# DearCaat/RRT-MIL

Hardware: AMD Instinct MI355X
Metric: slides/sec RRTEncoder fwd, N=9000 D=512 region_num=8 (higher is better)
Workload: dtype f32

## Files before the change

### include/rrt_hip.h

```cpp
#ifndef RRT_HIP_H
#define RRT_HIP_H
#include <stddef.h>
#include <stdint.h>

#ifdef __cplusplus
extern "C" {
#endif

#define RRT_ABI_VERSION 29
#define RRT_MAX_RMSA_LAYERS 8
#define RRT_MAX_CRMSA_K 8

enum {
  RRT_OK = 0,
  RRT_E_INVALID = -1,
  RRT_E_UNSUPPORTED = -2,
  RRT_E_WORKSPACE = -3,
  RRT_E_HANDOVER = -4
};

enum { RRT_COMPUTE_F32 = 0, RRT_COMPUTE_BF16 = 1, RRT_COMPUTE_F16 = 2, RRT_COMPUTE_F32X3 = 3 };
enum { RRT_POS_NONE = 0, RRT_POS_PEG = 1, RRT_POS_PPEG = 2 };
enum { RRT_EPEG_ATTN = 0, RRT_EPEG_VALUE_BF = 1, RRT_EPEG_VALUE_AF = 2 };

enum { RRT_ACT_NONE = 0, RRT_ACT_RELU = 1, RRT_ACT_GELU = 2, RRT_ACT_TANH = 3, RRT_ACT_SIGMOID = 4 };

typedef struct rrt_grid {
  int64_t L;
  int32_t H;
  int32_t s;
  int32_t regions_side;
  int64_t add;
} rrt_grid;

typedef struct rrt_encoder_desc {
  int32_t dim;
  int32_t n_heads;
  int32_t n_rmsa_layers;
  int32_t region_num;
  int32_t region_size;
  int32_t min_region_num;
  float   min_region_ratio;
  int32_t epeg;
  int32_t epeg_k;
  int32_t cr_msa;
  int32_t crmsa_k;
  int32_t crmsa_heads;
  int32_t crmsa_mlp;
  int32_t all_shortcut;
  int32_t compute;
  int32_t ffn;
  int32_t ffn_act;
  int32_t ffn_hidden;
  int32_t pos;
  int32_t pos_pos;
  int32_t peg_k;
  int32_t peg_1d;
  int32_t epeg_2d;
  int32_t epeg_type;
  int32_t weights16_valid;
  int32_t solo;
} rrt_encoder_desc;

typedef struct rrt_attn_weights {
  const float *norm_w, *norm_b;
  const float *qkv_w, *qkv_b;
  const float *proj_w, *proj_b;
  const float *pe_w, *pe_b;
  const float *norm2_w, *norm2_b;
  const float *fc1_w, *fc1_b;
  const float *fc2_w, *fc2_b;
} rrt_attn_weights;

typedef struct rrt_encoder_weights {
  rrt_attn_weights rmsa[RRT_MAX_RMSA_LAYERS];
  rrt_attn_weights crmsa;
  const float *phi;
  const float *phi0_w, *phi2_w;
  const float *norm_w, *norm_b;
  const float *pos_w[3], *pos_b[3];
  uint64_t version;
} rrt_encoder_weights;

int         rrt_abi_version(void);
const char *rrt_strerror(int code);

int rrt_region_grid(int64_t L, int32_t region_num, int32_t region_size,
                    int32_t min_region_num, float min_region_ratio, rrt_grid *out);

int rrt_encoder_workspace_size(const rrt_encoder_desc *desc, int64_t n_tokens, size_t *bytes);

#define RRT_PLAN_FUSED      1
#define RRT_PLAN_FUSED_PROJ 2
#define RRT_PLAN_FUSED16    4
#define RRT_PLAN_FUSED_X3   8
#define RRT_PLAN_CRMSA_PARTS 16
#define RRT_PLAN_ATTN_HD    32
int rrt_encoder_plan(const rrt_encoder_desc *desc, int64_t n_tokens, int32_t *flags);

int rrt_encoder_forward_f32(const rrt_encoder_desc *desc, const rrt_encoder_weights *w,
                            const float *x, float *y, int64_t n_tokens,
                            void *workspace, size_t workspace_bytes, void *stream);

enum {
  RRT_EV_START = 0,
  RRT_EV_LN_PARTITION,
  RRT_EV_QKV,
  RRT_EV_ATTN,
  RRT_EV_PROJ,
  RRT_EV_CR_COMBINE,
  RRT_EV_CR_INNER,
  RRT_EV_END,
  RRT_EV_COUNT
};
int rrt_encoder_forward_events_f32(const rrt_encoder_desc *desc, const rrt_encoder_weights *w,
                                   const float *x, float *y, int64_t n_tokens,
                                   void *workspace, size_t workspace_bytes, void *stream,
                                   void **events);

typedef struct rrt_phase_gate rrt_phase_gate;
int rrt_phase_gate_create(rrt_phase_gate **out);
int rrt_phase_gate_destroy(rrt_phase_gate *gate);
int rrt_encoder_forward_gated_f32(const rrt_encoder_desc *desc, const rrt_encoder_weights *w,
                                  const float *x, float *y, int64_t n_tokens,
                                  void *workspace, size_t workspace_bytes, void *stream,
                                  rrt_phase_gate *gate, void **events);

int rrt_encoder_batch_workspace_size(const rrt_encoder_desc *desc, int32_t batch, int64_t n_tokens, size_t *bytes);
int rrt_encoder_forward_batch_f32(const rrt_encoder_desc *desc, const rrt_encoder_weights *w,
                                  const float *x, float *y, int32_t batch, int64_t n_tokens,
                                  void *workspace, size_t workspace_bytes, void *stream);


int rrt_ln_partition_f32(const float *x, const float *gamma, const float *beta, float *u,
                         int64_t L, int32_t dim, const rrt_grid *g, void *stream);

int rrt_linear_f32(const float *A, const float *B, const float *bias, float *C,
                   int64_t M, int32_t N, int32_t K, int32_t q_cols, float q_scale,
                   int32_t compute , void *stream);

int rrt_linear_unpartition_residual_f32(const float *A, const float *B, const float *bias,
                                        const float *resid, float *out, int32_t N, int32_t K,
                                        const rrt_grid *g, int32_t compute, void *stream);

int rrt_region_attention_f32(const float *qkv, const float *pe_w, float *o,
                             int32_t n_regions, int32_t P, int32_t dim, int32_t heads,
                             int32_t epeg_k, void *stream);

int rrt_region_attention_hd_supported(int32_t P, int32_t dim, int32_t heads, int32_t epeg_k);
int rrt_region_attention_hd_f32(const float *qkv, const float *pe_w, float *o,
                                int32_t n_regions, int32_t P, int32_t dim, int32_t heads,
                                int32_t epeg_k, void *stream);

int rrt_rmsa_fused_f32(const float *u, const float *qkv_w, const float *qkv_b, const float *pe_w,
                       float *o, int32_t n_regions, int32_t P, int32_t dim, int32_t heads,
                       int32_t epeg_k, int32_t compute, void *stream);

int rrt_rmsa_fused_proj_f32(const float *u, const float *qkv_w, const float *qkv_b, const float *pe_w,
                            const float *proj_w, const float *proj_b, const float *resid, float *out,
                            float *o_scratch, int32_t *counters, int32_t dim, int32_t heads, int32_t epeg_k,
                            const rrt_grid *g, void *stream);
int rrt_rmsa_fused_proj_stats_f32(const float *u, const float *qkv_w, const float *qkv_b, const float *pe_w,
                                  const float *proj_w, const float *proj_b, const float *resid, float *out,
                                  float *o_scratch, int32_t *counters, const float *ln2_gamma, const float *phi,
                                  int32_t crmsa_k, float *part, int32_t dim, int32_t heads, int32_t epeg_k,
                                  const rrt_grid *g, void *stream);
int rrt_crmsa_combine_parts_f32(const float *x1, const float *part, const float *gamma, const float *beta,
                                const float *phi, float *wdisp, float *rep, int64_t n_tokens, int32_t dim, int32_t k,
                                const rrt_grid *g8, void *stream);
int rrt_device_error(int32_t clear);
int rrt_debug_rmsa_fused_proj_f32(const float *u, const float *qkv_w, const float *qkv_b, const float *pe_w,
                                  const float *proj_w, const float *proj_b, const float *resid, float *out,
                                  float *o_scratch, int32_t *counters, int32_t dim, int32_t heads, int32_t epeg_k,
                                  const rrt_grid *g, int32_t lag, int32_t spin_limit, int32_t wait_extra, void *stream);

int rrt_cast16(const float *src, uint16_t *dst, int64_t n, int32_t compute, void *stream);
int rrt_ln_partition16(const float *x, const float *gamma, const float *beta, uint16_t *u, int64_t L,
                       int32_t dim, const rrt_grid *g, int32_t compute, void *stream);
int rrt_linear16_f32(const uint16_t *A, const uint16_t *B, const float *bias, const float *resid, float *C,
                     int64_t M, int32_t N, int32_t K, const rrt_grid *g, int32_t compute, void *stream);
int rrt_rmsa_fused16(const uint16_t *u, const uint16_t *qkv_w, const float *qkv_b, const float *pe_w,
                     uint16_t *o, int32_t n_regions, int32_t P, int32_t dim, int32_t heads, int32_t epeg_k,
                     int32_t compute, void *stream);
int rrt_rmsa_pair16_proj(const uint16_t *u, const uint16_t *qkv_w, const float *qkv_b, const float *pe_w,
                         const uint16_t *proj_w, const float *proj_b, const float *resid, float *out, uint16_t *o,
                         int32_t *cnt, int32_t dim, int32_t heads, int32_t epeg_k, const rrt_grid *g, int32_t compute,
                         void *stream);

int rrt_cast_split(const float *src, void *dst, int64_t n, void *stream);
int rrt_ln_partition_split(const float *x, const float *gamma, const float *beta, void *u, int64_t L,
                           int32_t dim, const rrt_grid *g, void *stream);
int rrt_linear_split_f32(const void *A, const void *B, const float *bias, const float *resid, float *C,
                         int64_t M, int32_t N, int32_t K, const rrt_grid *g, void *stream);
int rrt_rmsa_fused_x3(const void *u, const void *qkv_w, const float *qkv_b, const float *pe_w, void *o,
                      int32_t n_regions, int32_t P, int32_t dim, int32_t heads, int32_t epeg_k, void *stream);

int rrt_crmsa_logits_f32(const float *x1, const float *gamma, const float *beta, const float *phi,
                         float *mean_rstd, float *logits, int64_t L, int32_t dim, int32_t k,
                         const rrt_grid *g8, void *stream);
int rrt_crmsa_combine_f32(const float *x1, const float *gamma, const float *beta,
                          const float *mean_rstd, const float *logits, float *wdisp, float *rep,
                          int64_t L, int32_t dim, int32_t k, const rrt_grid *g8, void *stream);
int rrt_crmsa_region_f32(const float *x1, const float *gamma, const float *beta, const float *phi,
                         float *mean_rstd, float *logits, float *wdisp, float *rep,
                         int64_t L, int32_t dim, int32_t k, const rrt_grid *g8, void *stream);
int rrt_crmsa_region4_f32(const float *x1, const float *gamma, const float *beta, const float *phi,
                          float *mean_rstd, float *logits, float *wdisp, float *rep,
                          int64_t L, int32_t dim, int32_t k, const rrt_grid *g8,
                          void *scratch, size_t scratch_bytes, void *stream);
int rrt_crmsa_stream4_f32(const float *x1, const float *gamma, const float *beta, const float *phi,
                          float *mean_rstd, float *logits, float *wdisp, float *rep,
                          int64_t L, int32_t dim, int32_t k, const rrt_grid *g8,
                          void *scratch, size_t scratch_bytes, void *stream);
int rrt_crmsa_dispatch_ln_f32(const float *x1, const float *x0, const float *wdisp,
                              const float *rep2, const float *gamma,
                              const float *beta, float *y, int64_t L, int32_t dim, int32_t k,
                              const rrt_grid *g8, void *stream);
int rrt_crmsa_mlp_logits_f32(const float *hid, const float *w2, float *logits, int64_t rows,
                             int32_t hdim, int32_t k, void *stream);
int rrt_layernorm_f32(const float *x1, const float *x0, const float *gamma, const float *beta,
                      float *y, int64_t L, int32_t dim, void *stream);

typedef struct rrt_mil_desc {
  rrt_encoder_desc enc;
  int32_t input_dim;
  int32_t emb_act;
  int32_t n_classes;
  int32_t pool_hidden;
  int32_t pool_act;
  int32_t pool_gated;
  int32_t input16;
} rrt_mil_desc;

typedef struct rrt_mil_weights {
  rrt_encoder_weights enc;
  const float *emb_w, *emb_b;
  const float *pool_a_w, *pool_a_b;
  const float *pool_b_w, *pool_b_b;
  const float *pool_c_w, *pool_c_b;
  const float *pred_w, *pred_b;
} rrt_mil_weights;

int rrt_attn_pool_workspace_size(int64_t n_tokens, int32_t dim, int32_t hidden, size_t *bytes);
int rrt_attn_pool_f32(const float *y, const float *hid_a, const float *hid_b, const float *c_w, const float *c_b,
                      float *pooled, float *attn, float *a_raw, int64_t n_tokens, int32_t dim, int32_t hidden,
                      void *workspace, size_t workspace_bytes, void *stream);
int rrt_attn_pool_backward_f32(const float *y, const float *hid_a, const float *hid_b, const float *c_w,
                               const float *attn, const float *pooled, const float *d_pooled,
                               const float *d_attn, const float *d_raw, const float *c_ext, float *dy,
                               float *dhid_a, float *dhid_b, float *dwcb, int64_t n_tokens, int32_t dim,
                               int32_t hidden, void *workspace, size_t workspace_bytes, void *stream);

int rrt_mil_workspace_size(const rrt_mil_desc *desc, int64_t n_tokens, size_t *bytes);

int rrt_mil_forward_f32(const rrt_mil_desc *desc, const rrt_mil_weights *w, const float *x,
                        float *logits, float *attn, int32_t no_norm, float *feat, int64_t n_tokens,
                        void *workspace, size_t workspace_bytes, void *stream);

int rrt_pool_workspace_size(int64_t n_tokens, int32_t dim, int32_t hidden, int32_t gated, size_t *bytes);
int rrt_pool_predict_f32(const float *y, const float *a_w, const float *a_b, const float *b_w,
                         const float *b_b, const float *c_w, const float *c_b, const float *pred_w,
                         const float *pred_b, float *pooled, float *logits, float *attn, int32_t no_norm,
                         int64_t n_tokens, int32_t dim, int32_t hidden, int32_t act, int32_t n_classes,
                         int32_t compute, void *workspace, size_t workspace_bytes, void *stream);

int rrt_linear_act_f32(const float *A, const float *B, const float *bias, float *C, int64_t M, int32_t N,
                       int32_t K, int32_t act, int32_t compute, void *stream);

int rrt_branch_pool_workspace_size(int64_t n_tokens, int32_t dim, int32_t hidden, int32_t n_branches, size_t *bytes);
int rrt_branch_pool_f32(const float *y, const float *hid_a, const float *hid_b, const float *c_w, const float *c_b,
                        float *pooled, float *attn, float *a_raw, int64_t n_tokens, int32_t dim, int32_t hidden,
                        int32_t n_branches, void *workspace, size_t workspace_bytes, void *stream);
int rrt_branch_pool_backward_f32(const float *y, const float *hid_a, const float *hid_b, const float *c_w,
                                 const float *attn, const float *pooled, const float *d_pooled, const float *d_raw,
                                 float *dy, float *dhid_a, float *dhid_b, float *dwcb, int64_t n_tokens, int32_t dim,
                                 int32_t hidden, int32_t n_branches, void *workspace, size_t workspace_bytes,
                                 void *stream);

int rrt_topk_rows_f32(const float *x, int64_t *idx, int32_t n_rows, int64_t n, int32_t k, void *stream);

typedef struct rrt_clam_desc {
  rrt_encoder_desc enc;
  int32_t input_dim;
  int32_t emb_act;
  int32_t has_rrt;
  int32_t n_classes;
  int32_t per_branch;
  int32_t gated;
  int32_t hidden;
  int32_t k_sample;
} rrt_clam_desc;

typedef struct rrt_clam_weights {
  rrt_encoder_weights enc;
  const float *emb_w, *emb_b;
  const float *a_w, *a_b;
  const float *b_w, *b_b;
  const float *c_w, *c_b;
  const float *cls_w, *cls_b;
} rrt_clam_weights;

int rrt_clam_workspace_size(const rrt_clam_desc *desc, int64_t n_tokens, size_t *bytes);
int rrt_clam_forward_f32(const rrt_clam_desc *desc, const rrt_clam_weights *w, const float *x, float *logits,
                         float *a_raw, float *attn, float *features, int64_t *topk_idx, int64_t n_tokens,
                         void *workspace, size_t workspace_bytes, void *stream);

int rrt_instance_max_workspace_size(int64_t n_tokens, int32_t dim, int32_t n_classes, size_t *bytes);
int rrt_instance_max_f32(const float *y, const float *w, const float *b, float *classes, float *cmax, int64_t *argmax,
                         int64_t n_tokens, int32_t dim, int32_t n_classes, void *workspace, size_t workspace_bytes,
                         void *stream);

int rrt_dsmil_pool_workspace_size(int64_t n_tokens, int32_t dim, int32_t q_dim, int32_t n_classes, size_t *bytes);
int rrt_dsmil_pool_f32(const float *feats, const int64_t *argmax, const float *q_w, const float *q_b, const float *fcc_w,
                       const float *fcc_b, float *logits, float *A, float *B, float *a_raw, int64_t n_tokens, int32_t dim,
                       int32_t q_dim, int32_t n_classes, void *workspace, size_t workspace_bytes, void *stream);

typedef struct rrt_dsmil_desc {
  rrt_encoder_desc enc;
  int32_t input_dim;
  int32_t emb_act;
  int32_t has_rrt;
  int32_t n_classes;
  int32_t q_dim;
} rrt_dsmil_desc;

typedef struct rrt_dsmil_weights {
  rrt_encoder_weights enc;
  const float *emb_w, *emb_b;
  const float *icls_w, *icls_b;
  const float *q_w, *q_b;
  const float *fcc_w, *fcc_b;
} rrt_dsmil_weights;

int rrt_dsmil_workspace_size(const rrt_dsmil_desc *desc, int64_t n_tokens, size_t *bytes);
int rrt_dsmil_forward_f32(const rrt_dsmil_desc *desc, const rrt_dsmil_weights *w, const float *x, float *logits,
                          float *classes_max, float *A, float *B, int64_t *argmax, int64_t n_tokens, void *workspace,
                          size_t workspace_bytes, void *stream);

typedef struct rrt_executor rrt_executor;
typedef struct rrt_bag {
  const float *x;
  float *y;
  int64_t n_tokens;
} rrt_bag;
int rrt_executor_create(const rrt_encoder_desc *desc, int32_t n_streams, int64_t max_tokens,
                        rrt_executor **out);
int rrt_executor_create_on_streams(const rrt_encoder_desc *desc, int32_t n_streams, void *const *streams,
                                   int64_t max_tokens, rrt_executor **out);
int rrt_executor_forward(rrt_executor *ex, const rrt_encoder_weights *w, const rrt_bag *bags,
                         int32_t n_bags, void *stream);
int rrt_executor_destroy(rrt_executor *ex);

int rrt_region_attention_backward_workspace_size(int32_t n_regions, int32_t P, int32_t dim, int32_t heads,
                                                 int32_t epeg_k, size_t *bytes);
int rrt_region_attention_backward_f32(const float *qkv, const float *pe_w, const float *o, const float *d_o,
                                      float *d_qkv, float *d_pe_w, int32_t n_regions, int32_t P, int32_t dim,
                                      int32_t heads, int32_t epeg_k, void *workspace, size_t workspace_bytes,
                                      void *stream);
int rrt_peg_f32(const float *x, const float *const *w, const float *const *b, float *y, int64_t N, int32_t dim, int32_t k,
                int32_t conv_1d, int32_t ppeg, void *stream);
int rrt_peg_backward_workspace_size(int64_t N, int32_t dim, int32_t k, int32_t ppeg, size_t *bytes);
int rrt_peg_backward_f32(const float *x, const float *dy, const float *const *w, float *dx, float *const *dw, float *const *db,
                         int64_t N, int32_t dim, int32_t k, int32_t conv_1d, int32_t ppeg, void *workspace,
                         size_t workspace_bytes, void *stream);
int rrt_attn_scoremap_scratch_size(int32_t n_regions, int32_t P, int32_t heads, int32_t k, int32_t backward, size_t *bytes);
int rrt_attn_scoremap_f32(const float *qkv, const float *pe_w, float *o, int32_t n_regions, int32_t P, int32_t dim,
                          int32_t heads, int32_t k, void *scratch, size_t scratch_bytes, void *stream);
int rrt_attn_scoremap_backward_f32(const float *qkv, const float *pe_w, const float *d_o, float *d_qkv, float *d_pe_w,
                                   int32_t n_regions, int32_t P, int32_t dim, int32_t heads, int32_t k, void *scratch,
                                   size_t scratch_bytes, void *stream);
// ... 110 lines not shown
```

### rrt-mil_amd/_lib.py

```python
import ctypes as C
import os

HERE = os.path.dirname(os.path.abspath(__file__))
LIB_PATH = os.path.join(HERE, "librrt_hip.so")

RRT_MAX_RMSA_LAYERS = 8
RRT_MAX_CRMSA_K = 8
ABI_VERSION = 29

_f32p = C.POINTER(C.c_float)


class Grid(C.Structure):
    _fields_ = [("L", C.c_int64), ("H", C.c_int32), ("s", C.c_int32),
                ("regions_side", C.c_int32), ("add", C.c_int64)]


class EncoderDesc(C.Structure):
    _fields_ = [("dim", C.c_int32), ("n_heads", C.c_int32), ("n_rmsa_layers", C.c_int32),
                ("region_num", C.c_int32), ("region_size", C.c_int32), ("min_region_num", C.c_int32),
                ("min_region_ratio", C.c_float), ("epeg", C.c_int32), ("epeg_k", C.c_int32),
                ("cr_msa", C.c_int32), ("crmsa_k", C.c_int32), ("crmsa_heads", C.c_int32),
                ("crmsa_mlp", C.c_int32), ("all_shortcut", C.c_int32), ("compute", C.c_int32),
                ("ffn", C.c_int32), ("ffn_act", C.c_int32), ("ffn_hidden", C.c_int32),
                ("pos", C.c_int32), ("pos_pos", C.c_int32), ("peg_k", C.c_int32), ("peg_1d", C.c_int32),
                ("epeg_2d", C.c_int32), ("epeg_type", C.c_int32), ("weights16_valid", C.c_int32),
                ("solo", C.c_int32)]


class AttnWeights(C.Structure):
    _fields_ = [(n, C.c_void_p) for n in ("norm_w", "norm_b", "qkv_w", "qkv_b", "proj_w", "proj_b",
                                          "pe_w", "pe_b", "norm2_w", "norm2_b", "fc1_w", "fc1_b",
                                          "fc2_w", "fc2_b")]


class EncoderWeights(C.Structure):
    _fields_ = [("rmsa", AttnWeights * RRT_MAX_RMSA_LAYERS), ("crmsa", AttnWeights),
                ("phi", C.c_void_p), ("phi0_w", C.c_void_p), ("phi2_w", C.c_void_p),
                ("norm_w", C.c_void_p), ("norm_b", C.c_void_p),
                ("pos_w", C.c_void_p * 3), ("pos_b", C.c_void_p * 3), ("version", C.c_uint64)]


class AttnGrads(C.Structure):
    _fields_ = [(n, C.c_void_p) for n in ("norm", "qkv_w", "qkv_b", "proj_w", "proj_b", "pe_w", "pe_b", "norm2",
                                          "fc1_w", "fc1_b", "fc2_w", "fc2_b")]


class EncoderGrads(C.Structure):
    _fields_ = [("rmsa", AttnGrads * RRT_MAX_RMSA_LAYERS), ("crmsa", AttnGrads), ("phi", C.c_void_p),
                ("phi0_w", C.c_void_p), ("phi2_w", C.c_void_p), ("norm", C.c_void_p),
                ("pos_w", C.c_void_p * 3), ("pos_b", C.c_void_p * 3)]


class MilDesc(C.Structure):
    _fields_ = [("enc", EncoderDesc), ("input_dim", C.c_int32), ("emb_act", C.c_int32),
                ("n_classes", C.c_int32), ("pool_hidden", C.c_int32), ("pool_act", C.c_int32),
                ("pool_gated", C.c_int32), ("input16", C.c_int32)]


class MilWeights(C.Structure):
    _fields_ = [("enc", EncoderWeights)] + [(n, C.c_void_p) for n in (
        "emb_w", "emb_b", "pool_a_w", "pool_a_b", "pool_b_w", "pool_b_b", "pool_c_w", "pool_c_b",
        "pred_w", "pred_b")]


class ClamDesc(C.Structure):
    _fields_ = [("enc", EncoderDesc), ("input_dim", C.c_int32), ("emb_act", C.c_int32), ("has_rrt", C.c_int32),
                ("n_classes", C.c_int32), ("per_branch", C.c_int32), ("gated", C.c_int32), ("hidden", C.c_int32),
                ("k_sample", C.c_int32)]


class ClamWeights(C.Structure):
    _fields_ = [("enc", EncoderWeights)] + [(n, C.c_void_p) for n in (
        "emb_w", "emb_b", "a_w", "a_b", "b_w", "b_b", "c_w", "c_b", "cls_w", "cls_b")]


class DsmilDesc(C.Structure):
    _fields_ = [("enc", EncoderDesc), ("input_dim", C.c_int32), ("emb_act", C.c_int32), ("has_rrt", C.c_int32),
                ("n_classes", C.c_int32), ("q_dim", C.c_int32)]


class DsmilWeights(C.Structure):
    _fields_ = [("enc", EncoderWeights)] + [(n, C.c_void_p) for n in (
        "emb_w", "emb_b", "icls_w", "icls_b", "q_w", "q_b", "fcc_w", "fcc_b")]


class NystromDesc(C.Structure):
    _fields_ = [(n, C.c_int32) for n in ("dim", "heads", "dim_head", "num_landmarks", "pinv_iterations", "residual",
                                         "residual_conv_kernel")]


class NystromWeights(C.Structure):
    _fields_ = [(n, C.c_void_p) for n in ("qkv_w", "out_w", "out_b", "conv_w")]


class TransmilDesc(C.Structure):
    _fields_ = [("input_dim", C.c_int32), ("n_classes", C.c_int32), ("act", C.c_int32), ("attn", NystromDesc)]


class TransmilLayerWeights(C.Structure):
    _fields_ = [("norm_w", C.c_void_p), ("norm_b", C.c_void_p), ("attn", NystromWeights)]


class TransmilWeights(C.Structure):
    _fields_ = [("fc1_w", C.c_void_p), ("fc1_b", C.c_void_p), ("cls_token", C.c_void_p), ("layer", TransmilLayerWeights * 2),
                ("pos_w", C.c_void_p * 3), ("pos_b", C.c_void_p * 3), ("norm_w", C.c_void_p), ("norm_b", C.c_void_p),
                ("fc2_w", C.c_void_p), ("fc2_b", C.c_void_p)]


class Bag(C.Structure):
    _fields_ = [("x", C.c_void_p), ("y", C.c_void_p), ("n_tokens", C.c_int64)]


ACT_NONE, ACT_RELU, ACT_GELU, ACT_TANH, ACT_SIGMOID = 0, 1, 2, 3, 4
ACT_BY_NAME = {"relu": ACT_RELU, "gelu": ACT_GELU, "tanh": ACT_TANH}

SIGNATURES = {
    "rrt_abi_version": (C.c_int, []),
    "rrt_strerror": (C.c_char_p, [C.c_int]),
    "rrt_region_grid": (C.c_int, [C.c_int64, C.c_int32, C.c_int32, C.c_int32, C.c_float, C.POINTER(Grid)]),
    "rrt_encoder_workspace_size": (C.c_int, [C.POINTER(EncoderDesc), C.c_int64, C.POINTER(C.c_size_t)]),
    "rrt_encoder_plan": (C.c_int, [C.POINTER(EncoderDesc), C.c_int64, C.POINTER(C.c_int32)]),
    "rrt_encoder_forward_f32": (C.c_int, [C.POINTER(EncoderDesc), C.POINTER(EncoderWeights), C.c_void_p,
                                          C.c_void_p, C.c_int64, C.c_void_p, C.c_size_t, C.c_void_p]),
    "rrt_encoder_forward_events_f32": (C.c_int, [C.POINTER(EncoderDesc), C.POINTER(EncoderWeights), C.c_void_p,
                                                 C.c_void_p, C.c_int64, C.c_void_p, C.c_size_t, C.c_void_p,
                                                 C.POINTER(C.c_void_p)]),
    "rrt_encoder_batch_workspace_size": (C.c_int, [C.POINTER(EncoderDesc), C.c_int32, C.c_int64, C.POINTER(C.c_size_t)]),
    "rrt_encoder_forward_batch_f32": (C.c_int, [C.POINTER(EncoderDesc), C.POINTER(EncoderWeights), C.c_void_p, C.c_void_p,
                                                C.c_int32, C.c_int64, C.c_void_p, C.c_size_t, C.c_void_p]),
    "rrt_phase_gate_create": (C.c_int, [C.POINTER(C.c_void_p)]),
    "rrt_phase_gate_destroy": (C.c_int, [C.c_void_p]),
    "rrt_encoder_forward_gated_f32": (C.c_int, [C.POINTER(EncoderDesc), C.POINTER(EncoderWeights), C.c_void_p,
                                                C.c_void_p, C.c_int64, C.c_void_p, C.c_size_t, C.c_void_p,
                                                C.c_void_p, C.POINTER(C.c_void_p)]),
    "rrt_ln_partition_f32": (C.c_int, [C.c_void_p, C.c_void_p, C.c_void_p, C.c_void_p, C.c_int64,
                                       C.c_int32, C.POINTER(Grid), C.c_void_p]),
    "rrt_linear_f32": (C.c_int, [C.c_void_p, C.c_void_p, C.c_void_p, C.c_void_p, C.c_int64, C.c_int32,
                                 C.c_int32, C.c_int32, C.c_float, C.c_int32, C.c_void_p]),
    "rrt_linear_unpartition_residual_f32": (C.c_int, [C.c_void_p, C.c_void_p, C.c_void_p, C.c_void_p,
                                                      C.c_void_p, C.c_int32, C.c_int32, C.POINTER(Grid),
                                                      C.c_int32, C.c_void_p]),
    "rrt_region_attention_f32": (C.c_int, [C.c_void_p, C.c_void_p, C.c_void_p, C.c_int32, C.c_int32,
                                           C.c_int32, C.c_int32, C.c_int32, C.c_void_p]),
    "rrt_region_attention_hd_supported": (C.c_int, [C.c_int32] * 4),
    "rrt_region_attention_hd_f32": (C.c_int, [C.c_void_p, C.c_void_p, C.c_void_p, C.c_int32, C.c_int32,
                                              C.c_int32, C.c_int32, C.c_int32, C.c_void_p]),
    "rrt_rmsa_fused_f32": (C.c_int, [C.c_void_p] * 5 + [C.c_int32] * 6 + [C.c_void_p]),
    "rrt_rmsa_fused_proj_f32": (C.c_int, [C.c_void_p] * 10 + [C.c_int32] * 3 + [C.c_void_p] * 2),
    "rrt_device_error": (C.c_int, [C.c_int32]),
    "rrt_rmsa_fused_proj_stats_f32": (C.c_int, [C.c_void_p] * 12 + [C.c_int32, C.c_void_p] + [C.c_int32] * 3 + [C.c_void_p] * 2),
    "rrt_crmsa_combine_parts_f32": (C.c_int, [C.c_void_p] * 7 + [C.c_int64, C.c_int32, C.c_int32, C.POINTER(Grid), C.c_void_p]),
    "rrt_debug_rmsa_fused_proj_f32": (C.c_int, [C.c_void_p] * 10 + [C.c_int32] * 3 + [C.c_void_p] + [C.c_int32] * 3 + [C.c_void_p]),
    "rrt_cast16": (C.c_int, [C.c_void_p, C.c_void_p, C.c_int64, C.c_int32, C.c_void_p]),
    "rrt_ln_partition16": (C.c_int, [C.c_void_p, C.c_void_p, C.c_void_p, C.c_void_p, C.c_int64, C.c_int32,
                                     C.POINTER(Grid), C.c_int32, C.c_void_p]),
    "rrt_linear16_f32": (C.c_int, [C.c_void_p] * 5 + [C.c_int64, C.c_int32, C.c_int32, C.POINTER(Grid), C.c_int32,
                                                      C.c_void_p]),
    "rrt_rmsa_fused16": (C.c_int, [C.c_void_p] * 5 + [C.c_int32] * 6 + [C.c_void_p]),
    "rrt_rmsa_pair16_proj": (C.c_int, [C.c_void_p] * 10 + [C.c_int32] * 3 + [C.POINTER(Grid), C.c_int32, C.c_void_p]),
    "rrt_cast_split": (C.c_int, [C.c_void_p, C.c_void_p, C.c_int64, C.c_void_p]),
    "rrt_ln_partition_split": (C.c_int, [C.c_void_p, C.c_void_p, C.c_void_p, C.c_void_p, C.c_int64, C.c_int32,
                                         C.POINTER(Grid), C.c_void_p]),
    "rrt_linear_split_f32": (C.c_int, [C.c_void_p] * 5 + [C.c_int64, C.c_int32, C.c_int32, C.POINTER(Grid), C.c_void_p]),
    "rrt_rmsa_fused_x3": (C.c_int, [C.c_void_p] * 5 + [C.c_int32] * 5 + [C.c_void_p]),
    "rrt_crmsa_logits_f32": (C.c_int, [C.c_void_p] * 6 + [C.c_int64, C.c_int32, C.c_int32,
                                                         C.POINTER(Grid), C.c_void_p]),
    "rrt_crmsa_combine_f32": (C.c_int, [C.c_void_p] * 7 + [C.c_int64, C.c_int32, C.c_int32,
                                                          C.POINTER(Grid), C.c_void_p]),
    "rrt_crmsa_region_f32": (C.c_int, [C.c_void_p] * 8 + [C.c_int64, C.c_int32, C.c_int32, C.POINTER(Grid), C.c_void_p]),
    "rrt_crmsa_region4_f32": (C.c_int, [C.c_void_p] * 8 + [C.c_int64, C.c_int32, C.c_int32, C.POINTER(Grid), C.c_void_p,
                                                         C.c_size_t, C.c_void_p]),
    "rrt_crmsa_stream4_f32": (C.c_int, [C.c_void_p] * 8 + [C.c_int64, C.c_int32, C.c_int32, C.POINTER(Grid), C.c_void_p,
                                                         C.c_size_t, C.c_void_p]),
    "rrt_crmsa_dispatch_ln_f32": (C.c_int, [C.c_void_p] * 7 + [C.c_int64, C.c_int32, C.c_int32,
                                                              C.POINTER(Grid), C.c_void_p]),
    "rrt_crmsa_mlp_logits_f32": (C.c_int, [C.c_void_p] * 3 + [C.c_int64, C.c_int32, C.c_int32, C.c_void_p]),
    "rrt_layernorm_f32": (C.c_int, [C.c_void_p] * 5 + [C.c_int64, C.c_int32, C.c_void_p]),
    "rrt_peg_f32": (C.c_int, [C.c_void_p] * 4 + [C.c_int64] + [C.c_int32] * 4 + [C.c_void_p]),
    "rrt_peg_backward_workspace_size": (C.c_int, [C.c_int64] + [C.c_int32] * 3 + [C.POINTER(C.c_size_t)]),
    "rrt_peg_backward_f32": (C.c_int, [C.c_void_p] * 6 + [C.c_int64] + [C.c_int32] * 4 + [C.c_void_p, C.c_size_t, C.c_void_p]),
    "rrt_attn_scoremap_scratch_size": (C.c_int, [C.c_int32] * 5 + [C.POINTER(C.c_size_t)]),
    "rrt_attn_scoremap_f32": (C.c_int, [C.c_void_p] * 3 + [C.c_int32] * 5 + [C.c_void_p, C.c_size_t, C.c_void_p]),
    "rrt_attn_scoremap_backward_f32": (C.c_int, [C.c_void_p] * 5 + [C.c_int32] * 5 + [C.c_void_p, C.c_size_t, C.c_void_p]),
    "rrt_value_pe_f32": (C.c_int, [C.c_void_p] * 4 + [C.c_int32] * 7 + [C.c_void_p]),
    "rrt_value_pe_backward_f32": (C.c_int, [C.c_void_p] * 7 + [C.c_int32] * 7 + [C.c_void_p]),
    "rrt_mil_workspace_size": (C.c_int, [C.POINTER(MilDesc), C.c_int64, C.POINTER(C.c_size_t)]),
    "rrt_mil_forward_f32": (C.c_int, [C.POINTER(MilDesc), C.POINTER(MilWeights), C.c_void_p, C.c_void_p,
                                      C.c_void_p, C.c_int32, C.c_void_p, C.c_int64, C.c_void_p, C.c_size_t,
                                      C.c_void_p]),
    "rrt_pool_workspace_size": (C.c_int, [C.c_int64, C.c_int32, C.c_int32, C.c_int32, C.POINTER(C.c_size_t)]),
    "rrt_pool_predict_f32": (C.c_int, [C.c_void_p] * 12 + [C.c_int32, C.c_int64] + [C.c_int32] * 5 +
                             [C.c_void_p, C.c_size_t, C.c_void_p]),
    "rrt_attn_pool_workspace_size": (C.c_int, [C.c_int64, C.c_int32, C.c_int32, C.POINTER(C.c_size_t)]),
    "rrt_attn_pool_f32": (C.c_int, [C.c_void_p] * 8 + [C.c_int64, C.c_int32, C.c_int32, C.c_void_p, C.c_size_t, C.c_void_p]),
    "rrt_attn_pool_backward_f32": (C.c_int, [C.c_void_p] * 14 + [C.c_int64, C.c_int32, C.c_int32, C.c_void_p, C.c_size_t,
                                                                 C.c_void_p]),
    "rrt_branch_pool_workspace_size": (C.c_int, [C.c_int64, C.c_int32, C.c_int32, C.c_int32, C.POINTER(C.c_size_t)]),
    "rrt_branch_pool_f32": (C.c_int, [C.c_void_p] * 8 + [C.c_int64, C.c_int32, C.c_int32, C.c_int32, C.c_void_p, C.c_size_t,
                                                         C.c_void_p]),
    "rrt_branch_pool_backward_f32": (C.c_int, [C.c_void_p] * 12 + [C.c_int64, C.c_int32, C.c_int32, C.c_int32, C.c_void_p,
                                                                   C.c_size_t, C.c_void_p]),
    "rrt_topk_rows_f32": (C.c_int, [C.c_void_p, C.c_void_p, C.c_int32, C.c_int64, C.c_int32, C.c_void_p]),
    "rrt_clam_workspace_size": (C.c_int, [C.POINTER(ClamDesc), C.c_int64, C.POINTER(C.c_size_t)]),
    "rrt_clam_forward_f32": (C.c_int, [C.POINTER(ClamDesc), C.POINTER(ClamWeights)] + [C.c_void_p] * 6 +
                             [C.c_int64, C.c_void_p, C.c_size_t, C.c_void_p]),
    "rrt_instance_max_workspace_size": (C.c_int, [C.c_int64, C.c_int32, C.c_int32, C.POINTER(C.c_size_t)]),
    "rrt_instance_max_f32": (C.c_int, [C.c_void_p] * 6 + [C.c_int64, C.c_int32, C.c_int32, C.c_void_p, C.c_size_t, C.c_void_p]),
    "rrt_dsmil_pool_workspace_size": (C.c_int, [C.c_int64, C.c_int32, C.c_int32, C.c_int32, C.POINTER(C.c_size_t)]),
    "rrt_dsmil_pool_f32": (C.c_int, [C.c_void_p] * 10 + [C.c_int64, C.c_int32, C.c_int32, C.c_int32, C.c_void_p, C.c_size_t,
                                                         C.c_void_p]),
    "rrt_dsmil_workspace_size": (C.c_int, [C.POINTER(DsmilDesc), C.c_int64, C.POINTER(C.c_size_t)]),
    "rrt_dsmil_forward_f32": (C.c_int, [C.POINTER(DsmilDesc), C.POINTER(DsmilWeights)] + [C.c_void_p] * 6 +
                              [C.c_int64, C.c_void_p, C.c_size_t, C.c_void_p]),
    "rrt_executor_create": (C.c_int, [C.POINTER(EncoderDesc), C.c_int32, C.c_int64, C.POINTER(C.c_void_p)]),
    "rrt_executor_create_on_streams": (C.c_int, [C.POINTER(EncoderDesc), C.c_int32, C.POINTER(C.c_void_p), C.c_int64,
                                                 C.POINTER(C.c_void_p)]),
    "rrt_executor_forward": (C.c_int, [C.c_void_p, C.POINTER(EncoderWeights), C.POINTER(Bag), C.c_int32,
                                       C.c_void_p]),
    "rrt_executor_destroy": (C.c_int, [C.c_void_p]),
    "rrt_region_attention_backward_workspace_size": (C.c_int, [C.c_int32] * 5 + [C.POINTER(C.c_size_t)]),
    "rrt_region_attention_backward_f32": (C.c_int, [C.c_void_p] * 6 + [C.c_int32] * 5 + [C.c_void_p, C.c_size_t,
                                                                                       C.c_void_p]),
    "rrt_layernorm_backward_f32": (C.c_int, [C.c_void_p] * 6 + [C.c_int64, C.c_int32, C.POINTER(Grid), C.c_void_p,
                                                                C.c_size_t, C.c_void_p]),
    "rrt_reduce_partials_f32": (C.c_int, [C.c_void_p] * 3 + [C.c_int32, C.c_int64, C.c_int64] + [C.c_int32] * 4 + [C.c_void_p]),
    "rrt_linear_backward_workspace_size": (C.c_int, [C.c_int64, C.c_int32, C.c_int32, C.POINTER(C.c_size_t)]),
    "rrt_linear_backward_f32": (C.c_int, [C.c_void_p] * 6 + [C.c_int64, C.c_int32, C.c_int32, C.c_int32,
                                                             C.c_void_p, C.c_size_t, C.c_void_p]),
    "rrt_encoder_train_sizes": (C.c_int, [C.POINTER(EncoderDesc), C.c_int64, C.POINTER(C.c_size_t),
                                          C.POINTER(C.c_size_t)]),
    "rrt_encoder_forward_train_f32": (C.c_int, [C.POINTER(EncoderDesc), C.POINTER(EncoderWeights), C.c_void_p,
                                                C.c_void_p, C.c_int64, C.c_void_p, C.c_size_t, C.c_float,
                                                C.c_uint64, C.POINTER(C.c_float), C.c_void_p]),
    "rrt_encoder_backward_f32": (C.c_int, [C.POINTER(EncoderDesc), C.POINTER(EncoderWeights), C.c_void_p, C.c_void_p,
                                           C.c_void_p, C.c_size_t, C.POINTER(EncoderGrads), C.c_void_p, C.c_int64,
                                           C.c_void_p, C.c_size_t, C.c_float, C.c_uint64, C.POINTER(C.c_float),
                                           C.c_void_p]),
    "rrt_linear_act_f32": (C.c_int, [C.c_void_p] * 4 + [C.c_int64, C.c_int32, C.c_int32, C.c_int32, C.c_int32,
                                                        C.c_void_p]),
    "rrt_nystrom_workspace_size": (C.c_int, [C.POINTER(NystromDesc), C.c_int64, C.POINTER(C.c_size_t)]),
    "rrt_nystrom_attention_f32": (C.c_int, [C.POINTER(NystromDesc), C.POINTER(NystromWeights), C.c_void_p, C.c_void_p,
                                            C.c_int64, C.c_void_p, C.c_size_t, C.c_void_p]),
    "rrt_nystrom_landmarks_f32": (C.c_int, [C.c_void_p] * 3 + [C.c_int64, C.c_int32, C.c_void_p]),
    "rrt_nystrom_landmark_sim_f32": (C.c_int, [C.c_void_p] * 3 + [C.c_int32, C.c_void_p]),
    "rrt_nystrom_landmark_attn_workspace_size": (C.c_int, [C.c_int64, C.c_int32, C.POINTER(C.c_size_t)]),
    "rrt_nystrom_landmark_attn_f32": (C.c_int, [C.c_void_p] * 3 + [C.c_int64, C.c_int32, C.c_void_p, C.c_size_t, C.c_void_p]),
    "rrt_nystrom_pinv_workspace_size": (C.c_int, [C.c_int32, C.POINTER(C.c_size_t)]),
    "rrt_nystrom_pinv_f32": (C.c_int, [C.c_void_p] * 2 + [C.c_int32, C.c_int32, C.c_void_p, C.c_size_t, C.c_void_p]),
    "rrt_nystrom_zav_f32": (C.c_int, [C.c_void_p] * 3 + [C.c_int32, C.c_void_p]),
    "rrt_nystrom_output_f32": (C.c_int, [C.c_void_p] * 5 + [C.c_int64, C.c_int32, C.c_int32, C.c_void_p]),
    "rrt_ppeg_side_f32": (C.c_int, [C.c_void_p] * 4 + [C.c_int32, C.c_int32, C.c_void_p]),
    "rrt_transmil_workspace_size": (C.c_int, [C.POINTER(TransmilDesc), C.c_int64, C.POINTER(C.c_size_t)]),
    "rrt_transmil_forward_f32": (C.c_int, [C.POINTER(TransmilDesc), C.POINTER(TransmilWeights)] + [C.c_void_p] * 3 +
                                 [C.c_int64, C.c_void_p, C.c_size_t, C.c_void_p]),
}

COMPUTE_F32, COMPUTE_BF16, COMPUTE_F16, COMPUTE_F32X3 = 0, 1, 2, 3
POS_NONE, POS_PEG, POS_PPEG = 0, 1, 2
EPEG_ATTN, EPEG_VALUE_BF, EPEG_VALUE_AF = 0, 1, 2

PLAN_FUSED, PLAN_FUSED_PROJ, PLAN_FUSED16, PLAN_FUSED_X3, PLAN_CRMSA_PARTS, PLAN_ATTN_HD = 1, 2, 4, 8, 16, 32
EV_START, EV_LN_PARTITION, EV_QKV, EV_ATTN, EV_PROJ, EV_CR_COMBINE, EV_CR_INNER, EV_END, EV_COUNT = range(9)

_lib = None


class RRTHipError(RuntimeError):
    pass


def load(path=None):
    global _lib
    if _lib is not None and path is None:
        return _lib
    p = path or os.environ.get("RRT_HIP_LIB") or LIB_PATH
    if not os.path.exists(p):
        raise RRTHipError(
            f"{p} is missing: the HIP extension is the only compute path. Build it with "
            "`python rrt-mil_amd/build.py` (needs /opt/rocm/bin/hipcc).")
    lib = C.CDLL(p)
    for name, (res, args) in SIGNATURES.items():
        fn = getattr(lib, name)
        fn.restype = res
        fn.argtypes = args
    if lib.rrt_abi_version() != ABI_VERSION:
        raise RRTHipError(f"librrt_hip.so ABI {lib.rrt_abi_version()} != binding {ABI_VERSION}; rebuild")
    if path is None:
        _lib = lib
    return lib


E_HANDOVER = -4


def device_error(clear=False):
    return int(load().rrt_device_error(1 if clear else 0))


def check(rc, what=""):
    if rc != 0:
        msg = load().rrt_strerror(rc).decode()
        if rc == -2:
            raise NotImplementedError(f"rrt_hip {what}: {msg}")
        if rc == E_HANDOVER:
            msg += (" -- sticky until cleared: torch.cuda.synchronize(), discard the outputs of the forwards in flight, "
                    "rrt_mil_amd.device_error(clear=True), run them again")
        raise RRTHipError(f"rrt_hip {what} failed ({rc}): {msg}")


def region_grid(L, region_num=8, region_size=0, min_region_num=0, min_region_ratio=0.0):
    g = Grid()
    check(load().rrt_region_grid(L, region_num, region_size, min_region_num, min_region_ratio, C.byref(g)),
          "rrt_region_grid")
    return g
```

### rrt-mil_amd/csrc/api.hip

```cpp
#include <math.h>
#include <stdio.h>
#include <string.h>

#include "internal.h"

namespace {

thread_local char g_detail[256] = "";

int unsupported(const char* why) {
  snprintf(g_detail, sizeof(g_detail), "%s", why);
  return RRT_E_UNSUPPORTED;
}

int64_t ceil_sqrt(int64_t n) {
  int64_t r = (int64_t)floor(sqrt((double)n));
  while (r * r > n) --r;
  while ((r + 1) * (r + 1) <= n) ++r;
  return r * r == n ? r : r + 1;
}

inline size_t align_up(size_t v, size_t a) { return (v + a - 1) / a * a; }

#define RRT_TRY(call)                     \
// ... 30 lines not shown
  const size_t R8 = (size_t)g8.regions_side * g8.regions_side;
  if (d.n_rmsa_layers > 0) w.w16 = (uint16_t*)take((size_t)d.n_rmsa_layers * 4 * D * D);
  if (d.cr_msa) w.wcr16 = (uint16_t*)take(2 * D * D);
  if (d.n_rmsa_layers > 0) {
    w.uo = take(Np * D);
    w.qkv = take(Np * 3 * D);
    w.xa = take((size_t)N * D);
    if (d.n_rmsa_layers > 1 || d.ffn) w.xb = take((size_t)N * D);
    w.proj_cnt = (int*)take((size_t)g.regions_side * g.regions_side);
    if (d.epeg && d.epeg_type != RRT_EPEG_ATTN) w.pe_out = take(Np * D);
    if (d.epeg && d.epeg_2d && d.epeg_type == RRT_EPEG_ATTN) {
      const size_t sm = attn_scoremap_scratch_floats(g.regions_side * g.regions_side, g.s * g.s, d.n_heads, d.epeg_k, 1);
      if (sm) w.smap = take(sm);
    }
  }
  if (d.ffn) {
    if (!w.xa) w.xa = take((size_t)N * D);
    if (!w.xb) w.xb = take((size_t)N * D);
    w.ffn_ln = take((size_t)N * D);
    w.ffn_hid = take((size_t)N * d.ffn_hidden);
  }
  if (d.cr_msa) {
    const size_t k = d.crmsa_k;
    w.mean_rstd = take((size_t)N * 2);
    w.logits = take(Np8 * k);
    w.wdisp = take(Np8 * k);
    w.rep = take(k * R8 * D);
    w.rep_qkv = take(k * R8 * 3 * D);
    w.rep_o = take(k * R8 * D);
    w.rep2 = take(k * R8 * D);
    w.rep16 = (uint16_t*)take(k * R8 * D / 2);
    w.repo16 = (uint16_t*)take(k * R8 * D / 2);
    if (d.n_rmsa_layers > 0) {
      w.cr_part = take(crmsa_region4_scratch_floats(to_dev(g8), d.crmsa_k));
      w.cr_cnt = (int*)take(64);
      if (D % 64 == 0) w.cr_pstat = take(crmsa_parts_floats(N, (int)D, d.crmsa_k));
    }
    if (d.crmsa_mlp) {
      w.v8 = take(Np8 * D);
      w.hid = take(Np8 * (D / 4));
    }
  }
  if (d.pos) w.xp = take((size_t)N * D);
  w.bytes = off ? off : 256;
  return w;
}

int check_desc(const rrt_encoder_desc* d, int64_t N) {
  if (!d || N <= 0) return RRT_E_INVALID;
  if (d->dim <= 0 || d->dim % 32 != 0) return unsupported("dim must be a positive multiple of 32");
  if (d->dim > 2048) return unsupported("dim > 2048");
  if (d->n_rmsa_layers < 0 || d->n_rmsa_layers > RRT_MAX_RMSA_LAYERS) return unsupported("n_layers-1 out of range");
  if (d->n_rmsa_layers > 0) {
    if (d->n_heads <= 0 || d->dim % d->n_heads != 0) return unsupported("n_heads must divide dim");
    if (d->epeg && (d->epeg_k <= 0 || d->epeg_k % 2 == 0)) return unsupported("epeg_k must be odd");
    if (d->epeg_type < RRT_EPEG_ATTN || d->epeg_type > RRT_EPEG_VALUE_AF) return unsupported("epeg_type must be attn / value_bf / value_af");
    if (d->epeg && (d->epeg_2d || d->epeg_type != RRT_EPEG_ATTN) && d->epeg_k > 63) return unsupported("epeg ablations: epeg_k <= 63");
    if (d->region_size <= 0 && d->region_num <= 0) return unsupported("region_num must be positive");
  }
  if (d->cr_msa) {
    if (d->crmsa_k <= 0 || d->crmsa_k > RRT_MAX_CRMSA_K) return unsupported("crmsa_k must be in [1,8]");
    if (d->crmsa_heads <= 0 || d->dim % d->crmsa_heads != 0) return unsupported("crmsa_heads must divide dim");
  }
  if (d->ffn) {
    if (d->ffn_hidden <= 0 || d->ffn_hidden % 32 != 0)
      return unsupported("ffn: hidden width int(dim * mlp_ratio) must be a positive multiple of 32");
    if (d->ffn_act != RRT_ACT_GELU && d->ffn_act != RRT_ACT_RELU) return unsupported("ffn_act must be gelu or relu");
  }
  if (d->pos) {
    if (d->pos != RRT_POS_PEG && d->pos != RRT_POS_PPEG) return unsupported("pos must be none / peg / ppeg");
    if (d->peg_k <= 0 || d->peg_k % 2 == 0 || d->peg_k > 11) return unsupported("peg_k must be odd and <= 11");
    if (d->pos_pos != -1 && d->pos_pos != 0) return unsupported("pos_pos must be -1 or 0");
  }
  if (N > (int64_t)4000000) return unsupported("bag larger than 4e6 tokens");
  if (d->compute < 0 || d->compute > RRT_COMPUTE_F32X3) return unsupported("compute must be RRT_COMPUTE_F32/BF16/F16/F32X3");
  return RRT_OK;
}

int region_grids(const rrt_encoder_desc* d, int64_t N, rrt_grid* g, rrt_grid* g8) {
  *g = rrt_grid{};
  if (d->n_rmsa_layers > 0) {
    int rc = rrt_region_grid(N, d->region_num, d->region_size, d->min_region_num, d->min_region_ratio, g);
    if (rc) return rc;
  }
  return rrt_region_grid(N, 8, 0, 0, 0.f, g8);
}
int resolve_grids(const rrt_encoder_desc* d, int64_t N, rrt_grid* g, rrt_grid* g8) {
  int rc = check_desc(d, N);
  return rc ? rc : region_grids(d, N, g, g8);
}

GridDev identity_grid(int64_t N) {
  GridDev g{};
  const int Hs = (int)ceil_sqrt(N);
  g.L = (int)N;
  g.H = g.s = Hs;
  g.rs = 1;
  g.P = g.Np = Hs * Hs;
  g.inv_H = g.inv_s = 1.0f / (float)Hs;
  g.inv_rs = 1.0f;
  g.inv_P = 1.0f / (float)g.P;
  g.Rt = 1;
  return g;
}

LinearEpilogue qkv_epilogue(const float* bias, int dim, int heads, int prec) {
  LinearEpilogue ep{};
  ep.prec = prec;
  ep.bias = bias;
  ep.q_cols = dim;
  ep.q_scale = 1.0f / sqrtf((float)(dim / heads));
  return ep;
}

LinearEpilogue proj_epilogue(const float* bias, const float* resid, const GridDev& g, int prec) {
  LinearEpilogue ep{};
  ep.prec = prec;
  ep.bias = bias;
  ep.resid = resid;
  ep.g = g;
  return ep;
}

hipError_t inner_attention(const float* u, int n_regions, int P, const rrt_attn_weights& w, int dim,
                           int heads, int epeg_k, float* qkv, float* o, int prec, bool solo, hipStream_t st) {
  const int M = n_regions * P;
  LinearEpilogue ep = qkv_epilogue(w.qkv_b, dim, heads, prec);
  ep.solo = solo;
  hipError_t e = launch_linear(u, w.qkv_w, qkv, M, 3 * dim, dim, ep, st);
  if (e != hipSuccess) return e;
  return launch_region_attention(qkv, epeg_k > 0 ? w.pe_w : nullptr, o, n_regions, P, dim, heads,
                                 epeg_k, st);
}

enum class LayerKind {
  Pair16Merged,
  Fused16,
  FusedX3,
  EpegVariant,
  FusedProj,
  Fused,
  Unfused,
};
enum class FrontKind { None, Mlp, Parts, RegionInFlight, Region4, Region, Stream4, TwoKernel };
enum class CastKind { None, Images16, Split };
struct EncoderPlan {
  LayerKind layer;
  bool parts;
  bool gated;
  bool attn_hd;
  CastKind casts;
  bool inner16;
  FrontKind front;
};

#ifndef RRT_STREAM4_MIN_P
#define RRT_STREAM4_MIN_P 145
#endif

EncoderPlan plan_encoder(const rrt_encoder_desc& d, const rrt_grid& g, const rrt_grid& g8, bool stops_before_crmsa) {
  EncoderPlan p{};
  p.layer = LayerKind::Unfused;
  const int D = d.dim;
  const bool want_x3 = d.compute == RRT_COMPUTE_F32X3;
  const int compute = want_x3 ? RRT_COMPUTE_F32 : d.compute;
  const bool lowp = compute != RRT_COMPUTE_F32 && D % 64 == 0;
  const GridDev gd8 = to_dev(g8);
  p.inner16 = d.cr_msa && lowp && rmsa_fused16_supported(64, D, d.crmsa_heads, 0);
  if (d.n_rmsa_layers > 0) {
    const GridDev gd = to_dev(g);
    const int R = gd.rs * gd.rs, heads = d.n_heads, ek = d.epeg ? d.epeg_k : 0;
    const bool rows_ok = rmsa_fused_supported_rows(gd.Np, D);
    static const bool want_merged16 = rrt_tune_env("RRT_PAIR16_PROJ") != nullptr;
    if (d.epeg && (d.epeg_2d || d.epeg_type != RRT_EPEG_ATTN)) {
      p.layer = LayerKind::EpegVariant;
    } else if (lowp && rmsa_fused16_supported(gd.P, D, heads, ek) && rows_ok) {
      p.layer = want_merged16 && rmsa_pair16_proj_supported(R, gd.P, D, heads, ek) ? LayerKind::Pair16Merged : LayerKind::Fused16;
    } else if (want_x3 && D % 256 == 0 && rmsa_fused_x3_supported(gd.P, D, heads, ek) && rows_ok) {
      p.layer = LayerKind::FusedX3;
    } else if (compute == RRT_COMPUTE_F32 && rows_ok && rmsa_fused_proj_supported(R, gd.P, D, heads, ek, compute)) {
      p.layer = LayerKind::FusedProj;
      p.parts = d.solo != 0 && d.cr_msa && !d.crmsa_mlp && !d.ffn && d.crmsa_k <= 4 && !stops_before_crmsa && D % 64 == 0 &&
                crmsa_combine_parts_supported(D, d.crmsa_k, gd8);
    } else if (rmsa_fused_supported(gd.P, D, heads, ek) && rows_ok) {
      p.layer = LayerKind::Fused;
    } else {
      p.attn_hd = region_attention_hd_supported(gd.P, D, heads, ek);
    }
    p.gated = gd.P > 112 && p.layer != LayerKind::EpegVariant && p.layer != LayerKind::Unfused;
    if (p.layer != LayerKind::EpegVariant) p.casts = lowp ? CastKind::Images16 : want_x3 ? CastKind::Split : CastKind::None;
  }
  if (!d.cr_msa || stops_before_crmsa) return p;
  const int k = d.crmsa_k;
  const bool has_counters = d.n_rmsa_layers > 0;
  static const bool no_region_inflight = rrt_tune_env("RRT_NO_REGION_INFLIGHT") != nullptr;
  static const bool region_lowp = rrt_tune_env("RRT_REGION_INFLIGHT_LOWP") != nullptr;
  if (d.crmsa_mlp) {
    p.front = FrontKind::Mlp;
  } else if (p.parts) {
    p.front = FrontKind::Parts;
  } else if (!no_region_inflight && !d.solo && p.layer != LayerKind::FusedX3 && (compute == RRT_COMPUTE_F32 || region_lowp) &&
             crmsa_region_supported(D, k, gd8)) {
    p.front = FrontKind::RegionInFlight;
  } else if (has_counters && crmsa_region4_supported(D, k, gd8) && gd8.P < RRT_STREAM4_MIN_P) {
    p.front = FrontKind::Region4;
  } else if (crmsa_region_enabled() && crmsa_region_supported(D, k, gd8)) {
    p.front = FrontKind::Region;
  } else if (has_counters && gd8.P >= RRT_STREAM4_MIN_P && crmsa_stream4_supported(D, k, gd8)) {
    p.front = FrontKind::Stream4;
  } else {
    p.front = FrontKind::TwoKernel;
  }
  return p;
}

}

GridDev to_dev(const rrt_grid& g) {
  GridDev d;
  d.L = (int)g.L;
  d.H = g.H;
  d.s = g.s;
  d.rs = g.regions_side;
  d.P = g.s * g.s;
  d.Np = g.H * g.H;
  d.inv_H = 1.0f / (float)d.H;
  d.inv_s = 1.0f / (float)d.s;
  d.inv_rs = 1.0f / (float)d.rs;
  d.inv_P = 1.0f / (float)d.P;
  d.Rt = d.rs * d.rs;
  return d;
}

extern "C" {

int rrt_abi_version(void) { return RRT_ABI_VERSION; }

const char* rrt_strerror(int code) {
  switch (code) {
    case RRT_OK: return "ok";
    case RRT_E_INVALID: return "invalid argument (null pointer or non-positive size)";
    case RRT_E_UNSUPPORTED: return g_detail[0] ? g_detail : "unsupported configuration";
    case RRT_E_WORKSPACE: return "workspace too small (see rrt_encoder_workspace_size)";
    case RRT_E_HANDOVER: return "an earlier merged R-MSA launch gave up its in-launch hand-over wait; outputs in flight are invalid "
                                "(synchronise, then rrt_device_error(1) to clear)";
    default: return code > 0 ? hipGetErrorString((hipError_t)code) : "unknown error";
  }
}

int rrt_region_grid(int64_t L, int32_t region_num, int32_t region_size, int32_t min_region_num,
                    float min_region_ratio, rrt_grid* out) {
  if (!out || L <= 0) return RRT_E_INVALID;
  if (region_size <= 0 && region_num <= 0) return RRT_E_INVALID;
  int64_t H = ceil_sqrt(L), s;
  if (region_size > 0) {
    H += ((-H) % region_size + region_size) % region_size;
    s = region_size;
  } else {
    H += ((-H) % region_num + region_num) % region_num;
    s = H / region_num;
  }
  int64_t add = H * H - L;
  if ((double)add > (double)L / ((double)min_region_ratio + 1e-8) || L < min_region_num) {
    H = ceil_sqrt(L);
    H += H % 2;
    add = H * H - L;
    s = H;
  }
  if (H > 46340) return RRT_E_INVALID;
  out->L = L;
  out->H = (int32_t)H;
  out->s = (int32_t)s;
  out->regions_side = (int32_t)(H / s);
  out->add = add;
  return RRT_OK;
}

int rrt_encoder_workspace_size(const rrt_encoder_desc* desc, int64_t n_tokens, size_t* bytes) {
  if (!bytes) return RRT_E_INVALID;
  rrt_grid g{}, g8{};
  int rc = resolve_grids(desc, n_tokens, &g, &g8);
  if (rc) return rc;
  *bytes = carve(*desc, n_tokens, g, g8, nullptr).bytes;
  return RRT_OK;
}

int rrt_encoder_plan(const rrt_encoder_desc* desc, int64_t n_tokens, int32_t* flags) {
  if (!flags) return RRT_E_INVALID;
  *flags = 0;
  rrt_grid g{}, g8{};
  int rc = resolve_grids(desc, n_tokens, &g, &g8);
  if (rc) return rc;
  if (desc->n_rmsa_layers <= 0) return RRT_OK;
  const EncoderPlan plan = plan_encoder(*desc, g, g8, false);
  switch (plan.layer) {
    case LayerKind::Pair16Merged:
    case LayerKind::Fused16: *flags = RRT_PLAN_FUSED16; break;
    case LayerKind::FusedX3: *flags = RRT_PLAN_FUSED_X3; break;
    case LayerKind::FusedProj: *flags = RRT_PLAN_FUSED | RRT_PLAN_FUSED_PROJ | (plan.parts ? RRT_PLAN_CRMSA_PARTS : 0); break;
    case LayerKind::Fused: *flags = RRT_PLAN_FUSED; break;
    case LayerKind::Unfused: *flags = plan.attn_hd ? RRT_PLAN_ATTN_HD : 0; break;
    case LayerKind::EpegVariant: break;
  }
  return RRT_OK;
}

struct rrt_phase_gate {
  hipEvent_t done;
  bool armed;
};

static int ffn_apply(const rrt_encoder_desc* desc, const rrt_attn_weights& lw, const float* xi, float* xo,
                     const Workspace& ws, int64_t N, hipStream_t st) {
  if (!lw.norm2_w || !lw.norm2_b || !lw.fc1_w || !lw.fc1_b || !lw.fc2_w || !lw.fc2_b) return RRT_E_INVALID;
  const int D = desc->dim;
  RRT_TRY(launch_layernorm(xi, nullptr, lw.norm2_w, lw.norm2_b, ws.ffn_ln, (int)N, D, st));
  LinearEpilogue e1{};
  e1.prec = desc->compute;
  e1.bias = lw.fc1_b;
  e1.act = desc->ffn_act;
  RRT_TRY(launch_linear(ws.ffn_ln, lw.fc1_w, ws.ffn_hid, (int)N, desc->ffn_hidden, D, e1, st));
  return (int)launch_linear(ws.ffn_hid, lw.fc2_w, xo, (int)N, D, desc->ffn_hidden,
                            proj_epilogue(lw.fc2_b, xi, identity_grid(N), desc->compute), st);
}

static int encoder_forward(const rrt_encoder_desc* desc_in, const rrt_encoder_weights* w, const float* x,
                           float* y, int64_t n_tokens, void* workspace, size_t workspace_bytes,
                           void* stream, void** events, rrt_phase_gate* gate = nullptr, float* rmsa_out = nullptr,
                           uint16_t* y16 = nullptr, bool* y16_done = nullptr) {
  if (y16_done) *y16_done = false;
  if (!desc_in || !w || !x || !y || x == y) return RRT_E_INVALID;
  int rc = check_desc(desc_in, n_tokens);
  if (rc) return rc;
  if (handover_err_peek(false)) return RRT_E_HANDOVER;
  rrt_grid g{}, g8{};
  rc = region_grids(desc_in, n_tokens, &g, &g8);
  if (rc) return rc;
  rrt_encoder_desc dloc = *desc_in;
  if (dloc.compute == RRT_COMPUTE_F32X3) dloc.compute = RRT_COMPUTE_F32;
  const rrt_encoder_desc* const desc = &dloc;
  hipStream_t st = (hipStream_t)stream;
  const int D = desc->dim;
  const int64_t N = n_tokens;
  Workspace ws = carve(*desc, N, g, g8, nullptr);
  if (!workspace || workspace_bytes < ws.bytes) return RRT_E_WORKSPACE;
  ws = carve(*desc, N, g, g8, (char*)workspace);
  const EncoderPlan plan = plan_encoder(*desc_in, g, g8, rmsa_out != nullptr);

  auto mark = [&](int i) -> hipError_t {
    return (events && events[i]) ? hipEventRecord((hipEvent_t)events[i], st) : hipSuccess;
  };
  RRT_TRY(mark(RRT_EV_START));

  auto ffn_block = [&](const rrt_attn_weights& lw, const float* xi, float* xo) -> int {
    return ffn_apply(desc, lw, xi, xo, ws, N, st);
  };

  const float* xin = x;
  auto pos_embed = [&]() -> int {
    if (!w->pos_w[0] || (desc->pos == RRT_POS_PPEG && (!w->pos_w[1] || !w->pos_w[2]))) return RRT_E_INVALID;
    RRT_TRY(launch_peg(xin, w->pos_w, w->pos_b, ws.xp, (int)N, D, desc->peg_k, desc->peg_1d, desc->pos == RRT_POS_PPEG, st));
    xin = ws.xp;
    return RRT_OK;
  };
  if (desc->pos && desc->pos_pos == -1) {
    rc = pos_embed();
    if (rc) return rc;
  }
  {
    const bool split = plan.casts == CastKind::Split;
    const size_t per_w = split ? 2 : 1;
    Cast16Jobs jobs{};
    auto add = [&](const float* src, uint16_t* dst, size_t n) {
      jobs.src[jobs.count] = src; jobs.dst[jobs.count] = dst; jobs.n4[jobs.count++] = n / 4;
    };
    if (plan.casts != CastKind::None) {
      for (int li = 0; li < desc->n_rmsa_layers; ++li) {
        const rrt_attn_weights& lw = w->rmsa[li];
        if (!lw.qkv_w || !lw.proj_w) return RRT_E_INVALID;
        uint16_t* base = ws.w16 + (size_t)li * per_w * 4 * D * D;
        add(lw.qkv_w, base, (size_t)3 * D * D);
        add(lw.proj_w, base + per_w * 3 * D * D, (size_t)D * D);
      }
    }
    if (plan.inner16) {
      if (!w->crmsa.qkv_w || !w->crmsa.proj_w) return RRT_E_INVALID;
      add(w->crmsa.qkv_w, ws.wcr16, (size_t)3 * D * D);
      add(w->crmsa.proj_w, ws.wcr16 + (size_t)3 * D * D, (size_t)D * D);
    }
    if (jobs.count && !desc->weights16_valid) RRT_TRY(split ? launch_cast_split(jobs, st) : launch_cast16(jobs, desc->compute, st));
  }
  rrt_phase_gate* const gt = (gate && plan.gated) ? gate : nullptr;
  auto gate_record = [&]() -> hipError_t {
    if (!gt) return hipSuccess;
    const hipError_t ge = hipEventRecord(gt->done, st);
    if (ge == hipSuccess) gt->armed = true;
    return ge;
  };
  auto core_begin = [&](bool marks) -> hipError_t {
    if (gt && gt->armed) {
      const hipError_t ge = hipStreamWaitEvent(st, gt->done, 0);
      if (ge != hipSuccess) return ge;
    }
    return marks ? mark(RRT_EV_LN_PARTITION) : hipSuccess;
  };
  auto core_end = [&](bool marks, bool record = true) -> hipError_t {
    hipError_t ge = record ? gate_record() : hipSuccess;
    if (ge == hipSuccess && marks) ge = mark(RRT_EV_QKV);
    if (ge == hipSuccess && marks) ge = mark(RRT_EV_ATTN);
    return ge;
  };
  static const bool gate_proj = rrt_tune_env("RRT_GATE_PROJ") != nullptr;
  for (int li = 0; li < desc->n_rmsa_layers; ++li) {
    if (li == 1 && desc->pos && desc->pos_pos == 0) {
      rc = pos_embed();
      if (rc) return rc;
    }
    const rrt_attn_weights& lw = w->rmsa[li];
    const bool last = li == desc->n_rmsa_layers - 1;
    if (!lw.norm_w || !lw.norm_b || !lw.qkv_w || !lw.proj_w || !lw.proj_b) return RRT_E_INVALID;
    if (desc->epeg && !lw.pe_w) return RRT_E_INVALID;
    if (plan.parts && last && (!w->crmsa.norm_w || !w->crmsa.norm_b || !w->phi)) return RRT_E_INVALID;
    const GridDev gd = to_dev(g);
    const int R = gd.rs * gd.rs, ek = desc->epeg ? desc->epeg_k : 0;
    const float* const pe_w = desc->epeg ? lw.pe_w : nullptr;
    const bool to_out = rmsa_out != nullptr && last;
    float* xout = desc->ffn ? ws.xa : (to_out ? rmsa_out : ((li & 1) ? ws.xb : ws.xa));
    float* const fout = to_out ? rmsa_out : ws.xb;
    const bool marks = li == 0 && plan.layer != LayerKind::EpegVariant;
    auto out_ep = [&](int prec) {
      LinearEpilogue ep = proj_epilogue(lw.proj_b, xin, gd, prec);
      ep.zero64 = ws.cr_cnt;
      return ep;
    };
    switch (plan.layer) {
      case LayerKind::Pair16Merged:
      case LayerKind::Fused16: {
        const bool merged16 = plan.layer == LayerKind::Pair16Merged;
        uint16_t* u16 = (uint16_t*)ws.uo;
        uint16_t* o16 = (uint16_t*)ws.qkv;
        const uint16_t* wq16 = ws.w16 + (size_t)li * 4 * D * D;
        RRT_TRY(launch_ln_partition16(xin, lw.norm_w, lw.norm_b, u16, D, gd, desc->compute, st, merged16 ? ws.proj_cnt : nullptr,
                                      merged16 ? R / 2 : 0));
        RRT_TRY(core_begin(marks));
        if (merged16) {
          PairProj pj{};
          pj.Wp = wq16 + (size_t)3 * D * D;
          pj.bias = lw.proj_b;
          pj.resid = xin;
          pj.out = xout;
          pj.cnt = ws.proj_cnt;
          pj.zero64 = ws.cr_cnt;
          pj.g = gd;
          RRT_TRY(launch_rmsa_pair16_proj(u16, wq16, lw.qkv_b, pe_w, o16, R, gd.P, D, desc->n_heads, ek, desc->compute, pj, st));
          RRT_TRY(core_end(marks));
        } else {
          RRT_TRY(launch_rmsa_fused16(u16, wq16, lw.qkv_b, pe_w, o16, R, gd.P, D, desc->n_heads, ek, desc->compute, st));
          RRT_TRY(core_end(marks));
          LinearEpilogue ep = out_ep(desc->compute);
          ep.solo = desc->solo != 0;
          RRT_TRY(launch_linear16(o16, wq16 + (size_t)3 * D * D, xout, gd.Np, D, D, ep, st));
        }
        break;
      }
      case LayerKind::FusedX3: {
        const uint16_t* wq = ws.w16 + (size_t)li * 8 * D * D;
        RRT_TRY(launch_ln_partition_split(xin, lw.norm_w, lw.norm_b, ws.uo, D, gd, st));
        RRT_TRY(core_begin(marks));
        RRT_TRY(launch_rmsa_fused_x3(ws.uo, wq, lw.qkv_b, pe_w, ws.qkv, R, gd.P, D, desc->n_heads, ek, st));
        RRT_TRY(core_end(marks));
        RRT_TRY(launch_linear_split(ws.qkv, wq + (size_t)6 * D * D, xout, gd.Np, D, D, out_ep(0), st));
        break;
      }
      case LayerKind::FusedProj: {
        RRT_TRY(launch_ln_partition(xin, lw.norm_w, lw.norm_b, ws.uo, D, gd, st, ws.proj_cnt, R));
        RRT_TRY(core_begin(marks));
        FusedProj pj{};
        pj.Wp = lw.proj_w;
        pj.bias = lw.proj_b;
        pj.resid = xin;
        pj.out = xout;
        pj.cnt = ws.proj_cnt;
        pj.zero64 = ws.cr_cnt;
        pj.g = gd;
        if (plan.parts && last) {
          pj.part = ws.cr_pstat;
          pj.ln_g = w->crmsa.norm_w;
          pj.phi = w->phi;
          pj.k = desc->crmsa_k;
        }
        RRT_TRY(launch_rmsa_fused(ws.uo, lw.qkv_w, lw.qkv_b, pe_w, ws.qkv, R, gd.P, D, desc->n_heads, ek, desc->compute, st,
                                  nullptr, &pj));
        RRT_TRY(core_end(marks));
        break;
      }
      case LayerKind::Fused: {
        RRT_TRY(launch_ln_partition(xin, lw.norm_w, lw.norm_b, ws.uo, D, gd, st));
        RRT_TRY(core_begin(marks));
        RRT_TRY(launch_rmsa_fused(ws.uo, lw.qkv_w, lw.qkv_b, pe_w, ws.qkv, R, gd.P, D, desc->n_heads, ek, desc->compute, st));
        RRT_TRY(core_end(marks, !gate_proj));
        RRT_TRY(launch_linear(ws.qkv, lw.proj_w, xout, gd.Np, D, D, out_ep(desc->compute), st));
        if (gate_proj) RRT_TRY(gate_record());
        break;
      }
      case LayerKind::Unfused: {
        RRT_TRY(launch_ln_partition(xin, lw.norm_w, lw.norm_b, ws.uo, D, gd, st));
        RRT_TRY(core_begin(marks));
        RRT_TRY(launch_linear(ws.uo, lw.qkv_w, ws.qkv, gd.Np, 3 * D, D, qkv_epilogue(lw.qkv_b, D, desc->n_heads, desc->compute), st));
        if (marks) RRT_TRY(mark(RRT_EV_QKV));
        RRT_TRY(launch_region_attention(ws.qkv, pe_w, ws.uo, R, gd.P, D, desc->n_heads, ek, st));
        if (marks) RRT_TRY(mark(RRT_EV_ATTN));
        RRT_TRY(launch_linear(ws.uo, lw.proj_w, xout, gd.Np, D, D, out_ep(desc->compute), st));
        break;
      }
      case LayerKind::EpegVariant: {
        RRT_TRY(launch_ln_partition(xin, lw.norm_w, lw.norm_b, ws.uo, D, gd, st));
        RRT_TRY(launch_linear(ws.uo, lw.qkv_w, ws.qkv, gd.Np, 3 * D, D, qkv_epilogue(lw.qkv_b, D, desc->n_heads, desc->compute), st));
        if (desc->epeg_type == RRT_EPEG_ATTN) {
          RRT_TRY(launch_attn_scoremap(ws.qkv, lw.pe_w, ws.uo, ws.smap, R, gd.P, D, desc->n_heads, desc->epeg_k, st));
        } else {
          RRT_TRY(launch_value_pe(ws.qkv, lw.pe_w, lw.pe_b, ws.pe_out, R, gd.P, gd.s, D, desc->n_heads, desc->epeg_k,
                                  desc->epeg_2d, st));
          if (desc->epeg_type == RRT_EPEG_VALUE_BF)
            RRT_TRY(launch_add_cols(ws.qkv + 2 * D, ws.pe_out, (size_t)gd.Np, D, 3 * D, st));
          RRT_TRY(launch_region_attention(ws.qkv, nullptr, ws.uo, R, gd.P, D, desc->n_heads, 0, st));
          if (desc->epeg_type == RRT_EPEG_VALUE_AF)
            RRT_TRY(launch_add_cols(ws.uo, ws.pe_out, (size_t)gd.Np, D, D, st));
        }
        RRT_TRY(launch_linear(ws.uo, lw.proj_w, xout, gd.Np, D, D, out_ep(desc->compute), st));
        break;
      }
    }
    if (marks) RRT_TRY(mark(RRT_EV_PROJ));
    xin = xout;
    if (desc->ffn) {
      rc = ffn_block(lw, xout, fout);
      if (rc) return rc;
      xin = fout;
    }
  }
  if (rmsa_out != nullptr) {
    if (xin != rmsa_out) RRT_TRY(hipMemcpyAsync(rmsa_out, xin, (size_t)N * D * sizeof(float), hipMemcpyDeviceToDevice, st));
    return RRT_OK;
  }
  const float* x0 = desc->all_shortcut ? x : nullptr;
  if (!w->norm_w || !w->norm_b) return RRT_E_INVALID;
  if (!desc->cr_msa) {
    RRT_TRY(launch_layernorm(xin, x0, w->norm_w, w->norm_b, y, (int)N, D, st));
    RRT_TRY(mark(RRT_EV_END));
    return RRT_OK;
  }
  const rrt_attn_weights& cw = w->crmsa;
  if (!cw.norm_w || !cw.norm_b || !cw.qkv_w || !cw.proj_w || !cw.proj_b) return RRT_E_INVALID;
  if (desc->crmsa_mlp ? (!w->phi0_w || !w->phi2_w) : !w->phi) return RRT_E_INVALID;
  const GridDev gd8 = to_dev(g8);
  const int k = desc->crmsa_k, R8 = gd8.rs * gd8.rs;
  uint16_t* const rep16 = plan.inner16 ? ws.rep16 : nullptr;
  switch (plan.front) {
    case FrontKind::Mlp: {
      RRT_TRY(launch_ln_partition(xin, cw.norm_w, cw.norm_b, ws.v8, D, gd8, st));
      LinearEpilogue ep{};
      ep.prec = desc->compute;
      RRT_TRY(launch_linear(ws.v8, w->phi0_w, ws.hid, gd8.Np, D / 4, D, ep, st));
      RRT_TRY(launch_crmsa_mlp_logits(ws.hid, w->phi2_w, ws.logits, gd8.Np, D / 4, k, st));
      RRT_TRY(launch_crmsa_combine(ws.v8, nullptr, nullptr, nullptr, ws.logits, ws.wdisp, ws.rep, rep16, desc->compute, D, k, gd8, st));
      break;
    }
    case FrontKind::Parts:
      RRT_TRY(launch_crmsa_combine_parts(xin, ws.cr_pstat, cw.norm_w, cw.norm_b, w->phi, ws.wdisp, ws.rep, rep16, desc->compute, D,
                                         k, gd8, st));
      break;
    case FrontKind::RegionInFlight:
      RRT_TRY(launch_crmsa_region(xin, cw.norm_w, cw.norm_b, w->phi, nullptr, nullptr, ws.wdisp, ws.rep, k, gd8, st, rep16,
                                  desc->compute));
      break;
    case FrontKind::Region4:
      RRT_TRY(launch_crmsa_region4(xin, cw.norm_w, cw.norm_b, w->phi, nullptr, ws.logits, ws.wdisp, ws.rep, rep16, desc->compute,
                                   ws.cr_part, ws.cr_cnt, k, gd8, st));
      break;
    case FrontKind::Region:
      RRT_TRY(launch_crmsa_region(xin, cw.norm_w, cw.norm_b, w->phi, nullptr, nullptr, ws.wdisp, ws.rep, k, gd8, st));
      break;
    case FrontKind::Stream4:
      RRT_TRY(launch_crmsa_stream4(xin, cw.norm_w, cw.norm_b, w->phi, nullptr, ws.logits, ws.wdisp, ws.rep, rep16, desc->compute,
                                   ws.cr_part, ws.cr_cnt, k, gd8, st));
      break;
    case FrontKind::TwoKernel:
      RRT_TRY(launch_crmsa_logits(xin, cw.norm_w, cw.norm_b, w->phi, ws.mean_rstd, ws.logits, D, k, gd8, st));
      RRT_TRY(launch_crmsa_combine(xin, cw.norm_w, cw.norm_b, ws.mean_rstd, ws.logits, ws.wdisp, ws.rep, rep16, desc->compute, D, k,
                                   gd8, st));
      break;
    case FrontKind::None: break;
  }
  RRT_TRY(mark(RRT_EV_CR_COMBINE));
  if (plan.inner16) {
    if (plan.front == FrontKind::Region) {
      Cast16Jobs cj{};
      cj.src[0] = ws.rep; cj.dst[0] = ws.rep16; cj.n4[0] = (size_t)k * R8 * D / 4; cj.count = 1;
      RRT_TRY(launch_cast16(cj, desc->compute, st));
    }
    RRT_TRY(launch_rmsa_fused16(ws.rep16, ws.wcr16, cw.qkv_b, nullptr, ws.repo16, k, R8, D, desc->crmsa_heads, 0,
                                desc->compute, st));
    LinearEpilogue ep{};
    ep.prec = desc->compute;
    ep.bias = cw.proj_b;
    RRT_TRY(launch_linear16(ws.repo16, ws.wcr16 + (size_t)3 * D * D, ws.rep2, k * R8, D, D, ep, st));
  } else {
    static const bool inner_solo = rrt_tune_env("RRT_INNER_SOLO") != nullptr;
    RRT_TRY(inner_attention(ws.rep, k, R8, cw, D, desc->crmsa_heads, 0, ws.rep_qkv, ws.rep_o, desc->compute, desc->solo != 0 || inner_solo, st));
    LinearEpilogue ep{};
    ep.prec = desc->compute;
    ep.bias = cw.proj_b;
    ep.solo = desc->solo != 0 || inner_solo;
    RRT_TRY(launch_linear(ws.rep_o, cw.proj_w, ws.rep2, k * R8, D, D, ep, st));
  }
  RRT_TRY(mark(RRT_EV_CR_INNER));
  if (desc->ffn) {
    RRT_TRY(launch_crmsa_dispatch_ln(xin, nullptr, ws.wdisp, ws.rep2, nullptr, nullptr, ws.xa, D, k, gd8, st));
    rc = ffn_block(cw, ws.xa, ws.xb);
    if (rc) return rc;
    RRT_TRY(launch_layernorm(ws.xb, x0, w->norm_w, w->norm_b, y, (int)N, D, st));
    RRT_TRY(mark(RRT_EV_END));
    return RRT_OK;
  }
  const bool want16 = y16 != nullptr && (desc->compute == RRT_COMPUTE_BF16 || desc->compute == RRT_COMPUTE_F16) && D % 4 == 0;
  RRT_TRY(launch_crmsa_dispatch_ln(xin, x0, ws.wdisp, ws.rep2, w->norm_w, w->norm_b, y, D, k,
                                   gd8, st, want16 ? y16 : nullptr, want16 ? desc->compute : 0));
  if (want16 && y16_done) *y16_done = true;
  RRT_TRY(mark(RRT_EV_END));
  return RRT_OK;
}

int rrt_encoder_forward_f32(const rrt_encoder_desc* desc, const rrt_encoder_weights* w, const float* x,
                            float* y, int64_t n_tokens, void* workspace, size_t workspace_bytes,
                            void* stream) {
  return encoder_forward(desc, w, x, y, n_tokens, workspace, workspace_bytes, stream, nullptr);
}

int rrt_phase_gate_create(rrt_phase_gate** out) {
  if (!out) return RRT_E_INVALID;
  rrt_phase_gate* g = new rrt_phase_gate();
  g->armed = false;
  hipError_t e = hipEventCreateWithFlags(&g->done, hipEventDisableTiming);
  if (e != hipSuccess) {
    delete g;
    return (int)e;
  }
  *out = g;
  return RRT_OK;
}

int rrt_phase_gate_destroy(rrt_phase_gate* g) {
  if (!g) return RRT_OK;
  (void)hipEventDestroy(g->done);
  delete g;
  return RRT_OK;
}

int rrt_encoder_forward_gated_f32(const rrt_encoder_desc* desc, const rrt_encoder_weights* w, const float* x,
                                  float* y, int64_t n_tokens, void* workspace, size_t workspace_bytes,
                                  void* stream, rrt_phase_gate* gate, void** events) {
  return encoder_forward(desc, w, x, y, n_tokens, workspace, workspace_bytes, stream, events, gate);
}

int rrt_encoder_forward_events_f32(const rrt_encoder_desc* desc, const rrt_encoder_weights* w,
                                   const float* x, float* y, int64_t n_tokens, void* workspace,
                                   size_t workspace_bytes, void* stream, void** events) {
  return encoder_forward(desc, w, x, y, n_tokens, workspace, workspace_bytes, stream, events);
}

namespace {
struct BatchWs {
  Workspace one;
  float *x1, *mean_rstd, *logits, *wdisp, *rep, *rep_qkv, *rep_o, *rep2;
  size_t one_bytes, bytes;
};
BatchWs carve_batch(const rrt_encoder_desc& d, int64_t B, int64_t N, const rrt_grid& g, const rrt_grid& g8, char* base) {
  BatchWs w{};
  w.one_bytes = carve(d, N, g, g8, nullptr).bytes;
  w.one = carve(d, N, g, g8, base);
  size_t off = align_up(w.one_bytes, 256);
  auto take = [&](size_t nfloat) {
    float* p = base ? (float*)(base + off) : nullptr;
    off = align_up(off + nfloat * sizeof(float), 256);
    return p;
  };
  const size_t D = d.dim, Np8 = (size_t)g8.H * g8.H, R8 = (size_t)g8.regions_side * g8.regions_side, k = d.crmsa_k;
  w.x1 = take((size_t)B * N * D);
  if (d.cr_msa) {
    w.mean_rstd = take((size_t)B * N * 2);
    w.logits = take((size_t)B * Np8 * k);
    w.wdisp = take((size_t)B * Np8 * k);
    w.rep = take(k * R8 * B * D);
    w.rep_qkv = take(k * R8 * B * 3 * D);
    w.rep_o = take(k * R8 * B * D);
    w.rep2 = take(k * R8 * B * D);
  }
  w.bytes = off;
  return w;
}
}

int rrt_encoder_batch_workspace_size(const rrt_encoder_desc* desc, int32_t batch, int64_t n_tokens, size_t* bytes) {
  if (!bytes || batch <= 0) return RRT_E_INVALID;
  rrt_grid g{}, g8{};
  int rc = resolve_grids(desc, n_tokens, &g, &g8);
  if (rc) return rc;
  *bytes = carve_batch(*desc, batch, n_tokens, g, g8, nullptr).bytes;
  return RRT_OK;
}

int rrt_encoder_forward_batch_f32(const rrt_encoder_desc* desc_in, const rrt_encoder_weights* w, const float* x, float* y,
                                  int32_t batch, int64_t n_tokens, void* workspace, size_t workspace_bytes, void* stream) {
  if (!desc_in || !w || !x || !y || x == y || batch <= 0) return RRT_E_INVALID;
  int rc = check_desc(desc_in, n_tokens);
  if (rc) return rc;
  if (batch > 1024) return unsupported("batch > 1024");
  rrt_encoder_desc dloc = *desc_in;
  dloc.weights16_valid = 0;
  dloc.solo = 0;
  const rrt_encoder_desc* const desc = &dloc;
  const int64_t N = n_tokens, B = batch;
  const int D = desc->dim;
  hipStream_t st = (hipStream_t)stream;
  rrt_grid g{}, g8{};
  rc = region_grids(desc, N, &g, &g8);
  if (rc) return rc;
  BatchWs bw = carve_batch(*desc, B, N, g, g8, nullptr);
  if (!workspace || workspace_bytes < bw.bytes) return RRT_E_WORKSPACE;
  bw = carve_batch(*desc, B, N, g, g8, (char*)workspace);
  for (int64_t b = 0; b < B; ++b) {
    rc = encoder_forward(&dloc, w, x + (size_t)b * N * D, y + (size_t)b * N * D, N, workspace, bw.one_bytes, stream, nullptr,
                         nullptr, bw.x1 + (size_t)b * N * D);
    if (rc) return rc;
    dloc.weights16_valid = 1;
  }
  dloc.weights16_valid = 0;
  if (!w->norm_w || !w->norm_b) return RRT_E_INVALID;
  if (!desc->cr_msa) {
    for (int64_t b = 0; b < B; ++b)
      RRT_TRY(launch_layernorm(bw.x1 + (size_t)b * N * D, desc->all_shortcut ? x + (size_t)b * N * D : nullptr, w->norm_w,
                               w->norm_b, y + (size_t)b * N * D, (int)N, D, st));
    return RRT_OK;
  }
  const rrt_attn_weights& cw = w->crmsa;
  if (!cw.norm_w || !cw.norm_b || !cw.qkv_w || !cw.proj_w || !cw.proj_b) return RRT_E_INVALID;
  if (desc->crmsa_mlp ? (!w->phi0_w || !w->phi2_w) : !w->phi) return RRT_E_INVALID;
  GridDev gd8 = to_dev(g8);
  const int k = desc->crmsa_k, R8 = gd8.rs * gd8.rs;
  gd8.Rt = R8 * (int)B;
  const size_t Np8 = (size_t)gd8.Np;
  const int prec = desc->compute == RRT_COMPUTE_F32X3 ? RRT_COMPUTE_F32 : desc->compute;
  for (int64_t b = 0; b < B; ++b) {
    const float* xb1 = bw.x1 + (size_t)b * N * D;
    float* lg = bw.logits + (size_t)b * Np8 * k;
    float* wd = bw.wdisp + (size_t)b * Np8 * k;
    float* repb = bw.rep + (size_t)b * R8 * D;
    if (desc->crmsa_mlp) {
      RRT_TRY(launch_ln_partition(xb1, cw.norm_w, cw.norm_b, bw.one.v8, D, gd8, st));
      LinearEpilogue ep{};
      ep.prec = prec;
      RRT_TRY(launch_linear(bw.one.v8, w->phi0_w, bw.one.hid, gd8.Np, D / 4, D, ep, st));
      RRT_TRY(launch_crmsa_mlp_logits(bw.one.hid, w->phi2_w, lg, gd8.Np, D / 4, k, st));
      RRT_TRY(launch_crmsa_combine(bw.one.v8, nullptr, nullptr, nullptr, lg, wd, repb, nullptr, 0, D, k, gd8, st));
    } else {
      float* mr = bw.mean_rstd + (size_t)b * N * 2;
      RRT_TRY(launch_crmsa_logits(xb1, cw.norm_w, cw.norm_b, w->phi, mr, lg, D, k, gd8, st));
      RRT_TRY(launch_crmsa_combine(xb1, cw.norm_w, cw.norm_b, mr, lg, wd, repb, nullptr, 0, D, k, gd8, st));
    }
  }
  RRT_TRY(inner_attention(bw.rep, k, R8 * (int)B, cw, D, desc->crmsa_heads, 0, bw.rep_qkv, bw.rep_o, prec, false, st));
  {
    LinearEpilogue ep{};
    ep.prec = prec;
    ep.bias = cw.proj_b;
    RRT_TRY(launch_linear(bw.rep_o, cw.proj_w, bw.rep2, k * R8 * (int)B, D, D, ep, st));
  }
  for (int64_t b = 0; b < B; ++b) {
    const float* xb1 = bw.x1 + (size_t)b * N * D;
    const float* x0 = desc->all_shortcut ? x + (size_t)b * N * D : nullptr;
    const float* wd = bw.wdisp + (size_t)b * Np8 * k;
    const float* rep2b = bw.rep2 + (size_t)b * R8 * D;
    float* yb = y + (size_t)b * N * D;
    if (desc->ffn) {
      RRT_TRY(launch_crmsa_dispatch_ln(xb1, nullptr, wd, rep2b, nullptr, nullptr, bw.one.xa, D, k, gd8, st));
      rc = ffn_apply(desc, cw, bw.one.xa, bw.one.xb, bw.one, N, st);
      if (rc) return rc;
      RRT_TRY(launch_layernorm(bw.one.xb, x0, w->norm_w, w->norm_b, yb, (int)N, D, st));
    } else {
      RRT_TRY(launch_crmsa_dispatch_ln(xb1, x0, wd, rep2b, w->norm_w, w->norm_b, yb, D, k, gd8, st));
    }
  }
  return RRT_OK;
}

int rrt_ln_partition_f32(const float* x, const float* gamma, const float* beta, float* u, int64_t L,
                         int32_t dim, const rrt_grid* g, void* stream) {
  if (!x || !gamma || !beta || !u || !g || L != g->L || dim <= 0 || dim % 4) return RRT_E_INVALID;
  if (dim > 2048) return unsupported("dim > 2048");
  return (int)launch_ln_partition(x, gamma, beta, u, dim, to_dev(*g), (hipStream_t)stream);
}

int rrt_linear_f32(const float* A, const float* B, const float* bias, float* C, int64_t M, int32_t N,
                   int32_t K, int32_t q_cols, float q_scale, int32_t compute, void* stream) {
  if (!A || !B || !C || M <= 0 || N <= 0 || K <= 0) return RRT_E_INVALID;
  if (K % 32) return unsupported("linear: K must be a multiple of 32");
  if (compute < 0 || compute > 2) return unsupported("compute must be RRT_COMPUTE_F32/BF16/F16");
  LinearEpilogue ep{};
  ep.prec = compute;
  ep.bias = bias;
  ep.q_cols = q_cols;
  ep.q_scale = q_scale;
  return (int)launch_linear(A, B, C, (int)M, N, K, ep, (hipStream_t)stream);
}

int rrt_linear_unpartition_residual_f32(const float* A, const float* B, const float* bias,
                                        const float* resid, float* out, int32_t N, int32_t K,
                                        const rrt_grid* g, int32_t compute, void* stream) {
  if (!A || !B || !resid || !out || !g || N <= 0 || K <= 0) return RRT_E_INVALID;
  if (K % 32) return unsupported("linear: K must be a multiple of 32");
  if (compute < 0 || compute > 2) return unsupported("compute must be RRT_COMPUTE_F32/BF16/F16");
  const LinearEpilogue ep = proj_epilogue(bias, resid, to_dev(*g), compute);
  return (int)launch_linear(A, B, out, ep.g.Np, N, K, ep, (hipStream_t)stream);
}

int rrt_region_attention_f32(const float* qkv, const float* pe_w, float* o, int32_t n_regions, int32_t P,
                             int32_t dim, int32_t heads, int32_t epeg_k, void* stream) {
  if (!qkv || !o || n_regions <= 0 || P <= 0 || dim <= 0 || heads <= 0 || dim % heads) return RRT_E_INVALID;
  if (pe_w && epeg_k > 0 && epeg_k % 2 == 0) return unsupported("epeg_k must be odd");
  return (int)launch_region_attention(qkv, pe_w, o, n_regions, P, dim, heads, epeg_k, (hipStream_t)stream);
}

int rrt_region_attention_hd_supported(int32_t P, int32_t dim, int32_t heads, int32_t epeg_k) {
  return region_attention_hd_supported(P, dim, heads, epeg_k) ? 1 : 0;
}

int rrt_region_attention_hd_f32(const float* qkv, const float* pe_w, float* o, int32_t n_regions, int32_t P, int32_t dim,
                                int32_t heads, int32_t epeg_k, void* stream) {
  if (n_regions <= 0 || P <= 0 || dim <= 0 || heads <= 0 || dim % heads) return RRT_E_INVALID;
  const int ek = pe_w ? epeg_k : 0;
  if (!region_attention_hd_supported(P, dim, heads, ek))
    return unsupported("region_attention_hd: needs a head dim that is a multiple of 16 in [16, 256] other than 64 and "
                       "epeg_k <= 63 (use rrt_region_attention_f32)");
  if (!qkv || !o) return RRT_E_INVALID;
  if (ek > 0 && ek % 2 == 0) return unsupported("epeg_k must be odd");
  if (n_regions > 65535) return unsupported("region_attention_hd: more than 65535 regions in one call");
  return (int)launch_region_attention_hd(qkv, pe_w, o, n_regions, P, dim, heads, ek, (hipStream_t)stream);
}

int rrt_rmsa_fused_f32(const float* u, const float* qkv_w, const float* qkv_b, const float* pe_w, float* o,
                       int32_t n_regions, int32_t P, int32_t dim, int32_t heads, int32_t epeg_k,
                       int32_t compute, void* stream) {
  if (!u || !qkv_w || !o || n_regions <= 0 || P <= 0 || dim <= 0 || heads <= 0) return RRT_E_INVALID;
  if (compute < 0 || compute > 2) return unsupported("compute must be RRT_COMPUTE_F32/BF16/F16");
  const int ek = pe_w ? epeg_k : 0;
  if (!rmsa_fused_supported(P, dim, heads, ek) || !rmsa_fused_supported_rows((long)n_regions * P, dim))
    return unsupported("rmsa_fused: needs head dim 64, 48 < P <= 208, epeg_k <= 63 (use linear + region_attention)");
  return (int)launch_rmsa_fused(u, qkv_w, qkv_b, pe_w, o, n_regions, P, dim, heads, ek, compute,
                                (hipStream_t)stream);
}

int rrt_device_error(int32_t clear) { return handover_err_peek(clear != 0); }

int rrt_rmsa_fused_proj_f32(const float* u, const float* qkv_w, const float* qkv_b, const float* pe_w,
                            const float* proj_w, const float* proj_b, const float* resid, float* out, float* o_scratch,
                            int32_t* counters, int32_t dim, int32_t heads, int32_t epeg_k, const rrt_grid* g,
                            void* stream) {
  return rrt_debug_rmsa_fused_proj_f32(u, qkv_w, qkv_b, pe_w, proj_w, proj_b, resid, out, o_scratch, counters, dim, heads,
                                       epeg_k, g, 0, 0, 0, stream);
}

}
static int fused_proj_stage(const float* u, const float* qkv_w, const float* qkv_b, const float* pe_w,
                            const float* proj_w, const float* proj_b, const float* resid, float* out, float* o_scratch,
                            int32_t* counters, int32_t dim, int32_t heads, int32_t epeg_k, const rrt_grid* g,
                            int32_t lag, int32_t spin_limit, int32_t wait_extra, const float* ln2_gamma, const float* phi,
                            int32_t crmsa_k, float* part, void* stream);
extern "C" {
int rrt_debug_rmsa_fused_proj_f32(const float* u, const float* qkv_w, const float* qkv_b, const float* pe_w,
                                  const float* proj_w, const float* proj_b, const float* resid, float* out, float* o_scratch,
                                  int32_t* counters, int32_t dim, int32_t heads, int32_t epeg_k, const rrt_grid* g,
                                  int32_t lag, int32_t spin_limit, int32_t wait_extra, void* stream) {
  return fused_proj_stage(u, qkv_w, qkv_b, pe_w, proj_w, proj_b, resid, out, o_scratch, counters, dim, heads, epeg_k, g, lag,
                          spin_limit, wait_extra, nullptr, nullptr, 0, nullptr, stream);
}

int rrt_rmsa_fused_proj_stats_f32(const float* u, const float* qkv_w, const float* qkv_b, const float* pe_w,
                                  const float* proj_w, const float* proj_b, const float* resid, float* out, float* o_scratch,
                                  int32_t* counters, const float* ln2_gamma, const float* phi, int32_t crmsa_k, float* part,
                                  int32_t dim, int32_t heads, int32_t epeg_k, const rrt_grid* g, void* stream) {
  if (!ln2_gamma || !phi || !part || crmsa_k < 1 || crmsa_k > RRT_MAX_CRMSA_K) return RRT_E_INVALID;
  return fused_proj_stage(u, qkv_w, qkv_b, pe_w, proj_w, proj_b, resid, out, o_scratch, counters, dim, heads, epeg_k, g, 0, 0, 0,
                          ln2_gamma, phi, crmsa_k, part, stream);
}

int rrt_crmsa_combine_parts_f32(const float* x1, const float* part, const float* gamma, const float* beta, const float* phi,
                                float* wdisp, float* rep, int64_t n_tokens, int32_t dim, int32_t k, const rrt_grid* g8,
                                void* stream) {
  if (!x1 || !part || !gamma || !beta || !phi || !wdisp || !rep || !g8 || n_tokens <= 0 || g8->L != n_tokens) return RRT_E_INVALID;
  const GridDev gd = to_dev(*g8);
  if (!crmsa_combine_parts_supported(dim, k, gd)) return unsupported("crmsa_combine_parts: dim % 64 == 0, dim <= 512, 1 <= k <= 8");
  return (int)launch_crmsa_combine_parts(x1, part, gamma, beta, phi, wdisp, rep, nullptr, 0, dim, k, gd, (hipStream_t)stream);
}
}

static int fused_proj_stage(const float* u, const float* qkv_w, const float* qkv_b, const float* pe_w,
                            const float* proj_w, const float* proj_b, const float* resid, float* out, float* o_scratch,
                            int32_t* counters, int32_t dim, int32_t heads, int32_t epeg_k, const rrt_grid* g,
                            int32_t lag, int32_t spin_limit, int32_t wait_extra, const float* ln2_gamma, const float* phi,
                            int32_t crmsa_k, float* part, void* stream) {
  if (!u || !qkv_w || !proj_w || !resid || !out || !o_scratch || !counters || !g || dim <= 0 || heads <= 0 || out == resid ||
      lag < 0 || spin_limit < 0 || wait_extra < 0)
    return RRT_E_INVALID;
  if (handover_err_peek(false)) return RRT_E_HANDOVER;
  const GridDev gd = to_dev(*g);
  const int ek = pe_w ? epeg_k : 0, R = gd.rs * gd.rs;
  if (!rmsa_fused_proj_supported(R, gd.P, dim, heads, ek, RRT_COMPUTE_F32) || !rmsa_fused_supported_rows(gd.Np, dim))
    return unsupported("rmsa_fused_proj: needs what rmsa_fused needs (head dim 64, 64 < P <= 208, epeg_k <= 63) and at "
                       "least two rounds of (region, head) items (heads * regions >= 2 x the CU count)");
  hipError_t e = hipMemsetAsync(counters, 0, (size_t)R * sizeof(int32_t), (hipStream_t)stream);
  if (e != hipSuccess) return (int)e;
  FusedProj pj{};
  pj.Wp = proj_w;
  pj.bias = proj_b;
  pj.resid = resid;
  pj.out = out;
  pj.cnt = counters;
  pj.g = gd;
  pj.lag = lag;
  pj.spin_limit = spin_limit;
  pj.wait_for = wait_extra > 0 ? heads + wait_extra : 0;
  pj.part = part;
  pj.ln_g = ln2_gamma;
  pj.phi = phi;
  pj.k = crmsa_k;
  if (lag > 0 && (lag < 8 * heads || lag > heads * R)) return unsupported("rmsa_fused_proj: lag must be in [8 * heads, heads * regions]");
  return (int)launch_rmsa_fused(u, qkv_w, qkv_b, pe_w, o_scratch, R, gd.P, dim, heads, ek, RRT_COMPUTE_F32,
                                (hipStream_t)stream, nullptr, &pj);
}
extern "C" {

int rrt_cast16(const float* src, uint16_t* dst, int64_t n, int32_t compute, void* stream) {
  if (!src || !dst || n <= 0 || n % 4) return RRT_E_INVALID;
  if (compute != RRT_COMPUTE_BF16 && compute != RRT_COMPUTE_F16) return unsupported("cast16: compute must be BF16 or F16");
  Cast16Jobs jobs{};
  jobs.src[0] = src; jobs.dst[0] = dst; jobs.n4[0] = (size_t)n / 4; jobs.count = 1;
  return (int)launch_cast16(jobs, compute, (hipStream_t)stream);
}

int rrt_ln_partition16(const float* x, const float* gamma, const float* beta, uint16_t* u, int64_t L, int32_t dim,
                       const rrt_grid* g, int32_t compute, void* stream) {
  if (!x || !gamma || !beta || !u || !g || L != g->L || dim <= 0 || dim % 4) return RRT_E_INVALID;
  if (dim > 2048) return unsupported("dim > 2048");
  if (compute != RRT_COMPUTE_BF16 && compute != RRT_COMPUTE_F16) return unsupported("compute must be BF16 or F16");
  return (int)launch_ln_partition16(x, gamma, beta, u, dim, to_dev(*g), compute, (hipStream_t)stream);
}

int rrt_linear16_f32(const uint16_t* A, const uint16_t* B, const float* bias, const float* resid, float* C, int64_t M,
                     int32_t N, int32_t K, const rrt_grid* g, int32_t compute, void* stream) {
  if (!A || !B || !C || M <= 0 || N <= 0 || K <= 0 || (resid && !g)) return RRT_E_INVALID;
  if (K % 64) return unsupported("linear16: K must be a multiple of 64");
  if (compute != RRT_COMPUTE_BF16 && compute != RRT_COMPUTE_F16) return unsupported("compute must be BF16 or F16");
  LinearEpilogue ep{};
  ep.prec = compute;
  ep.bias = bias;
  if (resid) {
    ep.resid = resid;
    ep.g = to_dev(*g);
    if (M != ep.g.Np) return RRT_E_INVALID;
  }
  return (int)launch_linear16(A, B, C, (int)M, N, K, ep, (hipStream_t)stream);
}

int rrt_rmsa_fused16(const uint16_t* u, const uint16_t* qkv_w, const float* qkv_b, const float* pe_w, uint16_t* o,
                     int32_t n_regions, int32_t P, int32_t dim, int32_t heads, int32_t epeg_k, int32_t compute,
                     void* stream) {
  if (!u || !qkv_w || !o || n_regions <= 0 || P <= 0 || dim <= 0 || heads <= 0) return RRT_E_INVALID;
  if (compute != RRT_COMPUTE_BF16 && compute != RRT_COMPUTE_F16) return unsupported("compute must be BF16 or F16");
  const int ek = pe_w ? epeg_k : 0;
  if (!rmsa_fused16_supported(P, dim, heads, ek) || !rmsa_fused_supported_rows((long)n_regions * P, dim))
    return unsupported("rmsa_fused16: needs head dim 64, 16 < P <= 256, epeg_k <= 63");
  return (int)launch_rmsa_fused16(u, qkv_w, qkv_b, pe_w, o, n_regions, P, dim, heads, ek, compute, (hipStream_t)stream);
}

int rrt_rmsa_pair16_proj(const uint16_t* u, const uint16_t* qkv_w, const float* qkv_b, const float* pe_w, const uint16_t* proj_w,
                         const float* proj_b, const float* resid, float* out, uint16_t* o, int32_t* cnt, int32_t dim,
                         int32_t heads, int32_t epeg_k, const rrt_grid* g, int32_t compute, void* stream) {
  if (!u || !qkv_w || !proj_w || !resid || !out || !o || !cnt || !g || dim <= 0 || heads <= 0) return RRT_E_INVALID;
  if (compute != RRT_COMPUTE_BF16 && compute != RRT_COMPUTE_F16) return unsupported("compute must be BF16 or F16");
  if (handover_err_peek(false)) return RRT_E_HANDOVER;
  const GridDev gd = to_dev(*g);
  const int ek = pe_w ? epeg_k : 0, R = gd.rs * gd.rs;
  if (!rmsa_pair16_proj_supported(R, gd.P, dim, heads, ek))
    return unsupported("rmsa_pair16_proj: head dim 64, regions of 65..96 or 113..128 tokens, a multiple of 16 regions, "
                       "at least two rounds of (pair, head) items");
  hipError_t e = hipMemsetAsync(cnt, 0, (size_t)(R / 2) * sizeof(int), (hipStream_t)stream);
  if (e != hipSuccess) return (int)e;
  PairProj pj{};
  pj.Wp = proj_w;
  pj.bias = proj_b;
  pj.resid = resid;
  pj.out = out;
  pj.cnt = cnt;
  pj.g = gd;
  return (int)launch_rmsa_pair16_proj(u, qkv_w, qkv_b, pe_w, o, R, gd.P, dim, heads, ek, compute, pj, (hipStream_t)stream);
}

int rrt_cast_split(const float* src, void* dst, int64_t n, void* stream) {
  if (!src || !dst || n <= 0 || n % 32) return RRT_E_INVALID;
  Cast16Jobs jobs{};
  jobs.src[0] = src; jobs.dst[0] = (uint16_t*)dst; jobs.n4[0] = (size_t)n / 4; jobs.count = 1;
  return (int)launch_cast_split(jobs, (hipStream_t)stream);
}

int rrt_ln_partition_split(const float* x, const float* gamma, const float* beta, void* u, int64_t L, int32_t dim,
                           const rrt_grid* g, void* stream) {
  if (!x || !gamma || !beta || !u || !g || L != g->L || dim <= 0 || dim % 32) return RRT_E_INVALID;
  if (dim > 2048) return unsupported("dim > 2048");
  return (int)launch_ln_partition_split(x, gamma, beta, u, dim, to_dev(*g), (hipStream_t)stream);
}

int rrt_linear_split_f32(const void* A, const void* B, const float* bias, const float* resid, float* C, int64_t M,
                         int32_t N, int32_t K, const rrt_grid* g, void* stream) {
  if (!A || !B || !C || M <= 0 || N <= 0 || K <= 0 || (resid && !g)) return RRT_E_INVALID;
  if (K % 32) return unsupported("linear_split: K must be a multiple of 32");
  LinearEpilogue ep{};
  ep.bias = bias;
  if (resid) {
    ep.resid = resid;
    ep.g = to_dev(*g);
    if (M != ep.g.Np) return RRT_E_INVALID;
  }
  return (int)launch_linear_split(A, B, C, (int)M, N, K, ep, (hipStream_t)stream);
}

int rrt_rmsa_fused_x3(const void* u, const void* qkv_w, const float* qkv_b, const float* pe_w, void* o,
                      int32_t n_regions, int32_t P, int32_t dim, int32_t heads, int32_t epeg_k, void* stream) {
  if (!u || !qkv_w || !o || n_regions <= 0 || P <= 0 || dim <= 0 || heads <= 0) return RRT_E_INVALID;
  const int ek = pe_w ? epeg_k : 0;
  if (!rmsa_fused_x3_supported(P, dim, heads, ek) || !rmsa_fused_supported_rows((long)n_regions * P, dim))
    return unsupported("rmsa_fused_x3: needs head dim 64, 48 < P <= 144, epeg_k <= 63");
  return (int)launch_rmsa_fused_x3(u, qkv_w, qkv_b, pe_w, o, n_regions, P, dim, heads, ek, (hipStream_t)stream);
}

int rrt_crmsa_logits_f32(const float* x1, const float* gamma, const float* beta, const float* phi,
                         float* mean_rstd, float* logits, int64_t L, int32_t dim, int32_t k,
                         const rrt_grid* g8, void* stream) {
  if (!x1 || !gamma || !beta || !phi || !mean_rstd || !logits || !g8 || L != g8->L) return RRT_E_INVALID;
  if (k <= 0 || k > RRT_MAX_CRMSA_K || dim % 4 || dim > 2048) return unsupported("crmsa: k in [1,8], dim%4==0, dim<=2048");
  return (int)launch_crmsa_logits(x1, gamma, beta, phi, mean_rstd, logits, dim, k, to_dev(*g8),
                                  (hipStream_t)stream);
}

int rrt_crmsa_combine_f32(const float* x1, const float* gamma, const float* beta, const float* mean_rstd,
                          const float* logits, float* wdisp, float* rep, int64_t L, int32_t dim, int32_t k,
                          const rrt_grid* g8, void* stream) {
  if (!x1 || !logits || !wdisp || !rep || !g8 || L != g8->L) return RRT_E_INVALID;
  if (mean_rstd && (!gamma || !beta)) return RRT_E_INVALID;
  if (k <= 0 || k > RRT_MAX_CRMSA_K || dim % 4) return unsupported("crmsa: k in [1,8], dim%4==0");
  return (int)launch_crmsa_combine(x1, gamma, beta, mean_rstd, logits, wdisp, rep, nullptr, 0, dim, k, to_dev(*g8),
                                   (hipStream_t)stream);
}

int rrt_crmsa_region_f32(const float* x1, const float* gamma, const float* beta, const float* phi, float* mean_rstd,
                         float* logits, float* wdisp, float* rep, int64_t L, int32_t dim, int32_t k, const rrt_grid* g8,
                         void* stream) {
  if (!x1 || !gamma || !beta || !phi || !wdisp || !rep || !g8 || L != g8->L) return RRT_E_INVALID;
  const GridDev gd = to_dev(*g8);
  if (!crmsa_region_supported(dim, k, gd)) return unsupported("crmsa_region: dim = 512, k <= 3, regions of <= 144 tokens");
  return (int)launch_crmsa_region(x1, gamma, beta, phi, mean_rstd, logits, wdisp, rep, k, gd, (hipStream_t)stream);
}

int rrt_crmsa_region4_f32(const float* x1, const float* gamma, const float* beta, const float* phi, float* mean_rstd,
                          float* logits, float* wdisp, float* rep, int64_t L, int32_t dim, int32_t k, const rrt_grid* g8,
                          void* scratch, size_t scratch_bytes, void* stream) {
  if (!x1 || !gamma || !beta || !phi || !logits || !wdisp || !rep || !g8 || !scratch || L != g8->L) return RRT_E_INVALID;
  const GridDev gd = to_dev(*g8);
  if (!crmsa_region4_supported(dim, k, gd)) return unsupported("crmsa_region4: dim = 512, k <= 8, regions of 4..576 tokens");
  if (scratch_bytes < 256 + crmsa_region4_scratch_floats(gd, k) * sizeof(float)) return RRT_E_WORKSPACE;
  hipError_t e = hipMemsetAsync(scratch, 0, 256, (hipStream_t)stream);
  if (e != hipSuccess) return (int)e;
  return (int)launch_crmsa_region4(x1, gamma, beta, phi, mean_rstd, logits, wdisp, rep, nullptr, 0,
                                   (float*)((char*)scratch + 256), (int*)scratch, k, gd, (hipStream_t)stream);
}

int rrt_crmsa_stream4_f32(const float* x1, const float* gamma, const float* beta, const float* phi, float* mean_rstd,
                          float* logits, float* wdisp, float* rep, int64_t L, int32_t dim, int32_t k, const rrt_grid* g8,
                          void* scratch, size_t scratch_bytes, void* stream) {
  if (!x1 || !gamma || !beta || !phi || !logits || !wdisp || !rep || !g8 || !scratch || L != g8->L) return RRT_E_INVALID;
  const GridDev gd = to_dev(*g8);
  if (!crmsa_stream4_supported(dim, k, gd) || !crmsa_region4_supported(dim, k, gd))
    return unsupported("crmsa_stream4: dim = 512, k <= 8, regions of 16..576 tokens");
  if (scratch_bytes < 256 + crmsa_region4_scratch_floats(gd, k) * sizeof(float)) return RRT_E_WORKSPACE;
  hipError_t e = hipMemsetAsync(scratch, 0, 256, (hipStream_t)stream);
  if (e != hipSuccess) return (int)e;
  return (int)launch_crmsa_stream4(x1, gamma, beta, phi, mean_rstd, logits, wdisp, rep, nullptr, 0,
                                   (float*)((char*)scratch + 256), (int*)scratch, k, gd, (hipStream_t)stream);
}

int rrt_crmsa_dispatch_ln_f32(const float* x1, const float* x0, const float* wdisp,
                              const float* rep2, const float* gamma, const float* beta, float* y, int64_t L,
                              int32_t dim, int32_t k, const rrt_grid* g8, void* stream) {
  if (!x1 || !wdisp || !rep2 || !gamma || !beta || !y || !g8 || L != g8->L) return RRT_E_INVALID;
  if (k <= 0 || k > RRT_MAX_CRMSA_K || dim % 4 || dim > 2048) return unsupported("crmsa: k in [1,8], dim%4==0, dim<=2048");
  return (int)launch_crmsa_dispatch_ln(x1, x0, wdisp, rep2, gamma, beta, y, dim, k, to_dev(*g8),
                                       (hipStream_t)stream);
}

int rrt_crmsa_mlp_logits_f32(const float* hid, const float* w2, float* logits, int64_t rows, int32_t hdim,
                             int32_t k, void* stream) {
  if (!hid || !w2 || !logits || rows <= 0 || hdim <= 0) return RRT_E_INVALID;
  if (k <= 0 || k > RRT_MAX_CRMSA_K) return unsupported("crmsa: k in [1,8]");
  return (int)launch_crmsa_mlp_logits(hid, w2, logits, (int)rows, hdim, k, (hipStream_t)stream);
}

int rrt_layernorm_f32(const float* x1, const float* x0, const float* gamma, const float* beta, float* y,
                      int64_t L, int32_t dim, void* stream) {
  if (!x1 || !gamma || !beta || !y || L <= 0 || dim <= 0 || dim % 4) return RRT_E_INVALID;
  if (dim > 2048) return unsupported("dim > 2048");
  return (int)launch_layernorm(x1, x0, gamma, beta, y, (int)L, dim, (hipStream_t)stream);
}

}

namespace {

struct PoolWs {
  float *hid_a, *hid_b, *a_raw, *part;
  size_t bytes;
};
PoolWs carve_pool(int64_t N, int dim, int hidden, int gated, char* base) {
  PoolWs w{};
  size_t off = 0;
  auto take = [&](size_t nfloat) {
    float* p = base ? (float*)(base + off) : nullptr;
    off = align_up(off + nfloat * sizeof(float), 256);
    return p;
  };
  const size_t nb = (size_t)(N + POOL_CHUNK - 1) / POOL_CHUNK;
  w.hid_a = take((size_t)N * hidden);
  if (gated) w.hid_b = take((size_t)N * hidden);
  w.a_raw = take((size_t)N);
  w.part = take(nb * ((size_t)dim + 4));
  w.bytes = off;
  return w;
}

int check_pool(int64_t N, int dim, int hidden, int act, int n_classes) {
  if (N <= 0 || dim <= 0 || hidden <= 0 || n_classes <= 0) return RRT_E_INVALID;
  if (dim % 32) return unsupported("pool: dim must be a multiple of 32");
  if (hidden % 4) return unsupported("pool: hidden width must be a multiple of 4");
  if (act < RRT_ACT_NONE || act > RRT_ACT_TANH) return unsupported("pool: act must be none/relu/gelu/tanh");
  if (N > (int64_t)1000000) return unsupported("pool: bag larger than 1e6 tokens");
  return RRT_OK;
}

int pool_predict(const float* y, const float* a_w, const float* a_b, const float* b_w, const float* b_b,
                 const float* c_w, const float* c_b, const float* pred_w, const float* pred_b, float* pooled,
                 float* logits, float* attn, int no_norm, int64_t N, int dim, int hidden, int act,
                 int n_classes, int compute, const PoolWs& ws, hipStream_t st, const uint16_t* y16 = nullptr,
                 const uint16_t* a_w16 = nullptr, const uint16_t* b_w16 = nullptr) {
  hipError_t e;
  LinearEpilogue ep{};
  ep.prec = compute;
  ep.bias = a_b;
  ep.act = act;
  const bool p16 = y16 != nullptr && a_w16 != nullptr && (!b_w || b_w16 != nullptr) && dim % 64 == 0 &&
                   (compute == RRT_COMPUTE_BF16 || compute == RRT_COMPUTE_F16);
  e = p16 ? launch_linear16(y16, a_w16, ws.hid_a, (int)N, hidden, dim, ep, st)
          : launch_linear(y, a_w, ws.hid_a, (int)N, hidden, dim, ep, st);
  if (e != hipSuccess) return (int)e;
  if (b_w) {
    ep.bias = b_b;
    ep.act = RRT_ACT_SIGMOID;
    e = p16 ? launch_linear16(y16, b_w16, ws.hid_b, (int)N, hidden, dim, ep, st)
            : launch_linear(y, b_w, ws.hid_b, (int)N, hidden, dim, ep, st);
    if (e != hipSuccess) return (int)e;
  }
  e = launch_pool_partial(y, ws.hid_a, b_w ? ws.hid_b : nullptr, c_w, c_b, ws.a_raw, ws.part, (int)N, dim,
                          hidden, st);
  if (e != hipSuccess) return (int)e;
  e = launch_pool_merge(ws.part, ws.a_raw, pred_w, pred_b, pooled, logits, attn, no_norm, (int)N, dim,
                        n_classes, st);
  return (int)e;
}

int check_mil(const rrt_mil_desc* d, int64_t N) {
  if (!d) return RRT_E_INVALID;
  int rc = check_desc(&d->enc, N);
  if (rc) return rc;
  if (d->input_dim <= 0 || d->input_dim % 32) return unsupported("input_dim must be a positive multiple of 32");
  if (d->emb_act != RRT_ACT_NONE && d->emb_act != RRT_ACT_RELU && d->emb_act != RRT_ACT_GELU)
    return unsupported("emb_act must be none/relu/gelu");
  return check_pool(N, d->enc.dim, d->pool_hidden, d->pool_act, d->n_classes);
}

int check_branch_pool(int64_t N, int dim, int hidden, int K) {
  if (N <= 0 || dim <= 0 || hidden <= 0) return RRT_E_INVALID;
  if (K < 1 || K > 8) return unsupported("branch pool: 1 <= n_branches <= 8");
  if (dim % 32) return unsupported("branch pool: dim must be a multiple of 32");
  if (dim > 2048) return unsupported("branch pool: dim > 2048");
  if (hidden % 4) return unsupported("branch pool: hidden width must be a multiple of 4");
  if (N > (int64_t)1000000) return unsupported("branch pool: bag larger than 1e6 tokens");
  return RRT_OK;
}

size_t branch_pool_workspace(int64_t N, int dim, int hidden, int K) {
  const size_t fwd = align_up(branch_pool_part_floats((int)N, dim, K) * sizeof(float), 256);
  const size_t bwd = align_up(branch_pool_backward_part_floats((int)N, hidden, K) * sizeof(float), 256);
  return fwd > bwd ? fwd : bwd;
}

struct ClamWs {
  float *hid_a, *hid_b, *a_raw, *attn, *pooled, *part;
  size_t bytes;
};
ClamWs carve_clam(int64_t N, int dim, int hidden, int gated, int K, char* base) {
  ClamWs w{};
  size_t off = 0;
  auto take = [&](size_t nfloat) {
    float* p = base ? (float*)(base + off) : nullptr;
    off = align_up(off + nfloat * sizeof(float), 256);
    return p;
  };
  w.hid_a = take((size_t)N * hidden);
  if (gated) w.hid_b = take((size_t)N * hidden);
  w.a_raw = take((size_t)K * N);
  w.attn = take((size_t)K * N);
  w.pooled = take((size_t)K * dim);
  w.part = take(branch_pool_part_floats((int)N, dim, K));
  w.bytes = off;
  return w;
}

int check_clam(const rrt_clam_desc* d, int64_t N) {
  if (!d || N <= 0) return RRT_E_INVALID;
  if (d->has_rrt) {
    int rc = check_desc(&d->enc, N);
    if (rc) return rc;
  }
  if (d->input_dim <= 0 || d->input_dim % 32) return unsupported("input_dim must be a positive multiple of 32");
  if (d->emb_act != RRT_ACT_NONE && d->emb_act != RRT_ACT_RELU && d->emb_act != RRT_ACT_GELU)
    return unsupported("emb_act must be none/relu/gelu");
  if (d->enc.compute < 0 || d->enc.compute > RRT_COMPUTE_F32X3) return unsupported("compute must be RRT_COMPUTE_*");
  if (d->n_classes <= 0) return RRT_E_INVALID;
  if (d->per_branch && d->n_classes > 8) return unsupported("CLAM_MB: n_classes <= 8 (one attention branch per class)");
  return check_branch_pool(N, d->enc.dim, d->hidden, d->per_branch ? d->n_classes : 1);
}


int check_instance_max(int64_t N, int dim, int C) {
  if (N <= 0 || dim <= 0) return RRT_E_INVALID;
  if (C < 1 || C > 8) return unsupported("instance max: 1 <= n_classes <= 8");
  if (dim % 32) return unsupported("instance max: dim must be a multiple of 32");
  if (dim > 2048) return unsupported("instance max: dim > 2048");
  if (N > (int64_t)1000000) return unsupported("instance max: bag larger than 1e6 tokens");
  return RRT_OK;
}

// ... 1699 lines not shown
```

### rrt-mil_amd/csrc/crmsa.hip

```cpp
#include "internal.h"

namespace {

constexpr int KMAX = RRT_MAX_CRMSA_K;

template <int PREC>
__device__ __forceinline__ uint2 r4_pack4(float4 v) {
  if constexpr (PREC == 2) {
    typedef _Float16 h4 __attribute__((ext_vector_type(4)));
    h4 r; r[0] = (_Float16)v.x; r[1] = (_Float16)v.y; r[2] = (_Float16)v.z; r[3] = (_Float16)v.w;
    return __builtin_bit_cast(uint2, r);
  } else {
    typedef __bf16 b4 __attribute__((ext_vector_type(4)));
    b4 r; r[0] = (__bf16)v.x; r[1] = (__bf16)v.y; r[2] = (__bf16)v.z; r[3] = (__bf16)v.w;
    return __builtin_bit_cast(uint2, r);
  }
}


constexpr int RW = 2;
#ifndef RRT_RW_DISPATCH
#define RRT_RW_DISPATCH 1
#endif
constexpr int RW_DISPATCH = RRT_RW_DISPATCH;
// ... 1787 lines not shown
    const float* __restrict__ x1, const float* __restrict__ x0, const float* __restrict__ wdisp,
    const float* __restrict__ rep2, const float* __restrict__ gamma,
    const float* __restrict__ beta, float* __restrict__ y, int L, int dim, int k, GridDev g,
    uint16_t* __restrict__ y16, int prec16) {
  constexpr int RW = RW_DISPATCH;
  const int lane = threadIdx.x & 63;
  const int t0 = __builtin_amdgcn_readfirstlane((blockIdx.x * 4 + (threadIdx.x >> 6)) * RW);
  if (t0 >= L) return;
  const int R = g.Rt;
  float4 r[RW][NV];
#pragma unroll
  for (int i = 0; i < RW; ++i) {
    const int t = t0 + i < L ? t0 + i : L - 1;
#pragma unroll
    for (int v = 0; v < NV; ++v) {
      int c = (v * 64 + lane) * 4;
      r[i][v] = (FULL || c < dim) ? ld_row<NT_DISPATCH>(x1 + (size_t)t * dim + c) : make_float4(0.f, 0.f, 0.f, 0.f);
      if (x0 && (FULL || c < dim)) {
        float4 s = *(const float4*)(x0 + (size_t)t * dim + c);
        r[i][v].x += s.x; r[i][v].y += s.y; r[i][v].z += s.z; r[i][v].w += s.w;
      }
    }
  }
  float4 gm_pre[NV], bt_pre[NV];
  if constexpr (KB > 0) {
    if (gamma != nullptr) {
#pragma unroll
      for (int v = 0; v < NV; ++v) {
        const int c = (v * 64 + lane) * 4;
        gm_pre[v] = (FULL || c < dim) ? *(const float4*)(gamma + c) : make_float4(0.f, 0.f, 0.f, 0.f);
        bt_pre[v] = (FULL || c < dim) ? *(const float4*)(beta + c) : make_float4(0.f, 0.f, 0.f, 0.f);
      }
    }
  }
  if (CRMSA && KB > 0) {
    float w[RW][KB > 0 ? KB : 1];
    float4 q[RW][KB > 0 ? KB : 1][NV];
    int reg[RW];
#pragma unroll
    for (int i = 0; i < RW; ++i) {
      const int t = t0 + i < L ? t0 + i : L - 1;
      const int slot = token_to_slot(t, g);
      reg[i] = fdiv(slot, g.P, g.inv_P);
      const float* wd = wdisp + (size_t)slot * k;
#pragma unroll
      for (int n = 0; n < KB; ++n) w[i][n] = wd[n < k ? n : k - 1];
    }
#pragma unroll
    for (int i = 0; i < RW; ++i) {
      const bool fetch = i == 0 || reg[i] != reg[0];
#pragma unroll
      for (int n = 0; n < KB; ++n) {
        const int nn = n < k ? n : k - 1;
        const float* rp = rep2 + ((size_t)nn * R + reg[i]) * dim;
#pragma unroll
        for (int v = 0; v < NV; ++v) {
          const int c = (v * 64 + lane) * 4;
          if (fetch) q[i][n][v] = (FULL || c < dim) ? *(const float4*)(rp + c) : make_float4(0.f, 0.f, 0.f, 0.f);
          else q[i][n][v] = q[0][n][v];
        }
      }
    }
    __builtin_amdgcn_sched_barrier(0);
#pragma unroll
    for (int i = 0; i < RW; ++i)
#pragma unroll
      for (int n = 0; n < KB; ++n) {
        const float wn = n < k ? w[i][n] : 0.f;
#pragma unroll
        for (int v = 0; v < NV; ++v) {
          r[i][v].x += wn * q[i][n][v].x; r[i][v].y += wn * q[i][n][v].y; r[i][v].z += wn * q[i][n][v].z; r[i][v].w += wn * q[i][n][v].w;
        }
      }
  } else if (CRMSA) {
#pragma unroll
    for (int i = 0; i < RW; ++i) {
      const int t = t0 + i < L ? t0 + i : L - 1;
      const int slot = token_to_slot(t, g);
      const int reg = fdiv(slot, g.P, g.inv_P);
      const float* wd = wdisp + (size_t)slot * k;
#pragma unroll
      for (int n = 0; n < KMAX; ++n)
        if (n < k) {
          const float w = wd[n];
          const float* rp = rep2 + ((size_t)n * R + reg) * dim;
#pragma unroll
          for (int v = 0; v < NV; ++v) {
            int c = (v * 64 + lane) * 4;
            if (FULL || c < dim) {
              const float4 q = *(const float4*)(rp + c);
              r[i][v].x += w * q.x; r[i][v].y += w * q.y; r[i][v].z += w * q.z; r[i][v].w += w * q.w;
            }
          }
        }
    }
  }
  if (gamma == nullptr) {
#pragma unroll
    for (int i = 0; i < RW; ++i) {
      if (t0 + i >= L) break;
#pragma unroll
      for (int v = 0; v < NV; ++v) {
        int c = (v * 64 + lane) * 4;
        if (FULL || c < dim) *(float4*)(y + (size_t)(t0 + i) * dim + c) = r[i][v];
      }
    }
    return;
  }
  const float inv_d = 1.0f / (float)dim;
  float mean[RW], rstd[RW];
#pragma unroll
  for (int i = 0; i < RW; ++i) {
    float sum = 0.f;
#pragma unroll
    for (int v = 0; v < NV; ++v) sum += (r[i][v].x + r[i][v].y) + (r[i][v].z + r[i][v].w);
    mean[i] = wave_sum(sum) * inv_d;
  }
#pragma unroll
  for (int i = 0; i < RW; ++i) {
    float sq = 0.f;
#pragma unroll
    for (int v = 0; v < NV; ++v) {
      int c = (v * 64 + lane) * 4;
      if (FULL || c < dim) {
        float a = r[i][v].x - mean[i], b = r[i][v].y - mean[i], cc = r[i][v].z - mean[i], d = r[i][v].w - mean[i];
        sq += (a * a + b * b) + (cc * cc + d * d);
      }
    }
    rstd[i] = 1.0f / sqrtf(wave_sum(sq) * inv_d + LN_EPS);
  }
#pragma unroll
  for (int v = 0; v < NV; ++v) {
    int c = (v * 64 + lane) * 4;
    if (FULL || c < dim) {
      float4 gm, bt;
      if constexpr (KB > 0) { gm = gm_pre[v]; bt = bt_pre[v]; }
      else { gm = *(const float4*)(gamma + c); bt = *(const float4*)(beta + c); }
#pragma unroll
      for (int i = 0; i < RW; ++i)
        if (t0 + i < L) {
          float4 o;
          o.x = (r[i][v].x - mean[i]) * rstd[i] * gm.x + bt.x;
          o.y = (r[i][v].y - mean[i]) * rstd[i] * gm.y + bt.y;
          o.z = (r[i][v].z - mean[i]) * rstd[i] * gm.z + bt.z;
          o.w = (r[i][v].w - mean[i]) * rstd[i] * gm.w + bt.w;
          st_row<NT_DISPATCH>(y + (size_t)(t0 + i) * dim + c, o);
          if (y16 != nullptr)
            *(uint2*)(y16 + (size_t)(t0 + i) * dim + c) = prec16 == 2 ? r4_pack4<2>(o) : r4_pack4<1>(o);
        }
    }
  }
}

__global__ __launch_bounds__(256) void crmsa_mlp_logits_kernel(const float* __restrict__ hid,
                                                               const float* __restrict__ w2,
                                                               float* __restrict__ logits, int rows,
                                                               int hdim, int k) {
  const int lane = threadIdx.x & 63;
  const int row = blockIdx.x * 4 + (threadIdx.x >> 6);
  if (row >= rows) return;
  float acc[KMAX];
#pragma unroll
  for (int n = 0; n < KMAX; ++n) acc[n] = 0.f;
  for (int j = lane; j < hdim; j += 64) {
    const float t = tanhf(hid[(size_t)row * hdim + j]);
#pragma unroll
    for (int n = 0; n < KMAX; ++n)
      if (n < k) acc[n] += t * w2[(size_t)n * hdim + j];
  }
#pragma unroll
  for (int n = 0; n < KMAX; ++n)
    if (n < k) {
      const float a = wave_sum(acc[n]);
      if (lane == 0) logits[(size_t)row * k + n] = a;
    }
}

#ifdef RRT_NO_DISPATCH_KB5
constexpr bool DISPATCH_KB5 = false;
#else
constexpr bool DISPATCH_KB5 = true;
#endif
template <bool CRMSA>
hipError_t launch_dispatch(const float* x1, const float* x0, const float* wdisp,
                           const float* rep2, const float* gamma, const float* beta, float* y, int L,
                           int dim, int k, const GridDev& g, hipStream_t st, uint16_t* y16 = nullptr, int prec16 = 0) {
  dim3 grid((L + 4 * RW_DISPATCH - 1) / (4 * RW_DISPATCH)), block(256);
#define RRT_DISPATCH(NV)                                                                                         \
  do {                                                                                                           \
    if (RRT_ALLOW_FULL && dim == NV * 256) {                                                                     \
      if (NV <= 2 && CRMSA && k <= 3)                                                                            \
        crmsa_dispatch_ln_kernel<NV, CRMSA, true, (NV <= 2 ? 3 : 0)><<<grid, block, 0, st>>>(x1, x0, wdisp, rep2, gamma, beta, y, L, dim, k, g, y16, prec16); \
      else if (NV <= 2 && CRMSA && DISPATCH_KB5 && k <= 5)   \
        crmsa_dispatch_ln_kernel<NV, CRMSA, true, (NV <= 2 ? 5 : 0)><<<grid, block, 0, st>>>(x1, x0, wdisp, rep2, gamma, beta, y, L, dim, k, g, y16, prec16); \
      else if (NV <= 2 && CRMSA)                                                                                 \
        crmsa_dispatch_ln_kernel<NV, CRMSA, true, (NV <= 2 ? 8 : 0)><<<grid, block, 0, st>>>(x1, x0, wdisp, rep2, gamma, beta, y, L, dim, k, g, y16, prec16); \
      else                                                                                                       \
        crmsa_dispatch_ln_kernel<NV, CRMSA, true><<<grid, block, 0, st>>>(x1, x0, wdisp, rep2, gamma, beta, y, L, dim, k, g, y16, prec16);  \
    } else                                                                                                       \
      crmsa_dispatch_ln_kernel<NV, CRMSA, false><<<grid, block, 0, st>>>(x1, x0, wdisp, rep2, gamma, beta, y, L, dim, k, g, y16, prec16); \
  } while (0)
  if (dim <= 256) RRT_DISPATCH(1);
  else if (dim <= 512) RRT_DISPATCH(2);
  else if (dim <= 1024) RRT_DISPATCH(4);
  else RRT_DISPATCH(8);
#undef RRT_DISPATCH
  return hipGetLastError();
}

}

#ifdef RRT_TRACE
RRT_TRACE_DEFINE_READER(rrt_debug_trace_crmsa)
#endif

hipError_t launch_crmsa_logits(const float* x1, const float* gamma, const float* beta,
                               const float* phi, float* mean_rstd, float* logits, int dim, int k,
                               const GridDev& g8, hipStream_t st) {
  static const bool old_pair = rrt_tune_env("RRT_CRMSA_OLD_PAIR") != nullptr;
  if (dim == 512 && k >= 1 && k <= KMAX && !old_pair) {
    const dim3 grid2((g8.Np + 7) / 8);
    switch (k) {
#define RRT_LG512(K_) case K_: crmsa_logits512_kernel<K_><<<grid2, 256, 0, st>>>(x1, gamma, beta, phi, mean_rstd, logits, g8); break;
      RRT_LG512(1) RRT_LG512(2) RRT_LG512(3) RRT_LG512(4) RRT_LG512(5) RRT_LG512(6) RRT_LG512(7) RRT_LG512(8)
#undef RRT_LG512
    }
    return hipGetLastError();
  }
  const int ngroups = (g8.Np + 4 * RW - 1) / (4 * RW);
  dim3 grid(ngroups < 1024 ? ngroups : 1024), block(256);
  const size_t lds = (size_t)dim * k * sizeof(float);
#define RRT_LOGITS(NV) \
  do {                                                                                                      \
    if (RRT_ALLOW_FULL && dim == NV * 256) crmsa_logits_kernel<NV, true><<<grid, block, lds, st>>>(x1, gamma, beta, phi, mean_rstd, logits, dim, k, g8);  \
    else crmsa_logits_kernel<NV, false><<<grid, block, lds, st>>>(x1, gamma, beta, phi, mean_rstd, logits, dim, k, g8);               \
  } while (0)
  if (dim <= 256) RRT_LOGITS(1);
  else if (dim <= 512) RRT_LOGITS(2);
  else if (dim <= 1024) RRT_LOGITS(4);
  else RRT_LOGITS(8);
#undef RRT_LOGITS
  return hipGetLastError();
}

bool crmsa_region_supported(int dim, int k, const GridDev& g8) {
  return dim == 512 && k >= 1 && k <= REGION_KMAX && g8.P <= 16 * REGION_NR_MAX;
}
bool crmsa_region_enabled() {
  static const bool on = rrt_tune_env("RRT_CRMSA_REGION") != nullptr;
  return on;
}
template <int GK>
static hipError_t launch_region_gk(const float* x1, const float* gamma, const float* beta, const float* phi, float* mean_rstd,
                                   float* logits, float* wdisp, float* rep, uint16_t* rep16, int prec16, int k, const GridDev& g8,
                                   hipStream_t st) {
  const size_t lds = (size_t)(REGION_KMAX * 512 + REGION_NR_MAX * 16 * (2 * REGION_KMAX + 2)) * 4 +
                     (size_t)8 * REGION_KMAX * 128 * 16;
  auto kern = crmsa_region_kernel<GK>;
  static OncePerDevice once;
  if (once.first()) (void)hipFuncSetAttribute((const void*)kern, hipFuncAttributeMaxDynamicSharedMemorySize, (int)lds);
  kern<<<dim3(g8.rs * g8.rs), dim3(1024), lds, st>>>(x1, gamma, beta, phi, mean_rstd, logits, wdisp, rep, rep16, prec16, k, g8);
  return hipGetLastError();
}
hipError_t launch_crmsa_region(const float* x1, const float* gamma, const float* beta, const float* phi,
                               float* mean_rstd, float* logits, float* wdisp, float* rep, int k, const GridDev& g8,
                               hipStream_t st, uint16_t* rep16, int prec16) {
  static const bool no_gpr = rrt_tune_env("RRT_NO_REGION_GPR") != nullptr;
  const bool al16 = ((((uintptr_t)gamma | (uintptr_t)beta | (uintptr_t)phi) & 15) == 0);
  if (!no_gpr && al16) {
    if (k == 1) return launch_region_gk<1>(x1, gamma, beta, phi, mean_rstd, logits, wdisp, rep, rep16, prec16, k, g8, st);
    if (k == 2) return launch_region_gk<2>(x1, gamma, beta, phi, mean_rstd, logits, wdisp, rep, rep16, prec16, k, g8, st);
    if (k == 3) return launch_region_gk<3>(x1, gamma, beta, phi, mean_rstd, logits, wdisp, rep, rep16, prec16, k, g8, st);
  }
  return launch_region_gk<0>(x1, gamma, beta, phi, mean_rstd, logits, wdisp, rep, rep16, prec16, k, g8, st);
}

bool crmsa_region4_supported(int dim, int k, const GridDev& g8) {
  static const bool off = rrt_tune_env("RRT_NO_CRMSA_REGION4") != nullptr;
  return !off && dim == 512 && k >= 1 && k <= R4_KMAX && g8.P >= 4 && g8.P <= 36 * R4_NB_MAX;
}
size_t crmsa_region4_scratch_floats(const GridDev& g8, int k) {
  const int nb = g8.P > 288 ? 16 : 8;
  return (size_t)g8.rs * g8.rs * nb * (k <= 3 ? 3 : R4_KMAX) * (512 + 8);
}
template <int NB, int NW, int NR, int KM, bool GPR = false>
static hipError_t launch_region4_cfg(const float* x1, const float* gamma, const float* beta, const float* phi,
                                     float* mean_rstd, float* logits, float* wdisp, float* rep, uint16_t* rep16, int prec16,
                                     float* part_g, int* counters, int k, const GridDev& g8, hipStream_t st) {
  static_assert(NB <= R4_NB_MAX && NW >= KM && NW % 2 == 0 && KM <= R4_KMAX, "region4 shape");
  constexpr int PQM = NR * NW, KC = KM < 4 ? KM : 4;
  const size_t lds = (size_t)(KM * 512 + PQM * (2 * KM + 2)) * 4 + (size_t)(NW / 2) * KC * 128 * 16;
  auto kern = crmsa_region4_kernel<NB, NW, NR, KM, GPR>;
  static OncePerDevice once;
  if (lds > 64 * 1024 && once.first())
    (void)hipFuncSetAttribute((const void*)kern, hipFuncAttributeMaxDynamicSharedMemorySize, (int)lds);
  kern<<<dim3(g8.rs * g8.rs * NB), dim3(64 * NW), lds, st>>>(x1, gamma, beta, phi, mean_rstd, logits, wdisp, rep, rep16, prec16,
                                                             part_g, counters, k, g8);
  return hipGetLastError();
}
hipError_t launch_crmsa_region4(const float* x1, const float* gamma, const float* beta, const float* phi,
                                float* mean_rstd, float* logits, float* wdisp, float* rep, uint16_t* rep16, int prec16,
                                float* part_g, int* counters, int k, const GridDev& g8, hipStream_t st) {
#define RRT_R4(NB_, NW_, NR_)                                                                                          \
  return k <= 3 ? launch_region4_cfg<NB_, NW_, NR_, 3>(x1, gamma, beta, phi, mean_rstd, logits, wdisp, rep, rep16, prec16, \
                                                       part_g, counters, k, g8, st)                                   \
                : launch_region4_cfg<NB_, NW_, NR_, 8>(x1, gamma, beta, phi, mean_rstd, logits, wdisp, rep, rep16, prec16, \
                                                       part_g, counters, k, g8, st)
  static const int cfg = rrt_tune_env("RRT_REGION4_CFG") ? atoi(rrt_tune_env("RRT_REGION4_CFG")) : 4;
  static const bool r4_gpr = rrt_tune_env("RRT_NO_REGION4_GPR") == nullptr;
#ifdef RRT_TUNING
  if (cfg == 86 && g8.P <= 576) { RRT_R4(8, 12, 6); }
  if (cfg == 164 && g8.P <= 512) { RRT_R4(16, 8, 4); }
  if (cfg == 166 && g8.P <= 576) { RRT_R4(16, 12, 3); }
  if (cfg == 84 && g8.P <= 384) { RRT_R4(8, 12, 4); }
#endif
  if (g8.P > 288) { RRT_R4(16, 12, 3); }
  if (g8.P > 144) { RRT_R4(8, 12, 3); }
  if (cfg == 8 && g8.P > 96 && k <= 3)
    return launch_region4_cfg<8, 4, 5, 3>(x1, gamma, beta, phi, mean_rstd, logits, wdisp, rep, rep16, prec16, part_g, counters, k, g8, st);
  if (g8.P <= 144 && cfg == 4 && k > 3 && k <= 5 && !(k == 5 && r4_gpr))
    return launch_region4_cfg<4, 12, 3, 5>(x1, gamma, beta, phi, mean_rstd, logits, wdisp, rep, rep16, prec16, part_g, counters, k, g8, st);
  if (g8.P <= 144 && cfg == 4 && r4_gpr && ((((uintptr_t)gamma | (uintptr_t)beta | (uintptr_t)phi) & 15) == 0)) {
#define RRT_R4G(K_) if (k == K_) return launch_region4_cfg<4, 12, 3, K_, true>(x1, gamma, beta, phi, mean_rstd, logits, wdisp, rep, rep16, prec16, part_g, counters, k, g8, st)
    RRT_R4G(1); RRT_R4G(3); RRT_R4G(5);
#undef RRT_R4G
  }
  RRT_R4(4, 12, 3);
#undef RRT_R4
}

bool crmsa_stream4_supported(int dim, int k, const GridDev& g8) {
  static const bool off = rrt_tune_env("RRT_NO_CRMSA_STREAM4") != nullptr;
  return !off && dim == 512 && k >= 1 && k <= R4_KMAX && g8.P >= 16 && g8.P <= 4 * S4_PQMAX;
}
template <int NW, int NR, int KM>
static hipError_t launch_stream4_cfg(const float* x1, const float* gamma, const float* beta, const float* phi,
                                     float* mean_rstd, float* logits, float* wdisp, float* rep, uint16_t* rep16, int prec16,
                                     float* part_g, int* counters, const GridDev& g8, hipStream_t st) {
  static_assert(NW >= KM && NW % 2 == 0 && KM <= R4_KMAX, "stream4 shape");
  constexpr int KC = KM < 4 ? KM : 4;
  const size_t lds = (size_t)(KM * NW * 8 + S4_PQMAX * (KM + 2)) * 4 + (size_t)(NW / 2) * KC * 128 * 16;
  auto kern = crmsa_stream4_kernel<NW, NR, KM>;
  static OncePerDevice once;
  if (lds > 64 * 1024 && once.first())
    (void)hipFuncSetAttribute((const void*)kern, hipFuncAttributeMaxDynamicSharedMemorySize, (int)lds);
  kern<<<dim3(g8.rs * g8.rs * 4), dim3(64 * NW), lds, st>>>(x1, gamma, beta, phi, mean_rstd, logits, wdisp, rep, rep16, prec16,
                                                            part_g, counters, g8);
  return hipGetLastError();
}
hipError_t launch_crmsa_stream4(const float* x1, const float* gamma, const float* beta, const float* phi,
                                float* mean_rstd, float* logits, float* wdisp, float* rep, uint16_t* rep16, int prec16,
                                float* part_g, int* counters, int k, const GridDev& g8, hipStream_t st) {
  if (!crmsa_stream4_supported(512, k, g8)) return hipErrorInvalidValue;
#define RRT_S4(NW_, NR_, KM_) case KM_: return launch_stream4_cfg<NW_, NR_, KM_>(x1, gamma, beta, phi, mean_rstd, logits, wdisp, rep, \
                                                                                rep16, prec16, part_g, counters, g8, st)
  switch (k) {
    RRT_S4(12, 3, 1); RRT_S4(12, 3, 2); RRT_S4(12, 3, 3); RRT_S4(8, 3, 4); RRT_S4(8, 3, 5); RRT_S4(8, 3, 6); RRT_S4(8, 2, 7); RRT_S4(8, 2, 8);
  }
#undef RRT_S4
  return hipErrorInvalidValue;
}

hipError_t launch_crmsa_combine(const float* x1, const float* gamma, const float* beta,
                                const float* mean_rstd, const float* logits, float* wdisp,
                                float* rep, uint16_t* rep16, int prec16, int dim, int k, const GridDev& g8, hipStream_t st) {
  dim3 grid(g8.rs * g8.rs, (dim + 63) / 64), block(256);
  const size_t lds = ((size_t)g8.P * KMAX + ((g8.P + 3) & ~3)) * 4 + (size_t)16 * KMAX * 16 * sizeof(float4);
  if (lds > 150 * 1024) return hipErrorInvalidValue;
  const bool vnorm = mean_rstd == nullptr;
  static const bool old_pair = rrt_tune_env("RRT_CRMSA_OLD_PAIR") != nullptr;
  if (!vnorm && dim == 512 && k >= 1 && k <= KMAX && !old_pair) {
    const size_t lds2 = (((size_t)g8.P * k + 3) & ~(size_t)3) * 4 + (size_t)((g8.P + 1) & ~1) * 8 + (size_t)16 * k * 16 * sizeof(float4);
    if (lds2 <= 64 * 1024) {
      switch (k) {
#define RRT_CB512(K_) case K_: crmsa_combine512_kernel<K_><<<grid, block, lds2, st>>>(x1, gamma, beta, mean_rstd, logits, wdisp, rep, rep16, prec16, g8); break;
        RRT_CB512(1) RRT_CB512(2) RRT_CB512(3) RRT_CB512(4) RRT_CB512(5) RRT_CB512(6) RRT_CB512(7) RRT_CB512(8)
#undef RRT_CB512
      }
      return hipGetLastError();
    }
  }
  auto kern = vnorm ? crmsa_combine_kernel<true> : crmsa_combine_kernel<false>;
  if (lds > 64 * 1024)
    (void)hipFuncSetAttribute((const void*)kern, hipFuncAttributeMaxDynamicSharedMemorySize, (int)lds);
  kern<<<grid, block, lds, st>>>(x1, gamma, beta, mean_rstd, logits, wdisp, rep, rep16, prec16, dim, k, g8);
  return hipGetLastError();
}

static size_t combine_parts_lds(int P, int KM) {
  return (size_t)P * KM * 4 * 2 + (size_t)((P + 1) & ~1) * 8 + (size_t)16 * (KM + 1) * 16 * 16;
}
bool crmsa_combine_parts_supported(int dim, int k, const GridDev& g8) {
  static const bool off = rrt_tune_env("RRT_NO_CRMSA_PARTS") != nullptr;
  return !off && dim % 64 == 0 && dim >= 64 && dim <= 512 && k >= 1 && k <= KMAX && combine_parts_lds(g8.P, k <= 4 ? 4 : 8) <= 150 * 1024;
}
size_t crmsa_parts_floats(long n_tokens, int dim, int k) { return (size_t)n_tokens * (dim / 64) * ((2 + k + 3) & ~3); }
hipError_t launch_crmsa_combine_parts(const float* x1, const float* part, const float* gamma, const float* beta,
                                      const float* phi, float* wdisp, float* rep, uint16_t* rep16, int prec16, int dim,
                                      int k, const GridDev& g8, hipStream_t st) {
  if (!crmsa_combine_parts_supported(dim, k, g8)) return hipErrorInvalidValue;
  dim3 grid(g8.rs * g8.rs, dim / 64), block(256);
  constexpr int TR = 9;
  static const bool no_coal = rrt_tune_env("RRT_NO_CPARTS_COAL") != nullptr;
  const bool coal = !no_coal && k >= 3 && k <= 4 && dim == 512 && g8.P <= 16 * TR && (((uintptr_t)part) & 15) == 0;
  const int al16 = ((((uintptr_t)gamma | (uintptr_t)beta | (uintptr_t)phi) & 15) == 0 ? 1 : 0) | (coal ? 2 : 0);
#define RRT_CPARTS(KM_)                                                                                              \
  do {                                                                                                               \
    const size_t lds = combine_parts_lds(g8.P, KM_) + (coal ? (size_t)16 * TR * 17 * 16 : 0);                        \
    const bool ck = coal && KM_ == 4;                                                                                \
    auto kern = ck ? crmsa_combine_parts_kernel<TR, KM_, true> : crmsa_combine_parts_kernel<TR, KM_, false>;         \
    static OncePerDevice once_coal, once_plain;       \
    if (lds > 64 * 1024 && (ck ? once_coal : once_plain).first())                                                    \
      (void)hipFuncSetAttribute((const void*)kern, hipFuncAttributeMaxDynamicSharedMemorySize, 150 * 1024);          \
    kern<<<grid, block, lds, st>>>(x1, part, gamma, beta, phi, wdisp, rep, rep16, prec16, dim, k, dim / 64, al16, g8); \
  } while (0)
  if (k <= 4) RRT_CPARTS(4);
  else RRT_CPARTS(8);
#undef RRT_CPARTS
  return hipGetLastError();
}

hipError_t launch_crmsa_mlp_logits(const float* hid, const float* w2, float* logits, int rows, int hdim,
                                   int k, hipStream_t st) {
  crmsa_mlp_logits_kernel<<<dim3((rows + 3) / 4), 256, 0, st>>>(hid, w2, logits, rows, hdim, k);
  return hipGetLastError();
}

hipError_t launch_crmsa_dispatch_ln(const float* x1, const float* x0, const float* wdisp,
                                    const float* rep2, const float* gamma,
                                    const float* beta, float* y, int dim, int k, const GridDev& g8,
                                    hipStream_t st, uint16_t* y16, int prec16) {
  if (y16 != nullptr && (gamma == nullptr || (prec16 != 1 && prec16 != 2) || dim % 4 != 0)) return hipErrorInvalidValue;
  return launch_dispatch<true>(x1, x0, wdisp, rep2, gamma, beta, y, g8.L, dim, k, g8, st, y16, prec16);
}

hipError_t launch_layernorm(const float* x1, const float* x0, const float* gamma,
                            const float* beta, float* y, int L, int dim, hipStream_t st) {
  GridDev g{};
  g.L = L;
  g.H = g.s = g.rs = g.P = 1;
  return launch_dispatch<false>(x1, x0, nullptr, nullptr, gamma, beta, y, L, dim, 0, g, st);
}
```

### rrt-mil_amd/csrc/internal.h

```cpp
#pragma once
#include <hip/hip_runtime.h>
#include "common.h"
#include "../../include/rrt_hip.h"

GridDev to_dev(const rrt_grid& g);

#ifdef RRT_TUNING
#include <stdlib.h>
inline const char* rrt_tune_env(const char* name) { return getenv(name); }
#else
inline const char* rrt_tune_env(const char*) { return nullptr; }
#endif

struct OncePerDevice {
  bool seen[64] = {};
  bool first() {
    int d = 0;
    (void)hipGetDevice(&d);
    d &= 63;
    if (seen[d]) return false;
    seen[d] = true;
    return true;
  }
};

hipError_t launch_ln_partition(const float* x, const float* gamma, const float* beta, float* u,
                               int dim, const GridDev& g, hipStream_t st, int* zero = nullptr, int n_zero = 0);

struct LinearEpilogue {
  int prec;
  const float* bias;
  int q_cols;
  float q_scale;
  int act;
  unsigned drop_thresh, drop_seed;
  float drop_scale;
  bool drop_on;
  const float* resid;
  GridDev g;
  int* zero64;
  bool solo;
};
hipError_t launch_linear(const float* A, const float* B, float* C, int M, int N, int K,
                         const LinearEpilogue& ep, hipStream_t st);

constexpr int CAST16_MAX_JOBS = 2 * RRT_MAX_RMSA_LAYERS + 2;
struct Cast16Jobs {
  const float* src[CAST16_MAX_JOBS];
  uint16_t* dst[CAST16_MAX_JOBS];
  size_t n4[CAST16_MAX_JOBS];
  int count;
};
hipError_t launch_cast16(const Cast16Jobs& jobs, int prec, hipStream_t st);
hipError_t launch_ln_partition16(const float* x, const float* gamma, const float* beta, uint16_t* u, int dim,
                                 const GridDev& g, int prec, hipStream_t st, int* zero = nullptr, int n_zero = 0);
hipError_t launch_cast_split(const Cast16Jobs& jobs, hipStream_t st);
hipError_t launch_ln_partition_split(const float* x, const float* gamma, const float* beta, void* u, int dim,
                                     const GridDev& g, hipStream_t st);
hipError_t launch_linear_split(const void* Asplit, const void* Bsplit, float* C, int M, int N, int K,
                               const LinearEpilogue& ep, hipStream_t st);
bool rmsa_pair16_supported(int n_regions, int P, int D, int heads, int epeg_k);
hipError_t launch_rmsa_pair16(const uint16_t* U, const uint16_t* W, const float* bqkv, const float* pe_w, uint16_t* O,
                              int n_regions, int P, int D, int heads, int epeg_k, int prec, hipStream_t st);
struct PairProj {
  const uint16_t* Wp;
  const float* bias;
  const float* resid;
  float* out;
  int* cnt;
  int* zero64;
  int lag;
  int n_items;
  GridDev g;
  int* err;
  int spin_limit;
  int wait_for;
};
bool rmsa_pair16_proj_supported(int n_regions, int P, int D, int heads, int epeg_k);
hipError_t launch_rmsa_pair16_proj(const uint16_t* U, const uint16_t* W, const float* bqkv, const float* pe_w, uint16_t* O,
                                   int n_regions, int P, int D, int heads, int epeg_k, int prec, const PairProj& proj,
                                   hipStream_t st);
bool rmsa_fused_x3_supported(int P, int D, int heads, int epeg_k);
hipError_t launch_rmsa_fused_x3(const void* Usplit, const void* Wsplit, const float* bqkv, const float* pe_w,
                                void* Osplit, int n_regions, int P, int D, int heads, int epeg_k, hipStream_t st);
hipError_t launch_linear16(const void* A16, const void* B16, float* C, int M, int N, int K, const LinearEpilogue& ep,
                           hipStream_t st);
bool rmsa_fused16_supported(int P, int D, int heads, int epeg_k);
hipError_t launch_rmsa_fused16(const uint16_t* U16, const uint16_t* Wqkv16, const float* bqkv, const float* pe_w,
                               uint16_t* O16, int n_regions, int P, int D, int heads, int epeg_k, int prec,
                               hipStream_t st);

hipError_t launch_region_attention(const float* qkv, const float* pe_w, float* o, int n_regions,
                                   int P, int dim, int heads, int epeg_k, hipStream_t st);
bool region_attention_hd_supported(int P, int dim, int heads, int epeg_k);
hipError_t launch_region_attention_hd(const float* qkv, const float* pe_w, float* o, int n_regions, int P, int dim,
                                      int heads, int epeg_k, hipStream_t st);

bool rmsa_fused_supported(int P, int D, int heads, int epeg_k);
bool rmsa_fused_supported_rows(long n_rows, int D);
struct FusedProj {
  const float* Wp;
  const float* bias;
  const float* resid;
  float* out;
  int* cnt;
  int* zero64;
  int lag;
  int n_items;
  GridDev g;
  int* err;
  int spin_limit;
  int wait_for;
  float* part;
  const float* ln_g;
  const float* phi;
  int k;
  int n_slabs;
};
int* handover_err_device();
int handover_err_peek(bool clear);
bool rmsa_fused_proj_supported(int n_regions, int P, int D, int heads, int epeg_k, int prec);
hipError_t launch_rmsa_fused(const float* U, const float* Wqkv, const float* bqkv, const float* pe_w,
                             float* O, int n_regions, int P, int D, int heads, int epeg_k, int prec,
                             hipStream_t st, float* stash = nullptr,
                             const FusedProj* proj = nullptr);

size_t attn_scoremap_lds(int P, int k);
size_t attn_scoremap_scratch_floats(int n_regions, int P, int heads, int k, int maps);
hipError_t launch_attn_scoremap(const float* qkv, const float* pe_w, float* o, float* smap, int n_regions, int P, int dim,
                                int heads, int k, hipStream_t st);
hipError_t launch_value_pe(const float* qkv, const float* w, const float* bias, float* pe, int n_regions, int P, int s,
                           int dim, int heads, int k, int two_d, hipStream_t st);
hipError_t launch_add_cols(float* dst, const float* src, size_t rows, int dim, int ld, hipStream_t st);
hipError_t launch_value_pe_backward(const float* dpe, const float* qkv, const float* vsub, const float* w, float* dqkv, float* dw,
                                    float* db, int n_regions, int P, int s, int dim, int heads, int k, int two_d,
                                    hipStream_t st);
hipError_t launch_copy_cols(float* dst, const float* src, size_t rows, int dim, int ld, int off, hipStream_t st);
hipError_t launch_sub(float* dst, const float* a, const float* b, size_t n, hipStream_t st);
hipError_t launch_small_k_matmul(const float* A, const float* W, float* Cm, int M, int N, int Kd, hipStream_t st);
hipError_t launch_attn_scoremap_backward(const float* qkv, const float* pe_w, const float* dO, float* dqkv, float* dpe_w,
                                         float* scratch, int n_regions, int P, int dim, int heads, int k, hipStream_t st);

hipError_t launch_crmsa_logits(const float* x1, const float* gamma, const float* beta,
                               const float* phi, float* mean_rstd, float* logits, int dim, int k,
                               const GridDev& g8, hipStream_t st);
bool crmsa_region_supported(int dim, int k, const GridDev& g8);
bool crmsa_region_enabled();
bool crmsa_region4_supported(int dim, int k, const GridDev& g8);
size_t crmsa_region4_scratch_floats(const GridDev& g8, int k);
hipError_t launch_crmsa_region4(const float* x1, const float* gamma, const float* beta, const float* phi,
                                float* mean_rstd, float* logits, float* wdisp, float* rep, uint16_t* rep16, int prec16,
                                float* part_g, int* counters, int k, const GridDev& g8, hipStream_t st);
hipError_t launch_crmsa_region(const float* x1, const float* gamma, const float* beta, const float* phi,
                               float* mean_rstd, float* logits, float* wdisp, float* rep, int k, const GridDev& g8,
                               hipStream_t st, uint16_t* rep16 = nullptr, int prec16 = 0);
bool crmsa_stream4_supported(int dim, int k, const GridDev& g8);
hipError_t launch_crmsa_stream4(const float* x1, const float* gamma, const float* beta, const float* phi,
                                float* mean_rstd, float* logits, float* wdisp, float* rep, uint16_t* rep16, int prec16,
                                float* part_g, int* counters, int k, const GridDev& g8, hipStream_t st);
hipError_t launch_crmsa_combine(const float* x1, const float* gamma, const float* beta,
                                const float* mean_rstd, const float* logits, float* wdisp,
                                float* rep, uint16_t* rep16, int prec16, int dim, int k, const GridDev& g8, hipStream_t st);
bool crmsa_combine_parts_supported(int dim, int k, const GridDev& g8);
size_t crmsa_parts_floats(long n_tokens, int dim, int k);
hipError_t launch_crmsa_combine_parts(const float* x1, const float* part, const float* gamma, const float* beta,
                                      const float* phi, float* wdisp, float* rep, uint16_t* rep16, int prec16, int dim,
                                      int k, const GridDev& g8, hipStream_t st);
hipError_t launch_crmsa_mlp_logits(const float* hid, const float* w2, float* logits, int rows, int hdim,
                                   int k, hipStream_t st);
hipError_t launch_crmsa_dispatch_ln(const float* x1, const float* x0, const float* wdisp,
                                    const float* rep2, const float* gamma,
                                    const float* beta, float* y, int dim, int k, const GridDev& g8,
                                    hipStream_t st, uint16_t* y16 = nullptr, int prec16 = 0);
hipError_t launch_layernorm(const float* x1, const float* x0, const float* gamma,
                            const float* beta, float* y, int L, int dim, hipStream_t st);

constexpr int POOL_CHUNK = 32;
hipError_t launch_pool_partial(const float* y, const float* hid_a, const float* hid_b, const float* wc,
                               const float* bc, float* a_raw, float* part, int N, int dim, int hid,
                               hipStream_t st);
hipError_t launch_pool_merge(const float* part, const float* a_raw, const float* pred_w, const float* pred_b,
                             float* pooled, float* logits, float* attn, int no_norm, int N, int dim,
                             int n_classes, hipStream_t st);

size_t pool_backward_part_floats(int N, int hid);
hipError_t launch_pool_backward(const float* y, const float* hid_a, const float* hid_b, const float* wc, const float* attn,
                                const float* pooled, const float* d_pooled, const float* d_attn, const float* d_raw,
                                const float* c_ext, float* dy, float* dhid_a, float* dhid_b, float* dwcb, float* part, int N,
                                int dim, int hid, hipStream_t st);

size_t branch_pool_part_floats(int N, int dim, int K);
size_t branch_pool_backward_part_floats(int N, int hid, int K);
size_t branch_pool_merge_lds(int N, int dim);
size_t branch_pool_backward_lds(int dim, int hid, int K);
hipError_t launch_branch_pool(const float* y, const float* hid_a, const float* hid_b, const float* wc, const float* bc,
                              const float* cls_w, const float* cls_b, float* pooled, float* logits, float* attn, float* a_raw,
                              float* part, int per_branch, int n_classes, int N, int dim, int hid, int K, hipStream_t st);
hipError_t launch_branch_pool_backward(const float* y, const float* hid_a, const float* hid_b, const float* wc, const float* attn,
                                       const float* pooled, const float* d_pooled, const float* d_raw, float* dy, float* dhid_a,
                                       float* dhid_b, float* dwcb, float* part, int N, int dim, int hid, int K, hipStream_t st);
hipError_t launch_topk_rows(const float* x, long long* out, int rows, int N, int k, hipStream_t st);

constexpr int IMAX_CHUNK = 128;
constexpr int DS_CHUNK = 32;
size_t instance_max_part_records(int N);
size_t dsmil_pool_part_floats(int N, int dim, int K);
size_t dsmil_pool_merge_lds(int N, int dim);
hipError_t launch_instance_max(const float* y, const float* w, const float* b, float* classes, float* cmax, long long* argmax,
                               float* pv, int* pi, int N, int dim, int K, hipStream_t st);
hipError_t launch_dsmil_pool(const float* feats, const long long* argmax, const float* q_w, const float* q_b, const float* fcc_w,
                             const float* fcc_b, float* logits, float* A, float* B, float* raw, float* v, float* vb, float* lpart,
                             float* part, int N, int dim, int Q, int K, hipStream_t st);

size_t linear_bwd_workspace(int M, int N, int K);
hipError_t launch_linear_backward(const float* dY, const float* X, const float* W, float* dX, float* dW, float* db,
                                  int M, int N, int K, int prec, void* ws, hipStream_t st, const float* WT_ready = nullptr);
hipError_t launch_transpose(const float* in, float* out, int R, int C, hipStream_t st);
constexpr int TRANSPOSE_MAX_JOBS = 2 * RRT_MAX_RMSA_LAYERS + 2;
struct TransposeJobs {
  const float* in[TRANSPOSE_MAX_JOBS];
  float* out[TRANSPOSE_MAX_JOBS];
  int R[TRANSPOSE_MAX_JOBS], C[TRANSPOSE_MAX_JOBS], blk0[TRANSPOSE_MAX_JOBS];
  int n;
};
hipError_t launch_transpose_batch(TransposeJobs& jobs, hipStream_t st);
hipError_t launch_reduce_partials(const float* part, float* out, int S, size_t n, hipStream_t st);
constexpr int REDUCE_MAX_JOBS = 16;
struct ReduceJobs {
  const float* part[REDUCE_MAX_JOBS];
  float* out[REDUCE_MAX_JOBS];
  float* out_tr[REDUCE_MAX_JOBS];
  unsigned long long n[REDUCE_MAX_JOBS], split[REDUCE_MAX_JOBS];
  int S[REDUCE_MAX_JOBS], tr_dim[REDUCE_MAX_JOBS], tr_k[REDUCE_MAX_JOBS];
  unsigned blk0[REDUCE_MAX_JOBS + 1];
  int count;
};
hipError_t reduce_or_defer(ReduceJobs* defer, const float* part, float* out, int S, size_t n, hipStream_t st,
                           size_t split = 0, float* out_tr = nullptr, int tr_dim = 0, int tr_k = 0);
hipError_t launch_reduce_jobs(ReduceJobs& jobs, hipStream_t st);
hipError_t launch_reduce_partials_scatter(const float* part, float* out, int S, size_t n, size_t split, float* out_tr,
                                          int tr_dim, int tr_k, hipStream_t st);
hipError_t launch_gemm_tn(const float* dY, const float* X, float* dW, float* scratch, int M, int N, int K,
                          hipStream_t st);
hipError_t launch_colsum(const float* Y, float* out, float* scratch, int M, int N, hipStream_t st);
size_t ln_bwd_workspace(int dim);
hipError_t launch_ln_backward(const float* dy, const float* x, const float* gamma, const float* add, float* dx,
                              float* dgb, float* part, int L, int dim, const GridDev* g, hipStream_t st,
                              ReduceJobs* defer = nullptr);
bool attn_bwd_supported(int P, int D, int heads, int epeg_k);
size_t attn_bwd_workspace(int n_regions, int P, int D, int heads, int epeg_k);
hipError_t launch_attention_backward(const float* qkv, const float* pe_w, const float* O, const float* dO,
                                     float* dqkv, float* dpe, float* dpe_part, int n_regions, int P, int D,
                                     int heads, int epeg_k, hipStream_t st, ReduceJobs* defer = nullptr,
                                     float* defer_part = nullptr);
hipError_t launch_partition_rows(const float* src, float* dst, int dim, const GridDev& g, unsigned drop_thresh,
                                 unsigned drop_seed, float drop_scale, hipStream_t st);
hipError_t launch_apply_drop_mask(float* buf, int rows, int cols, unsigned drop_thresh, unsigned drop_seed,
                                  float drop_scale, hipStream_t st);
hipError_t launch_crmsa_tokdot(const float* x, const float* mean_rstd, const float* gamma, const float* beta,
                               const float* vec, float* out, int dim, int k, const GridDev& g, hipStream_t st);
hipError_t launch_crmsa_wsum(const float* X, const float* W, float* out, int dim, int k, const GridDev& g,
                             hipStream_t st);
hipError_t launch_crmsa_bwd_region(const float* lg, const float* dC, const float* dWd, float* dlg, float* Cw, int k,
                                   const GridDev& g, hipStream_t st);
size_t crmsa_bwd_dx_workspace(int dim, int k);
hipError_t launch_crmsa_bwd_dx(const float* x1, const float* dx2, const float* mean_rstd, const float* gamma,
                               const float* beta, const float* phi, const float* Cw, const float* dlg,
                               const float* drep, float* dx1, float* out_rows, float* part, int dim, int k,
                               const GridDev& g, bool mlp, hipStream_t st, float* dphi_t = nullptr,
                               ReduceJobs* defer = nullptr);
hipError_t launch_crmsa_mlp_bwd_hidden(const float* hid, const float* dlg, const float* w2, float* th, float* dhid,
                                       size_t rows, int hdim, int k, hipStream_t st);
hipError_t launch_act_forward(const float* hpre, float* h, size_t n, int act, unsigned thresh, unsigned seed,
                              float scale, hipStream_t st);
hipError_t launch_act_backward(float* dh, const float* hpre, size_t n, int act, unsigned thresh, unsigned seed,
                               float scale, hipStream_t st);
hipError_t launch_copy_drop_mask(const float* src, float* dst, size_t n, unsigned drop_thresh, unsigned drop_seed,
                                 float drop_scale, hipStream_t st);
hipError_t launch_peg(const float* x, const float* const* w, const float* const* b, float* y, int N, int C, int k,
                      int conv_1d, int ppeg, hipStream_t st);
size_t peg_bwd_workspace(int N, int C, int k, int ppeg);
hipError_t launch_peg_backward(const float* x, const float* dy, const float* const* w, float* dx, float* const* dw,
                               float* const* db, int N, int C, int k, int conv_1d, int ppeg, void* ws, hipStream_t st);

void nystrom_chunks(long np, int* nsub, int* sub_per_chunk, int* nch);
size_t nystrom_lattn_floats(long np, int heads);
size_t nystrom_pinv_floats(int heads);
hipError_t launch_nystrom_landmarks(const float* qkv, float* ql, float* kl, long np, int heads, hipStream_t st);
hipError_t launch_nystrom_sim2(const float* ql, const float* kl, float* a2, int heads, hipStream_t st);
hipError_t launch_nystrom_lattn(const float* qkv, const float* ql, float* av, float* ws, long np, int heads, hipStream_t st);
hipError_t launch_nystrom_pinv(const float* a2, float* z, float* ws, int heads, int iters, hipStream_t st);
hipError_t launch_nystrom_zav(const float* z, const float* av, float* wz, int heads, hipStream_t st);
hipError_t launch_nystrom_output(const float* qkv, const float* kl, const float* wz, const float* conv_w, float* o, long np,
                                 int heads, int ks, hipStream_t st);
hipError_t launch_transmil_assemble(const float* h, const float* cls, float* seq, int N, int rows, int dim, hipStream_t st);
hipError_t launch_transmil_head(const float* x, const float* w, const float* b, float* logits, int dim, int n_classes,
                                hipStream_t st);
hipError_t launch_ppeg_side(const float* x, const float* const* w, const float* const* b, float* y, int side, int C,
                            hipStream_t st);
```

### rrt-mil_amd/csrc/ln_partition.hip

```cpp
#include "internal.h"

template <int NV, bool FULL>
__global__ __launch_bounds__(256) void ln_partition_kernel(const float* __restrict__ x,
                                                           const float* __restrict__ gamma,
                                                           const float* __restrict__ beta,
                                                           float* __restrict__ u, int dim, GridDev g,
                                                           int* __restrict__ zero, int n_zero) {
  if (zero != nullptr && blockIdx.x == 0)
    for (int i = threadIdx.x; i < n_zero; i += 256) zero[i] = 0;
  const int lane = threadIdx.x & 63;
  const int t = blockIdx.x * 4 + (threadIdx.x >> 6);
  if (t >= g.Np) return;
  float* dst = u + (size_t)token_to_slot(t, g) * dim;
  if (t >= g.L) {
#pragma unroll
    for (int v = 0; v < NV; ++v) {
      int c = (v * 64 + lane) * 4;
      if (FULL || c < dim) *(float4*)(dst + c) = make_float4(0.f, 0.f, 0.f, 0.f);
    }
    return;
  }
  const float* src = x + (size_t)t * dim;
  float4 r[NV];
  float sum = 0.f;
#pragma unroll
  for (int v = 0; v < NV; ++v) {
    int c = (v * 64 + lane) * 4;
    r[v] = (FULL || c < dim) ? ld_row<NT_LN1>(src + c) : make_float4(0.f, 0.f, 0.f, 0.f);
    sum += (r[v].x + r[v].y) + (r[v].z + r[v].w);
  }
  const float inv_d = 1.0f / (float)dim;
  const float mean = wave_sum(sum) * inv_d;
  float sq = 0.f;
#pragma unroll
  for (int v = 0; v < NV; ++v) {
    int c = (v * 64 + lane) * 4;
    if (FULL || c < dim) {
      float a = r[v].x - mean, b = r[v].y - mean, cc = r[v].z - mean, d = r[v].w - mean;
      sq += (a * a + b * b) + (cc * cc + d * d);
    }
  }
  const float rstd = 1.0f / sqrtf(wave_sum(sq) * inv_d + LN_EPS);
#pragma unroll
  for (int v = 0; v < NV; ++v) {
    int c = (v * 64 + lane) * 4;
    if (FULL || c < dim) {
      float4 gm = *(const float4*)(gamma + c), bt = *(const float4*)(beta + c);
      float4 o;
      o.x = (r[v].x - mean) * rstd * gm.x + bt.x;
      o.y = (r[v].y - mean) * rstd * gm.y + bt.y;
      o.z = (r[v].z - mean) * rstd * gm.z + bt.z;
      o.w = (r[v].w - mean) * rstd * gm.w + bt.w;
      *(float4*)(dst + c) = o;
    }
  }
}

hipError_t launch_ln_partition(const float* x, const float* gamma, const float* beta, float* u,
                               int dim, const GridDev& g, hipStream_t st, int* zero, int n_zero) {
  dim3 grid((g.Np + 3) / 4), block(256);
#define RRT_LNP(NV)                                                                              \
  do {                                                                                         \
    if (RRT_ALLOW_FULL && dim == NV * 256) ln_partition_kernel<NV, true><<<grid, block, 0, st>>>(x, gamma, beta, u, dim, g, zero, n_zero);  \
    else ln_partition_kernel<NV, false><<<grid, block, 0, st>>>(x, gamma, beta, u, dim, g, zero, n_zero);                 \
  } while (0)
  if (dim <= 256) RRT_LNP(1);
  else if (dim <= 512) RRT_LNP(2);
  else if (dim <= 1024) RRT_LNP(4);
  else RRT_LNP(8);
#undef RRT_LNP
  return hipGetLastError();
}
```

Before: 5373.

## Add persistent row-looping LayerNorm kernels with software-pipelined row prefetch

Adds persistent variants of the LN-partition and CR-MSA dispatch/LayerNorm kernels. Each launches a grid capped at CU count times rows_w (default 1), and every wave loops over rows, loading the next row while it reduces and writes the current one. Gamma and beta are hoisted into registers once per wave. The aim is to cut block launch overhead and hide memory latency in these bandwidth-bound row kernels, at the cost of lower occupancy, which may leave the memory system with too few requests in flight.

```diff
diff --git a/include/rrt_hip.h b/include/rrt_hip.h
--- a/include/rrt_hip.h
+++ b/include/rrt_hip.h
@@ -97,10 +97,15 @@
 #define RRT_PLAN_CRMSA_PARTS 16
 #define RRT_PLAN_ATTN_HD    32
 int rrt_encoder_plan(const rrt_encoder_desc *desc, int64_t n_tokens, int32_t *flags);
+int rrt_encoder_plan_rows(const rrt_encoder_desc *desc, int64_t n_tokens, int32_t *w);
 
 int rrt_encoder_forward_f32(const rrt_encoder_desc *desc, const rrt_encoder_weights *w,
                             const float *x, float *y, int64_t n_tokens,
                             void *workspace, size_t workspace_bytes, void *stream);
+
+int rrt_debug_encoder_forward_rows_f32(const rrt_encoder_desc *desc, const rrt_encoder_weights *w,
+                                       const float *x, float *y, int64_t n_tokens,
+                                       void *workspace, size_t workspace_bytes, void *stream, int32_t rows_w);
 
 enum {
   RRT_EV_START = 0,
@@ -134,6 +139,10 @@
 
 int rrt_ln_partition_f32(const float *x, const float *gamma, const float *beta, float *u,
                          int64_t L, int32_t dim, const rrt_grid *g, void *stream);
+
+int rrt_ln_partition_rows_f32(const float *x, const float *gamma, const float *beta, float *u,
+                              int64_t L, int32_t dim, const rrt_grid *g, int32_t w,
+                              int32_t *zero, int32_t n_zero, void *stream);
 
 int rrt_linear_f32(const float *A, const float *B, const float *bias, float *C,
                    int64_t M, int32_t N, int32_t K, int32_t q_cols, float q_scale,
@@ -216,6 +225,10 @@
                               const float *rep2, const float *gamma,
                               const float *beta, float *y, int64_t L, int32_t dim, int32_t k,
                               const rrt_grid *g8, void *stream);
+int rrt_crmsa_dispatch_ln_rows_f32(const float *x1, const float *x0, const float *wdisp,
+                                   const float *rep2, const float *gamma,
+                                   const float *beta, float *y, int64_t L, int32_t dim, int32_t k,
+                                   const rrt_grid *g8, int32_t w, uint16_t *y16, int32_t prec16, void *stream);
 int rrt_crmsa_mlp_logits_f32(const float *hid, const float *w2, float *logits, int64_t rows,
                              int32_t hdim, int32_t k, void *stream);
 int rrt_layernorm_f32(const float *x1, const float *x0, const float *gamma, const float *beta,
diff --git a/rrt-mil_amd/_lib.py b/rrt-mil_amd/_lib.py
--- a/rrt-mil_amd/_lib.py
+++ b/rrt-mil_amd/_lib.py
@@ -121,8 +121,11 @@
     "rrt_region_grid": (C.c_int, [C.c_int64, C.c_int32, C.c_int32, C.c_int32, C.c_float, C.POINTER(Grid)]),
     "rrt_encoder_workspace_size": (C.c_int, [C.POINTER(EncoderDesc), C.c_int64, C.POINTER(C.c_size_t)]),
     "rrt_encoder_plan": (C.c_int, [C.POINTER(EncoderDesc), C.c_int64, C.POINTER(C.c_int32)]),
+    "rrt_encoder_plan_rows": (C.c_int, [C.POINTER(EncoderDesc), C.c_int64, C.POINTER(C.c_int32)]),
     "rrt_encoder_forward_f32": (C.c_int, [C.POINTER(EncoderDesc), C.POINTER(EncoderWeights), C.c_void_p,
                                           C.c_void_p, C.c_int64, C.c_void_p, C.c_size_t, C.c_void_p]),
+    "rrt_debug_encoder_forward_rows_f32": (C.c_int, [C.POINTER(EncoderDesc), C.POINTER(EncoderWeights), C.c_void_p,
+                                                     C.c_void_p, C.c_int64, C.c_void_p, C.c_size_t, C.c_void_p, C.c_int32]),
     "rrt_encoder_forward_events_f32": (C.c_int, [C.POINTER(EncoderDesc), C.POINTER(EncoderWeights), C.c_void_p,
                                                  C.c_void_p, C.c_int64, C.c_void_p, C.c_size_t, C.c_void_p,
                                                  C.POINTER(C.c_void_p)]),
@@ -136,6 +139,8 @@
                                                 C.c_void_p, C.POINTER(C.c_void_p)]),
     "rrt_ln_partition_f32": (C.c_int, [C.c_void_p, C.c_void_p, C.c_void_p, C.c_void_p, C.c_int64,
                                        C.c_int32, C.POINTER(Grid), C.c_void_p]),
+    "rrt_ln_partition_rows_f32": (C.c_int, [C.c_void_p, C.c_void_p, C.c_void_p, C.c_void_p, C.c_int64,
+                                            C.c_int32, C.POINTER(Grid), C.c_int32, C.c_void_p, C.c_int32, C.c_void_p]),
     "rrt_linear_f32": (C.c_int, [C.c_void_p, C.c_void_p, C.c_void_p, C.c_void_p, C.c_int64, C.c_int32,
                                  C.c_int32, C.c_int32, C.c_float, C.c_int32, C.c_void_p]),
     "rrt_linear_unpartition_residual_f32": (C.c_int, [C.c_void_p, C.c_void_p, C.c_void_p, C.c_void_p,
@@ -175,6 +180,8 @@
                                                          C.c_size_t, C.c_void_p]),
     "rrt_crmsa_dispatch_ln_f32": (C.c_int, [C.c_void_p] * 7 + [C.c_int64, C.c_int32, C.c_int32,
                                                               C.POINTER(Grid), C.c_void_p]),
+    "rrt_crmsa_dispatch_ln_rows_f32": (C.c_int, [C.c_void_p] * 7 + [C.c_int64, C.c_int32, C.c_int32,
+                                                                   C.POINTER(Grid), C.c_int32, C.c_void_p, C.c_int32, C.c_void_p]),
     "rrt_crmsa_mlp_logits_f32": (C.c_int, [C.c_void_p] * 3 + [C.c_int64, C.c_int32, C.c_int32, C.c_void_p]),
     "rrt_layernorm_f32": (C.c_int, [C.c_void_p] * 5 + [C.c_int64, C.c_int32, C.c_void_p]),
     "rrt_peg_f32": (C.c_int, [C.c_void_p] * 4 + [C.c_int64] + [C.c_int32] * 4 + [C.c_void_p]),
diff --git a/rrt-mil_amd/csrc/api.hip b/rrt-mil_amd/csrc/api.hip
--- a/rrt-mil_amd/csrc/api.hip
+++ b/rrt-mil_amd/csrc/api.hip
@@ -206,7 +206,11 @@
   CastKind casts;
   bool inner16;
   FrontKind front;
+  int rows_w;
+  bool rows_ln1;
 };
+
+constexpr int ROWS_W_DEFAULT = 1;
 
 #ifndef RRT_STREAM4_MIN_P
 #define RRT_STREAM4_MIN_P 145
@@ -221,6 +225,18 @@
   const bool lowp = compute != RRT_COMPUTE_F32 && D % 64 == 0;
   const GridDev gd8 = to_dev(g8);
   p.inner16 = d.cr_msa && lowp && rmsa_fused16_supported(64, D, d.crmsa_heads, 0);
+  {
+    static const char* rows_env = rrt_tune_env("RRT_ROWS_W");
+    static const bool rows_lowp = rrt_tune_env("RRT_ROWS_LOWP") != nullptr;
+    int w = ROWS_W_DEFAULT;
+    if (rows_env != nullptr && atoi(rows_env) >= 0 && atoi(rows_env) <= ROWS_W_MAX) w = atoi(rows_env);
+    const bool exact = d.compute == RRT_COMPUTE_F32;
+    const bool fits = D <= 512 && (!d.cr_msa || d.crmsa_k <= 3);
+    if (!d.solo && fits && (exact || (rows_lowp && lowp))) {
+      p.rows_w = w;
+      p.rows_ln1 = exact && w > 0;
+    }
+  }
   if (d.n_rmsa_layers > 0) {
     const GridDev gd = to_dev(g);
     const int R = gd.rs * gd.rs, heads = d.n_heads, ek = d.epeg ? d.epeg_k : 0;
@@ -359,6 +375,16 @@
   return RRT_OK;
 }
 
+int rrt_encoder_plan_rows(const rrt_encoder_desc* desc, int64_t n_tokens, int32_t* w) {
+  if (!w) return RRT_E_INVALID;
+  *w = 0;
+  rrt_grid g{}, g8{};
+  int rc = resolve_grids(desc, n_tokens, &g, &g8);
+  if (rc) return rc;
+  *w = plan_encoder(*desc, g, g8, false).rows_w;
+  return RRT_OK;
+}
+
 struct rrt_phase_gate {
   hipEvent_t done;
   bool armed;
@@ -381,7 +407,7 @@
 static int encoder_forward(const rrt_encoder_desc* desc_in, const rrt_encoder_weights* w, const float* x,
                            float* y, int64_t n_tokens, void* workspace, size_t workspace_bytes,
                            void* stream, void** events, rrt_phase_gate* gate = nullptr, float* rmsa_out = nullptr,
-                           uint16_t* y16 = nullptr, bool* y16_done = nullptr) {
+                           uint16_t* y16 = nullptr, bool* y16_done = nullptr, int rows_w_forced = -1) {
   if (y16_done) *y16_done = false;
   if (!desc_in || !w || !x || !y || x == y) return RRT_E_INVALID;
   int rc = check_desc(desc_in, n_tokens);
@@ -399,7 +425,11 @@
   Workspace ws = carve(*desc, N, g, g8, nullptr);
   if (!workspace || workspace_bytes < ws.bytes) return RRT_E_WORKSPACE;
   ws = carve(*desc, N, g, g8, (char*)workspace);
-  const EncoderPlan plan = plan_encoder(*desc_in, g, g8, rmsa_out != nullptr);
+  EncoderPlan plan = plan_encoder(*desc_in, g, g8, rmsa_out != nullptr);
+  if (rows_w_forced >= 0) {
+    plan.rows_w = rows_w_forced;
+    plan.rows_ln1 = rows_w_forced > 0 && desc_in->compute == RRT_COMPUTE_F32;
+  }
 
   auto mark = [&](int i) -> hipError_t {
     return (events && events[i]) ? hipEventRecord((hipEvent_t)events[i], st) : hipSuccess;
@@ -527,7 +557,7 @@
         break;
       }
       case LayerKind::FusedProj: {
-        RRT_TRY(launch_ln_partition(xin, lw.norm_w, lw.norm_b, ws.uo, D, gd, st, ws.proj_cnt, R));
+        RRT_TRY(launch_ln_partition(xin, lw.norm_w, lw.norm_b, ws.uo, D, gd, st, ws.proj_cnt, R, plan.rows_ln1 ? plan.rows_w : 0));
         RRT_TRY(core_begin(marks));
         FusedProj pj{};
         pj.Wp = lw.proj_w;
@@ -549,7 +579,7 @@
         break;
       }
       case LayerKind::Fused: {
-        RRT_TRY(launch_ln_partition(xin, lw.norm_w, lw.norm_b, ws.uo, D, gd, st));
+        RRT_TRY(launch_ln_partition(xin, lw.norm_w, lw.norm_b, ws.uo, D, gd, st, nullptr, 0, plan.rows_ln1 ? plan.rows_w : 0));
         RRT_TRY(core_begin(marks));
         RRT_TRY(launch_rmsa_fused(ws.uo, lw.qkv_w, lw.qkv_b, pe_w, ws.qkv, R, gd.P, D, desc->n_heads, ek, desc->compute, st));
         RRT_TRY(core_end(marks, !gate_proj));
@@ -558,7 +588,7 @@
         break;
       }
       case LayerKind::Unfused: {
-        RRT_TRY(launch_ln_partition(xin, lw.norm_w, lw.norm_b, ws.uo, D, gd, st));
+        RRT_TRY(launch_ln_partition(xin, lw.norm_w, lw.norm_b, ws.uo, D, gd, st, nullptr, 0, plan.rows_ln1 ? plan.rows_w : 0));
         RRT_TRY(core_begin(marks));
         RRT_TRY(launch_linear(ws.uo, lw.qkv_w, ws.qkv, gd.Np, 3 * D, D, qkv_epilogue(lw.qkv_b, D, desc->n_heads, desc->compute), st));
         if (marks) RRT_TRY(mark(RRT_EV_QKV));
@@ -600,7 +630,7 @@
   const float* x0 = desc->all_shortcut ? x : nullptr;
   if (!w->norm_w || !w->norm_b) return RRT_E_INVALID;
   if (!desc->cr_msa) {
-    RRT_TRY(launch_layernorm(xin, x0, w->norm_w, w->norm_b, y, (int)N, D, st));
+    RRT_TRY(launch_layernorm(xin, x0, w->norm_w, w->norm_b, y, (int)N, D, st, plan.rows_w));
     RRT_TRY(mark(RRT_EV_END));
     return RRT_OK;
   }
@@ -670,16 +700,16 @@
   }
   RRT_TRY(mark(RRT_EV_CR_INNER));
   if (desc->ffn) {
-    RRT_TRY(launch_crmsa_dispatch_ln(xin, nullptr, ws.wdisp, ws.rep2, nullptr, nullptr, ws.xa, D, k, gd8, st));
+    RRT_TRY(launch_crmsa_dispatch_ln(xin, nullptr, ws.wdisp, ws.rep2, nullptr, nullptr, ws.xa, D, k, gd8, st, nullptr, 0, plan.rows_w));
     rc = ffn_block(cw, ws.xa, ws.xb);
     if (rc) return rc;
-    RRT_TRY(launch_layernorm(ws.xb, x0, w->norm_w, w->norm_b, y, (int)N, D, st));
+    RRT_TRY(launch_layernorm(ws.xb, x0, w->norm_w, w->norm_b, y, (int)N, D, st, plan.rows_w));
     RRT_TRY(mark(RRT_EV_END));
     return RRT_OK;
   }
   const bool want16 = y16 != nullptr && (desc->compute == RRT_COMPUTE_BF16 || desc->compute == RRT_COMPUTE_F16) && D % 4 == 0;
   RRT_TRY(launch_crmsa_dispatch_ln(xin, x0, ws.wdisp, ws.rep2, w->norm_w, w->norm_b, y, D, k,
-                                   gd8, st, want16 ? y16 : nullptr, want16 ? desc->compute : 0));
+                                   gd8, st, want16 ? y16 : nullptr, want16 ? desc->compute : 0, plan.rows_w));
   if (want16 && y16_done) *y16_done = true;
   RRT_TRY(mark(RRT_EV_END));
   return RRT_OK;
@@ -689,6 +719,13 @@
                             float* y, int64_t n_tokens, void* workspace, size_t workspace_bytes,
                             void* stream) {
   return encoder_forward(desc, w, x, y, n_tokens, workspace, workspace_bytes, stream, nullptr);
+}
+
+int rrt_debug_encoder_forward_rows_f32(const rrt_encoder_desc* desc, const rrt_encoder_weights* w, const float* x, float* y,
+                                       int64_t n_tokens, void* workspace, size_t workspace_bytes, void* stream, int32_t rows_w) {
+  if (rows_w < 0 || rows_w > ROWS_W_MAX) return RRT_E_INVALID;
+  return encoder_forward(desc, w, x, y, n_tokens, workspace, workspace_bytes, stream, nullptr, nullptr, nullptr, nullptr, nullptr,
+                         rows_w);
 }
 
 int rrt_phase_gate_create(rrt_phase_gate** out) {
@@ -853,6 +890,14 @@
   if (!x || !gamma || !beta || !u || !g || L != g->L || dim <= 0 || dim % 4) return RRT_E_INVALID;
   if (dim > 2048) return unsupported("dim > 2048");
   return (int)launch_ln_partition(x, gamma, beta, u, dim, to_dev(*g), (hipStream_t)stream);
+}
+
+int rrt_ln_partition_rows_f32(const float* x, const float* gamma, const float* beta, float* u, int64_t L,
+                              int32_t dim, const rrt_grid* g, int32_t w, int32_t* zero, int32_t n_zero, void* stream) {
+  if (!x || !gamma || !beta || !u || !g || L != g->L || dim <= 0 || dim % 4) return RRT_E_INVALID;
+  if (w < 0 || w > ROWS_W_MAX || n_zero < 0 || (n_zero > 0 && !zero)) return RRT_E_INVALID;
+  if (dim > 2048) return unsupported("dim > 2048");
+  return (int)launch_ln_partition(x, gamma, beta, u, dim, to_dev(*g), (hipStream_t)stream, n_zero > 0 ? zero : nullptr, n_zero, w);
 }
 
 int rrt_linear_f32(const float* A, const float* B, const float* bias, float* C, int64_t M, int32_t N,
@@ -1159,6 +1204,22 @@
   if (k <= 0 || k > RRT_MAX_CRMSA_K || dim % 4 || dim > 2048) return unsupported("crmsa: k in [1,8], dim%4==0, dim<=2048");
   return (int)launch_crmsa_dispatch_ln(x1, x0, wdisp, rep2, gamma, beta, y, dim, k, to_dev(*g8),
                                        (hipStream_t)stream);
+}
+
+int rrt_crmsa_dispatch_ln_rows_f32(const float* x1, const float* x0, const float* wdisp, const float* rep2, const float* gamma,
+                                   const float* beta, float* y, int64_t L, int32_t dim, int32_t k, const rrt_grid* g8, int32_t w,
+                                   uint16_t* y16, int32_t prec16, void* stream) {
+  if (!x1 || !gamma || !beta || !y || L <= 0 || L > INT32_MAX || dim <= 0 || w < 0 || w > ROWS_W_MAX) return RRT_E_INVALID;
+  if (dim % 4 || dim > 2048) return unsupported("dim % 4 == 0, dim <= 2048");
+  if (y16 != nullptr && prec16 != RRT_COMPUTE_BF16 && prec16 != RRT_COMPUTE_F16) return RRT_E_INVALID;
+  if (k == 0) {
+    if (wdisp || rep2 || y16) return RRT_E_INVALID;
+    return (int)launch_layernorm(x1, x0, gamma, beta, y, (int)L, dim, (hipStream_t)stream, w);
+  }
+  if (!wdisp || !rep2 || !g8 || L != g8->L) return RRT_E_INVALID;
+  if (k < 0 || k > RRT_MAX_CRMSA_K) return unsupported("crmsa: k in [1,8]");
+  return (int)launch_crmsa_dispatch_ln(x1, x0, wdisp, rep2, gamma, beta, y, dim, k, to_dev(*g8), (hipStream_t)stream, y16,
+                                       y16 ? prec16 : 0, w);
 }
 
 int rrt_crmsa_mlp_logits_f32(const float* hid, const float* w2, float* logits, int64_t rows, int32_t hdim,
diff --git a/rrt-mil_amd/csrc/crmsa.hip b/rrt-mil_amd/csrc/crmsa.hip
--- a/rrt-mil_amd/csrc/crmsa.hip
+++ b/rrt-mil_amd/csrc/crmsa.hip
@@ -1963,6 +1963,193 @@
   }
 }
 
+
+template <typename T>
+__device__ __forceinline__ T* rows_base(T* p) {
+  asm volatile("" : "+s"(p));
+  return p;
+}
+typedef __attribute__((address_space(1))) f32x4 rows_gvec;
+typedef unsigned rows_u32x2 __attribute__((ext_vector_type(2)));
+typedef __attribute__((address_space(1))) rows_u32x2 rows_gu2;
+template <bool NT> __device__ __forceinline__ float4 rows_ld(const float* p) {
+  const rows_gvec* gp = (const rows_gvec*)p;
+  f32x4 v;
+  if constexpr (NT) v = __builtin_nontemporal_load(gp); else v = *gp;
+  return make_float4(v.x, v.y, v.z, v.w);
+}
+template <bool NT> __device__ __forceinline__ void rows_st(float* p, const float4 v) {
+  const f32x4 w = {v.x, v.y, v.z, v.w};
+  rows_gvec* gp = (rows_gvec*)p;
+  if constexpr (NT) __builtin_nontemporal_store(w, gp); else *gp = w;
+}
+template <int NV, bool FULL>
+__device__ __forceinline__ void dispatch_rows_request(const float* __restrict__ x1, int t, int dim, int lane, float4 (&r)[NV]) {
+  const float* src = rows_base(x1) + (size_t)t * dim;
+#pragma unroll
+  for (int v = 0; v < NV; ++v) {
+    int c = (v * 64 + lane) * 4;
+    r[v] = (FULL || c < dim) ? rows_ld<NT_DISPATCH>(src + c) : make_float4(0.f, 0.f, 0.f, 0.f);
+  }
+}
+
+template <int NV, bool CRMSA, bool FULL, int KB>
+__device__ __forceinline__ void dispatch_rows_token(float4 (&r)[NV], float4 (&r_next)[NV], int t_next,
+                                                    const float4 (&gm)[NV], const float4 (&bt)[NV], int t,
+                                                    const float* __restrict__ x1, const float* __restrict__ x0,
+                                                    const float* __restrict__ wdisp, const float* __restrict__ rep2, const float* gamma, float* __restrict__ y,
+                                                    int dim, int k, int lane, float inv_d, const GridDev& g,
+                                                    uint16_t* __restrict__ y16, int prec16) {
+  constexpr int KQ = KB > 0 ? KB : 1;
+  const int R = g.Rt;
+  {
+    float4 s[NV];
+#pragma unroll
+    for (int v = 0; v < NV; ++v) s[v] = make_float4(0.f, 0.f, 0.f, 0.f);
+    if (x0) {
+      const float* sp = rows_base(x0) + (size_t)t * dim;
+#pragma unroll
+      for (int v = 0; v < NV; ++v) {
+        int c = (v * 64 + lane) * 4;
+        if (FULL || c < dim) s[v] = rows_ld<false>(sp + c);
+      }
+    }
+    float w[KQ];
+    float4 q[KQ][NV];
+    if constexpr (CRMSA && KB > 0) {
+      const int slot = __builtin_amdgcn_readfirstlane(token_to_slot(t, g));
+      const int reg = __builtin_amdgcn_readfirstlane(fdiv(slot, g.P, g.inv_P));
+      const float* wd = wdisp + (size_t)slot * k;
+      const float* const rep2u = rows_base(rep2);
+#pragma unroll
+      for (int n = 0; n < KB; ++n) w[n] = wd[n < k ? n : k - 1];
+#pragma unroll
+      for (int n = 0; n < KB; ++n) {
+        const int nn = n < k ? n : k - 1;
+        const float* rp = rep2u + ((size_t)nn * R + reg) * dim;
+#pragma unroll
+        for (int v = 0; v < NV; ++v) {
+          const int c = (v * 64 + lane) * 4;
+          q[n][v] = (FULL || c < dim) ? rows_ld<false>(rp + c) : make_float4(0.f, 0.f, 0.f, 0.f);
+        }
+      }
+    }
+    dispatch_rows_request<NV, FULL>(x1, t_next, dim, lane, r_next);
+    asm volatile("" ::: "memory");
+    __builtin_amdgcn_sched_barrier(0);
+    if (x0) {
+#pragma unroll
+      for (int v = 0; v < NV; ++v) {
+        int c = (v * 64 + lane) * 4;
+        if (FULL || c < dim) { r[v].x += s[v].x; r[v].y += s[v].y; r[v].z += s[v].z; r[v].w += s[v].w; }
+      }
+    }
+    if constexpr (CRMSA && KB > 0) {
+#pragma unroll
+      for (int n = 0; n < KB; ++n) {
+        const float wv = n < k ? w[n] : 0.f;
+#pragma unroll
+        for (int v = 0; v < NV; ++v) {
+          r[v].x += wv * q[n][v].x; r[v].y += wv * q[n][v].y; r[v].z += wv * q[n][v].z; r[v].w += wv * q[n][v].w;
+        }
+      }
+    } else if constexpr (CRMSA) {
+      const int slot = token_to_slot(t, g);
+      const int rg = fdiv(slot, g.P, g.inv_P);
+      const float* wd = wdisp + (size_t)slot * k;
+#pragma unroll
+      for (int n = 0; n < KMAX; ++n)
+        if (n < k) {
+          const float wv = wd[n];
+          const float* rp = rep2 + ((size_t)n * R + rg) * dim;
+#pragma unroll
+          for (int v = 0; v < NV; ++v) {
+            int c = (v * 64 + lane) * 4;
+            if (FULL || c < dim) {
+              const float4 qq = *(const float4*)(rp + c);
+              r[v].x += wv * qq.x; r[v].y += wv * qq.y; r[v].z += wv * qq.z; r[v].w += wv * qq.w;
+            }
+          }
+        }
+    }
+    float* const yr = rows_base(y) + (size_t)t * dim;
+    uint16_t* const yr16 = rows_base(y16) + (size_t)t * dim;
+    if (gamma == nullptr) {
+#pragma unroll
+      for (int v = 0; v < NV; ++v) {
+        int c = (v * 64 + lane) * 4;
+        if (FULL || c < dim) rows_st<false>(yr + c, r[v]);
+      }
+    } else {
+      float sum = 0.f;
+#pragma unroll
+      for (int v = 0; v < NV; ++v) sum += (r[v].x + r[v].y) + (r[v].z + r[v].w);
+      const float mean = wave_sum(sum) * inv_d;
+      float sq = 0.f;
+#pragma unroll
+      for (int v = 0; v < NV; ++v) {
+        int c = (v * 64 + lane) * 4;
+        if (FULL || c < dim) {
+          float a = r[v].x - mean, b = r[v].y - mean, cc = r[v].z - mean, d = r[v].w - mean;
+          sq += (a * a + b * b) + (cc * cc + d * d);
+        }
+      }
+      const float rstd = 1.0f / sqrtf(wave_sum(sq) * inv_d + LN_EPS);
+#pragma unroll
+      for (int v = 0; v < NV; ++v) {
+        int c = (v * 64 + lane) * 4;
+        if (FULL || c < dim) {
+          float4 o;
+          o.x = (r[v].x - mean) * rstd * gm[v].x + bt[v].x;
+          o.y = (r[v].y - mean) * rstd * gm[v].y + bt[v].y;
+          o.z = (r[v].z - mean) * rstd * gm[v].z + bt[v].z;
+          o.w = (r[v].w - mean) * rstd * gm[v].w + bt[v].w;
+          rows_st<NT_DISPATCH>(yr + c, o);
+          if (y16 != nullptr)
+          {
+            const uint2 h = prec16 == 2 ? r4_pack4<2>(o) : r4_pack4<1>(o);
+            const rows_u32x2 hv = {h.x, h.y};
+            *(rows_gu2*)(yr16 + c) = hv;
+          }
+        }
+      }
+    }
+  }
+}
+
+template <int NV, bool CRMSA, bool FULL, int KB = 0>
+__global__ __launch_bounds__(256) void crmsa_dispatch_ln_rows_kernel(
+    const float* __restrict__ x1, const float* __restrict__ x0, const float* __restrict__ wdisp,
+    const float* __restrict__ rep2, const float* __restrict__ gamma,
+    const float* __restrict__ beta, float* __restrict__ y, int L, int dim, int k, GridDev g,
+    uint16_t* __restrict__ y16, int prec16) {
+  const int lane = threadIdx.x & 63;
+  const int W = gridDim.x * 4;
+  int t = __builtin_amdgcn_readfirstlane(blockIdx.x * 4 + (threadIdx.x >> 6));
+  if (t >= L) return;
+  const int last = L - 1;
+  float4 gm[NV], bt[NV];
+#pragma unroll
+  for (int v = 0; v < NV; ++v) {
+    const int c = (v * 64 + lane) * 4;
+    gm[v] = (gamma != nullptr && (FULL || c < dim)) ? *(const float4*)(gamma + c) : make_float4(0.f, 0.f, 0.f, 0.f);
+    bt[v] = (gamma != nullptr && (FULL || c < dim)) ? *(const float4*)(beta + c) : make_float4(0.f, 0.f, 0.f, 0.f);
+  }
+  const float inv_d = 1.0f / (float)dim;
+  float4 ra[NV], rb[NV];
+  dispatch_rows_request<NV, FULL>(x1, t, dim, lane, ra);
+  for (;;) {
+    const int tn = t + W;
+    dispatch_rows_token<NV, CRMSA, FULL, KB>(ra, rb, tn < L ? tn : last, gm, bt, t, x1, x0, wdisp, rep2, gamma, y, dim, k, lane,
+                                             inv_d, g, y16, prec16);
+    if (tn >= L) break;
+    t = tn + W;
+    dispatch_rows_token<NV, CRMSA, FULL, KB>(rb, ra, t < L ? t : last, gm, bt, tn, x1, x0, wdisp, rep2, gamma, y, dim, k, lane,
+                                             inv_d, g, y16, prec16);
+    if (t >= L) break;
+  }
+}
+
 __global__ __launch_bounds__(256) void crmsa_mlp_logits_kernel(const float* __restrict__ hid,
                                                                const float* __restrict__ w2,
                                                                float* __restrict__ logits, int rows,
@@ -1995,7 +2182,33 @@
 template <bool CRMSA>
 hipError_t launch_dispatch(const float* x1, const float* x0, const float* wdisp,
                            const float* rep2, const float* gamma, const float* beta, float* y, int L,
-                           int dim, int k, const GridDev& g, hipStream_t st, uint16_t* y16 = nullptr, int prec16 = 0) {
+                           int dim, int k, const GridDev& g, hipStream_t st, uint16_t* y16 = nullptr, int prec16 = 0,
+                           int rows_w = 0) {
+  if (rows_w > 0) {
+    if (rows_w > ROWS_W_MAX) return hipErrorInvalidValue;
+    const int row_blocks = (L + 3) / 4, fixed = device_cu_count() * rows_w;
+    dim3 grid(row_blocks < fixed ? row_blocks : fixed), block(256);
+#define RRT_DISPATCH_ROWS(NV)                                                                                    \
+  do {                                                                                                           \
+    if (RRT_ALLOW_FULL && dim == NV * 256) {                                                                     \
+      if (NV <= 2 && CRMSA && k <= 3)                                                                            \
+        crmsa_dispatch_ln_rows_kernel<NV, CRMSA, true, (NV <= 2 ? 3 : 0)><<<grid, block, 0, st>>>(x1, x0, wdisp, rep2, gamma, beta, y, L, dim, k, g, y16, prec16); \
+      else if (NV <= 2 && CRMSA && DISPATCH_KB5 && k <= 5)                                                       \
+        crmsa_dispatch_ln_rows_kernel<NV, CRMSA, true, (NV <= 2 ? 5 : 0)><<<grid, block, 0, st>>>(x1, x0, wdisp, rep2, gamma, beta, y, L, dim, k, g, y16, prec16); \
+      else if (NV <= 2 && CRMSA)                                                                                 \
+        crmsa_dispatch_ln_rows_kernel<NV, CRMSA, true, (NV <= 2 ? 8 : 0)><<<grid, block, 0, st>>>(x1, x0, wdisp, rep2, gamma, beta, y, L, dim, k, g, y16, prec16); \
+      else                                                                                                       \
+        crmsa_dispatch_ln_rows_kernel<NV, CRMSA, true><<<grid, block, 0, st>>>(x1, x0, wdisp, rep2, gamma, beta, y, L, dim, k, g, y16, prec16);  \
+    } else                                                                                                       \
+      crmsa_dispatch_ln_rows_kernel<NV, CRMSA, false><<<grid, block, 0, st>>>(x1, x0, wdisp, rep2, gamma, beta, y, L, dim, k, g, y16, prec16); \
+  } while (0)
+    if (dim <= 256) RRT_DISPATCH_ROWS(1);
+    else if (dim <= 512) RRT_DISPATCH_ROWS(2);
+    else if (dim <= 1024) RRT_DISPATCH_ROWS(4);
+    else RRT_DISPATCH_ROWS(8);
+#undef RRT_DISPATCH_ROWS
+    return hipGetLastError();
+  }
   dim3 grid((L + 4 * RW_DISPATCH - 1) / (4 * RW_DISPATCH)), block(256);
 #define RRT_DISPATCH(NV)                                                                                         \
   do {                                                                                                           \
@@ -2240,15 +2453,15 @@
 hipError_t launch_crmsa_dispatch_ln(const float* x1, const float* x0, const float* wdisp,
                                     const float* rep2, const float* gamma,
                                     const float* beta, float* y, int dim, int k, const GridDev& g8,
-                                    hipStream_t st, uint16_t* y16, int prec16) {
+                                    hipStream_t st, uint16_t* y16, int prec16, int rows_w) {
   if (y16 != nullptr && (gamma == nullptr || (prec16 != 1 && prec16 != 2) || dim % 4 != 0)) return hipErrorInvalidValue;
-  return launch_dispatch<true>(x1, x0, wdisp, rep2, gamma, beta, y, g8.L, dim, k, g8, st, y16, prec16);
+  return launch_dispatch<true>(x1, x0, wdisp, rep2, gamma, beta, y, g8.L, dim, k, g8, st, y16, prec16, rows_w);
 }
 
 hipError_t launch_layernorm(const float* x1, const float* x0, const float* gamma,
-                            const float* beta, float* y, int L, int dim, hipStream_t st) {
+                            const float* beta, float* y, int L, int dim, hipStream_t st, int rows_w) {
   GridDev g{};
   g.L = L;
   g.H = g.s = g.rs = g.P = 1;
-  return launch_dispatch<false>(x1, x0, nullptr, nullptr, gamma, beta, y, L, dim, 0, g, st);
-}
+  return launch_dispatch<false>(x1, x0, nullptr, nullptr, gamma, beta, y, L, dim, 0, g, st, nullptr, 0, rows_w);
+}
diff --git a/rrt-mil_amd/csrc/internal.h b/rrt-mil_amd/csrc/internal.h
--- a/rrt-mil_amd/csrc/internal.h
+++ b/rrt-mil_amd/csrc/internal.h
@@ -24,8 +24,10 @@
   }
 };
 
+constexpr int ROWS_W_MAX = 3;
+int device_cu_count();
 hipError_t launch_ln_partition(const float* x, const float* gamma, const float* beta, float* u,
-                               int dim, const GridDev& g, hipStream_t st, int* zero = nullptr, int n_zero = 0);
+                               int dim, const GridDev& g, hipStream_t st, int* zero = nullptr, int n_zero = 0, int rows_w = 0);
 
 struct LinearEpilogue {
   int prec;
@@ -171,9 +173,10 @@
 hipError_t launch_crmsa_dispatch_ln(const float* x1, const float* x0, const float* wdisp,
                                     const float* rep2, const float* gamma,
                                     const float* beta, float* y, int dim, int k, const GridDev& g8,
-                                    hipStream_t st, uint16_t* y16 = nullptr, int prec16 = 0);
+                                    hipStream_t st, uint16_t* y16 = nullptr, int prec16 = 0,
+                                    int rows_w = 0);
 hipError_t launch_layernorm(const float* x1, const float* x0, const float* gamma,
-                            const float* beta, float* y, int L, int dim, hipStream_t st);
+                            const float* beta, float* y, int L, int dim, hipStream_t st, int rows_w = 0);
 
 constexpr int POOL_CHUNK = 32;
 hipError_t launch_pool_partial(const float* y, const float* hid_a, const float* hid_b, const float* wc,
diff --git a/rrt-mil_amd/csrc/ln_partition.hip b/rrt-mil_amd/csrc/ln_partition.hip
--- a/rrt-mil_amd/csrc/ln_partition.hip
+++ b/rrt-mil_amd/csrc/ln_partition.hip
@@ -56,8 +56,123 @@
   }
 }
 
+template <int NV, bool FULL>
+__device__ __forceinline__ void lnp_rows_request(const float* __restrict__ x, int t, int dim, int lane, float4 (&r)[NV]) {
+  const float* src = x + (size_t)t * dim;
+#pragma unroll
+  for (int v = 0; v < NV; ++v) {
+    int c = (v * 64 + lane) * 4;
+    r[v] = (FULL || c < dim) ? ld_row<NT_LN1>(src + c) : make_float4(0.f, 0.f, 0.f, 0.f);
+  }
+}
+template <int NV, bool FULL>
+__device__ __forceinline__ void lnp_rows_reduce(const float4 (&r)[NV], const float4 (&gm)[NV], const float4 (&bt)[NV],
+                                                float* __restrict__ u, int t, int dim, int lane, float inv_d, const GridDev& g) {
+  float* dst = u + (size_t)token_to_slot(t, g) * dim;
+  if (t >= g.L) {
+#pragma unroll
+    for (int v = 0; v < NV; ++v) {
+      int c = (v * 64 + lane) * 4;
+      if (FULL || c < dim) *(float4*)(dst + c) = make_float4(0.f, 0.f, 0.f, 0.f);
+    }
+    return;
+  }
+  float sum = 0.f;
+#pragma unroll
+  for (int v = 0; v < NV; ++v) sum += (r[v].x + r[v].y) + (r[v].z + r[v].w);
+  const float mean = wave_sum(sum) * inv_d;
+  float sq = 0.f;
+#pragma unroll
+  for (int v = 0; v < NV; ++v) {
+    int c = (v * 64 + lane) * 4;
+    if (FULL || c < dim) {
+      float a = r[v].x - mean, b = r[v].y - mean, cc = r[v].z - mean, d = r[v].w - mean;
+      sq += (a * a + b * b) + (cc * cc + d * d);
+    }
+  }
+  const float rstd = 1.0f / sqrtf(wave_sum(sq) * inv_d + LN_EPS);
+#pragma unroll
+  for (int v = 0; v < NV; ++v) {
+    int c = (v * 64 + lane) * 4;
+    if (FULL || c < dim) {
+      float4 o;
+      o.x = (r[v].x - mean) * rstd * gm[v].x + bt[v].x;
+      o.y = (r[v].y - mean) * rstd * gm[v].y + bt[v].y;
+      o.z = (r[v].z - mean) * rstd * gm[v].z + bt[v].z;
+      o.w = (r[v].w - mean) * rstd * gm[v].w + bt[v].w;
+      *(float4*)(dst + c) = o;
+    }
+  }
+}
+
+template <int NV, bool FULL>
+__global__ __launch_bounds__(256) void ln_partition_rows_kernel(const float* __restrict__ x,
+                                                                const float* __restrict__ gamma,
+                                                                const float* __restrict__ beta,
+                                                                float* __restrict__ u, int dim, GridDev g,
+                                                                int* __restrict__ zero, int n_zero) {
+  if (zero != nullptr && blockIdx.x == 0)
+    for (int i = threadIdx.x; i < n_zero; i += 256) zero[i] = 0;
+  const int lane = threadIdx.x & 63;
+  const int W = gridDim.x * 4;
+  int t = __builtin_amdgcn_readfirstlane(blockIdx.x * 4 + (threadIdx.x >> 6));
+  if (t >= g.Np) return;
+  float4 gm[NV], bt[NV];
+#pragma unroll
+  for (int v = 0; v < NV; ++v) {
+    int c = (v * 64 + lane) * 4;
+    gm[v] = (FULL || c < dim) ? *(const float4*)(gamma + c) : make_float4(0.f, 0.f, 0.f, 0.f);
+    bt[v] = (FULL || c < dim) ? *(const float4*)(beta + c) : make_float4(0.f, 0.f, 0.f, 0.f);
+  }
+  const float inv_d = 1.0f / (float)dim;
+  const int last = g.L - 1;
+  float4 ra[NV], rb[NV];
+  lnp_rows_request<NV, FULL>(x, t < g.L ? t : last, dim, lane, ra);
+  for (;;) {
+    const int tn = t + W;
+    lnp_rows_request<NV, FULL>(x, tn < g.L ? tn : last, dim, lane, rb);
+    __builtin_amdgcn_sched_barrier(0);
+    lnp_rows_reduce<NV, FULL>(ra, gm, bt, u, t, dim, lane, inv_d, g);
+    if (tn >= g.Np) break;
+    t = tn + W;
+    lnp_rows_request<NV, FULL>(x, t < g.L ? t : last, dim, lane, ra);
+    __builtin_amdgcn_sched_barrier(0);
+    lnp_rows_reduce<NV, FULL>(rb, gm, bt, u, tn, dim, lane, inv_d, g);
+    if (t >= g.Np) break;
+  }
+}
+
+int device_cu_count() {
+  static int cus[64] = {};
+  int d = 0;
+  (void)hipGetDevice(&d);
+  d &= 63;
+  if (cus[d] == 0) {
+    int n = 0;
+    if (hipDeviceGetAttribute(&n, hipDeviceAttributeMultiprocessorCount, d) != hipSuccess || n <= 0) n = 256;
+    cus[d] = n;
+  }
+  return cus[d];
+}
+
 hipError_t launch_ln_partition(const float* x, const float* gamma, const float* beta, float* u,
-                               int dim, const GridDev& g, hipStream_t st, int* zero, int n_zero) {
+                               int dim, const GridDev& g, hipStream_t st, int* zero, int n_zero, int rows_w) {
+  if (rows_w > 0) {
+    if (rows_w > ROWS_W_MAX) return hipErrorInvalidValue;
+    const int rows_blocks = (g.Np + 3) / 4, fixed = device_cu_count() * rows_w;
+    dim3 grid(rows_blocks < fixed ? rows_blocks : fixed), block(256);
+#define RRT_LNP_ROWS(NV)                                                                         \
+  do {                                                                                         \
+    if (RRT_ALLOW_FULL && dim == NV * 256) ln_partition_rows_kernel<NV, true><<<grid, block, 0, st>>>(x, gamma, beta, u, dim, g, zero, n_zero);  \
+    else ln_partition_rows_kernel<NV, false><<<grid, block, 0, st>>>(x, gamma, beta, u, dim, g, zero, n_zero);            \
+  } while (0)
+    if (dim <= 256) RRT_LNP_ROWS(1);
+    else if (dim <= 512) RRT_LNP_ROWS(2);
+    else if (dim <= 1024) RRT_LNP_ROWS(4);
+    else RRT_LNP_ROWS(8);
+#undef RRT_LNP_ROWS
+    return hipGetLastError();
+  }
   dim3 grid((g.Np + 3) / 4), block(256);
 #define RRT_LNP(NV)                                                                              \
   do {                                                                                         \
```

After: 5454, median of 6. 1.02x the previous value.
